# Simple-Robotics/proxsuite

Hardware: AMD Instinct MI355X
Metric: QPs/sec (batch, dense backend) at fixed (n, n_eq, n_in); max |KKT residual| vs ref (higher is better)
Workload: dtype f64; 1 GPU; c2: 2048 random dense fp64 QPs per GPU, n=100 n_eq=50 n_in=100, eps_abs=1e-09 eps_rel=0 NO_INITIAL_GUESS (reference generators and seeds, benchmark/timings-parallel.cpp:43-63; BASELINE.json configs); batch_per_gpu=2048, n=100, n_eq=50, n_in=100, threads_per_qp=64, lds_bytes_per_qp=18968, parallelism=batch sharded over 1 GPU(s), dense_backend=PrimalDualLDLT

## Files before the change

include/proxqp_hip.h:

```cpp
#ifndef PROXQP_HIP_H
#define PROXQP_HIP_H

#include "pqp_types.h"

#ifdef __cplusplus
extern "C" {
#endif

typedef struct pqp_batch pqp_batch;

enum pqp_error
{
  PQP_OK = 0,
  PQP_ERR_INVALID_ARGUMENT = -1,
  PQP_ERR_NO_DEVICE = -2,
  PQP_ERR_HIP = -3,
  PQP_ERR_UNSUPPORTED = -4
};

#define PQP_STATS_COUNT 33

const char* pqp_last_error(void);
int pqp_device_count(void);

int pqp_batch_create(int64_t batch_size, int64_t dim, int64_t n_eq, int64_t n_in,
                     int box_constraints, int hessian_type, int dense_backend, int device,
                     pqp_batch** out);
void pqp_batch_destroy(pqp_batch* h);

int64_t pqp_batch_size(const pqp_batch* h);
int pqp_batch_dense_backend(const pqp_batch* h);

pqp_settings* pqp_batch_settings(pqp_batch* h, int64_t idx);

int pqp_batch_init(pqp_batch* h, int64_t idx, const double* H, const double* g, const double* A,
                   const double* b, const double* C, const double* l, const double* u,
                   const double* l_box, const double* u_box, int compute_preconditioner,
                   double rho, double mu_eq, double mu_in, double manual_minimal_H_eigenvalue);

int pqp_batch_update(pqp_batch* h, int64_t idx, const double* H, const double* g, const double* A,
                     const double* b, const double* C, const double* l, const double* u,
                     const double* l_box, const double* u_box, int update_preconditioner,
                     double rho, double mu_eq, double mu_in, double manual_minimal_H_eigenvalue);

int pqp_batch_warm_start(pqp_batch* h, int64_t idx, const double* x, const double* y,
                         const double* z);

int pqp_batch_cleanup(pqp_batch* h, int64_t idx);

int pqp_batch_reset_qp(pqp_batch* h, int64_t idx);

int pqp_batch_flush(pqp_batch* h);

int pqp_batch_solve(pqp_batch* h);

int pqp_batch_solve_range(pqp_batch* h, int64_t first, int64_t count);

int pqp_batch_solve_subset(pqp_batch* h, const int64_t* idx, int64_t count);

int pqp_batch_solve_async(pqp_batch* h);
int pqp_batch_solve_range_async(pqp_batch* h, int64_t first, int64_t count);
int pqp_batch_solve_subset_async(pqp_batch* h, const int64_t* idx, int64_t count);
int pqp_batch_wait(pqp_batch* h);

int pqp_batch_enable_host_results(pqp_batch* h, int enable);
int pqp_batch_host_results(pqp_batch* h, const double** x, const double** y, const double** z, const double** se,
                           const double** si, const pqp_info** info);
int pqp_batch_host_results_fresh(pqp_batch* h, int64_t idx);
int pqp_batch_host_results_fresh_range(pqp_batch* h, int64_t first, int64_t count);

int pqp_batch_copy_qp(pqp_batch* dst, int64_t dst_idx, pqp_batch* src, int64_t src_idx);

int pqp_batch_set_stream(pqp_batch* h, void* stream);
int pqp_batch_own_stream(pqp_batch* h);

int pqp_batch_backward(pqp_batch* h, const double* loss_derivatives, double eps, double rho_backward,
                       double mu_backward);
int pqp_batch_backward_range(pqp_batch* h, int64_t first, int64_t count, const double* loss_derivatives,
                             double eps, double rho_backward, double mu_backward);
int pqp_batch_backward_subset(pqp_batch* h, const int64_t* idx, int64_t count, const double* loss_derivatives,
                              double eps, double rho_backward, double mu_backward);
int pqp_batch_get_backward(pqp_batch* h, int64_t idx, double* dL_dH, double* dL_dg, double* dL_dA,
                           double* dL_db, double* dL_dC, double* dL_du, double* dL_dl);

int pqp_batch_set_schedule(pqp_batch* h, int longest_first);

int pqp_batch_get_results(pqp_batch* h, int64_t idx, double* x, double* y, double* z, double* se,
                          double* si, pqp_info* info);

int pqp_batch_result_device_ptrs(pqp_batch* h, double** x, double** y, double** z);

int pqp_batch_pack_results(pqp_batch* h, int64_t first, int64_t count, double* out, void* stream);

int pqp_batch_get_scaled(pqp_batch* h, int64_t idx, double* H, double* g, double* A, double* b,
                         double* C, double* l, double* u, double* delta, double* c);

int pqp_batch_get_schur_factor(pqp_batch* h, int64_t idx, double* WS, double* dS, double* G, int32_t* slots,
                               int64_t* meta, double* mus);

int pqp_batch_get_primal_factor(pqp_batch* h, int64_t idx, double* F, double* dF, double* WL, double* WU,
                                double* Zr, double* Zc, int64_t* meta, double* rho, double* i_scaled);

int pqp_batch_get_stats(pqp_batch* h, int64_t* stats);

int pqp_batch_get_trace(pqp_batch* h, int64_t idx, double* records, int64_t capacity, int64_t* n_records);

double pqp_batch_last_solve_ms(const pqp_batch* h);
double pqp_batch_last_prologue_ms(const pqp_batch* h);
int pqp_batch_launch_config(const pqp_batch* h, int* threads, int64_t* lds_bytes);
const char* pqp_batch_last_kernel(const pqp_batch* h);

typedef struct pqp_multi pqp_multi;
int pqp_multi_create(int64_t batch_size, int64_t dim, int64_t n_eq, int64_t n_in, int box_constraints,
                     int hessian_type, int dense_backend, const int* devices, int n_devices, pqp_multi** out);
void pqp_multi_destroy(pqp_multi* m);
int64_t pqp_multi_size(const pqp_multi* m);
int pqp_multi_shard_count(const pqp_multi* m);
int pqp_multi_shard(pqp_multi* m, int g, pqp_batch** shard, int64_t* first, int64_t* count);
int pqp_multi_locate(const pqp_multi* m, int64_t idx, int* shard, int64_t* local);
pqp_settings* pqp_multi_settings(pqp_multi* m, int64_t idx);
int pqp_multi_init(pqp_multi* m, int64_t idx, const double* H, const double* g, const double* A, const double* b,
                   const double* C, const double* l, const double* u, const double* l_box, const double* u_box,
                   int compute_preconditioner, double rho, double mu_eq, double mu_in,
                   double manual_minimal_H_eigenvalue);
int pqp_multi_update(pqp_multi* m, int64_t idx, const double* H, const double* g, const double* A, const double* b,
                     const double* C, const double* l, const double* u, const double* l_box, const double* u_box,
                     int update_preconditioner, double rho, double mu_eq, double mu_in,
                     double manual_minimal_H_eigenvalue);
int pqp_multi_warm_start(pqp_multi* m, int64_t idx, const double* x, const double* y, const double* z);
int pqp_multi_cleanup(pqp_multi* m, int64_t idx);
int pqp_multi_flush(pqp_multi* m);
int pqp_multi_solve(pqp_multi* m);
int pqp_multi_solve_range(pqp_multi* m, int64_t first, int64_t count);
int pqp_multi_solve_async(pqp_multi* m);
int pqp_multi_solve_range_async(pqp_multi* m, int64_t first, int64_t count);
int pqp_multi_wait(pqp_multi* m);
int pqp_multi_get_results(pqp_multi* m, int64_t idx, double* x, double* y, double* z, double* se, double* si,
                          pqp_info* info);
int pqp_multi_gather_device(pqp_multi* m, int root_shard, double* out);
int pqp_multi_get_trace(pqp_multi* m, int64_t idx, double* records, int64_t capacity, int64_t* n_records);
double pqp_multi_last_solve_ms(const pqp_multi* m);

int pqp_box_calibrate(int device, double* out, int n_out);

#ifdef __cplusplus
}
#endif

#endif
```

proxsuite_amd/_build.py:

```python
from __future__ import annotations

import os
import shutil
import subprocess
from pathlib import Path

ROOT = Path(__file__).resolve().parent.parent
CSRC = ROOT / "proxsuite_amd" / "csrc"
INCLUDE = ROOT / "include"

HIP_LIB = CSRC / "libproxqp_hip.so"
HIP_STATS_LIB = CSRC / "libproxqp_hip_stats.so"
RANDQP_LIB = CSRC / "libpqp_randqp.so"

HOST_CXXFLAGS = ["-O3", "-march=x86-64-v3", "-mtune=generic", "-std=gnu++17", "-fPIC", "-fopenmp"]


def _newer(target: Path, sources) -> bool:
    if not target.exists():
        return False
    t = target.stat().st_mtime
    return all(Path(s).stat().st_mtime <= t for s in sources)


def _run(cmd, cwd=None):
    r = subprocess.run(cmd, cwd=cwd, capture_output=True, text=True)
    if r.returncode != 0:
        raise RuntimeError("build failed: %s\n%s\n%s" % (" ".join(map(str, cmd)), r.stdout, r.stderr))
    return r


def build_randqp(force: bool = False) -> Path:
    src = [CSRC / "random_qp.cpp"]
    if not force and _newer(RANDQP_LIB, src):
        return RANDQP_LIB
    _run(["g++", *HOST_CXXFLAGS, "-shared", "-o", str(RANDQP_LIB), *map(str, src)])
    return RANDQP_LIB


KERNEL_TUS = (1, 2, 3, 4, 5, 6, 7, 8, 9, 12, 13, 14, 15, 16, 17, 18)
OBJ_DIR = ROOT / "build" / "obj"


def hip_sources():
    return [CSRC / "pqp_capi.hip", CSRC / "pqp_multi.hip", CSRC / "pqp_kernels.hip", CSRC / "pqp_calib.hip"]


def hip_headers():
    return sorted(CSRC.glob("*.hpp")) + sorted(INCLUDE.glob("*.h"))


CODEGEN_FLAGS = ["-mllvm", "-sink-insts-to-avoid-spills", "-mllvm", "-disable-machine-licm"]
TU_FLAGS = {17: ["-mllvm", "-disable-lsr"],
            18: ["-mllvm", "-disable-lsr", "-DPQP_ZG_DEPTH=4"],
            1: ["-mllvm", "-disable-lsr"], 4: ["-mllvm", "-disable-lsr"], 7: ["-mllvm", "-disable-lsr"], 13: ["-mllvm", "-disable-lsr"], 15: ["-mllvm", "-disable-lsr"]}


def hip_flags(extra_flags=()):
    return ["--offload-arch=gfx950", "-O3", "-std=c++17", "-fPIC", "-ffp-contract=fast", *CODEGEN_FLAGS,
            "-Rpass-analysis=kernel-resource-usage",
            "-I", str(INCLUDE), "-I", str(CSRC), *extra_flags]


def parse_kernel_resources(stderr: str) -> dict:
    import re
    out, cur = {}, None
    for line in stderr.splitlines():
        m = re.search(r"remark:\s+(Function Name|[A-Za-z ]+(?:\[[^\]]*\])?):\s*(\S+)", line)
        if not m:
            continue
        key, val = m.group(1).strip(), m.group(2)
        if key == "Function Name":
            cur = out.setdefault(val, {})
        elif cur is not None:
            key = re.sub(r"\s*\[.*\]", "", key).strip().replace(" ", "_")
            try:
                cur[key] = int(val)
            except ValueError:
                cur[key] = val
    return out


def kernel_label(mangled: str) -> str:
    import re
    m = re.match(r"_Z\d+([A-Za-z_0-9]+?)I((?:Li\d+E)+)E", mangled)
    if not m:
        return mangled
    return "%s<%s>" % (m.group(1), ",".join(re.findall(r"Li(\d+)E", m.group(2))))


def flags_tag(extra_flags) -> str:
    import hashlib
    return "v" + hashlib.sha1(" ".join(extra_flags).encode()).hexdigest()[:8]


def hipcc() -> str:
    return shutil.which("hipcc") or "/opt/rocm/bin/hipcc"


HOST_OBJECTS = {"capi.o": "pqp_capi.hip", "multi.o": "pqp_multi.hip", "calib.o": "pqp_calib.hip"}


def hip_objects(odir: Path, tus=KERNEL_TUS):
    return [odir / o for o in HOST_OBJECTS] + [odir / ("kernels_%d.o" % k) for k in tus]


def compile_tu(k: int, obj: Path, extra_flags=()):
    return _run([hipcc(), *hip_flags(extra_flags), *TU_FLAGS.get(k, []), "-DPQP_TU=%d" % k, "-c",
                 str(CSRC / "pqp_kernels.hip"), "-o", str(obj)])


def link_hip(lib: Path, odir: Path = None, replaced=None, tus=KERNEL_TUS) -> Path:
    odir, replaced = odir or OBJ_DIR / "default", replaced or {}
    Path(lib).parent.mkdir(parents=True, exist_ok=True)
    _run([hipcc(), "--offload-arch=gfx950", "-shared", "-fPIC", "-o", str(lib),
          *[str(replaced.get(o.name, o)) for o in hip_objects(odir, tus)]])
    return Path(lib)


def build_hip(force: bool = False, extra_flags=(), out: Path = None, tus=KERNEL_TUS) -> Path:
    from concurrent.futures import ThreadPoolExecutor
    lib = Path(out) if out else HIP_LIB
    deps = list(hip_sources()) + hip_headers() + [Path(__file__)]
    if not force and _newer(lib, deps):
        return lib
    tag = "default" if not extra_flags else flags_tag(extra_flags)
    odir = OBJ_DIR / tag
    odir.mkdir(parents=True, exist_ok=True)
    common = hip_headers() + [Path(__file__)]
    only = {"pqp_dwave.hpp": ("kernels_17.o", "kernels_6.o")}
    def deps_of(o):
        return [h for h in common if h.name not in only or o.name in only[h.name]] + [CSRC / HOST_OBJECTS.get(o.name, "pqp_kernels.hip")]
    def compile_object(o):
        if o.name in HOST_OBJECTS:
            return _run([hipcc(), *hip_flags(extra_flags), "-c", str(CSRC / HOST_OBJECTS[o.name]), "-o", str(o)])
        return compile_tu(int(o.stem.split("_")[1]), o, extra_flags)
    todo = [o for o in hip_objects(odir, tus) if force or not _newer(o, deps_of(o))]
    with ThreadPoolExecutor(max_workers=max(1, min(len(todo), os.cpu_count() or 1))) as ex:
        results = list(ex.map(compile_object, todo))
    link_hip(lib, odir, tus=tus)
    import json
    rec_path = odir / "kernel_resources.json"
    rec = json.loads(rec_path.read_text()) if rec_path.exists() else {}
    for o, r in zip(todo, results):
        rec = {k: v for k, v in rec.items() if v.get("object") != o.name}
        for name, fields in parse_kernel_resources(r.stderr).items():
            rec[kernel_label(name)] = dict(fields, object=o.name)
    rec_path.write_text(json.dumps(rec, indent=1, sort_keys=True))
    return lib


def kernel_resources(tag: str = "default") -> dict:
    import json
    p = OBJ_DIR / tag / "kernel_resources.json"
    rec = json.loads(p.read_text()) if p.exists() else {}
    live = {"kernels_%d.o" % k for k in KERNEL_TUS}
    return {k: v for k, v in rec.items() if v.get("object") in live}


def build_hip_stats(force: bool = False) -> Path:
    lib = HIP_STATS_LIB
    deps = list(hip_sources()) + hip_headers() + [Path(__file__)]
    if not force and _newer(lib, deps):
        return lib
    return build_hip(extra_flags=("-DPQP_STATS",), out=lib)


VARIANT_DIR = CSRC / "variants"


def build_hip_variants(force: bool = False):
    out = []
    deps = list(hip_sources()) + hip_headers() + [Path(__file__)]
    build_hip()
    for w in (3, 4):
        lib = VARIANT_DIR / ("libproxqp_hip_wps512_%d.so" % w)
        if force or not _newer(lib, deps):
            o3 = OBJ_DIR / "default" / ("kernels_3_wps%d.o" % w)
            compile_tu(3, o3, ("-DPQP_WPS_512=%d" % w,))
            link_hip(lib, replaced={"kernels_3.o": o3})
        out.append(lib)
    return out


def build_tu_variant(tu, extra_flags, out: Path):
    build_hip()
    repl, res = {}, {}
    for t in ([tu] if isinstance(tu, int) else list(tu)):
        o = OBJ_DIR / "default" / ("kernels_%d_%s.o" % (t, flags_tag(extra_flags)))
        r = compile_tu(t, o, tuple(extra_flags))
        repl["kernels_%d.o" % t] = o
        res.update({kernel_label(k): v for k, v in parse_kernel_resources(r.stderr).items()})
    return link_hip(out, replaced=repl), res


def build_oracle(force: bool = False) -> Path:
    odir = ROOT / "oracle"
    lib = odir / "liboracle.so"
    srcs = [odir / "proxqp_oracle.cpp", odir / "oracle_capi.cpp", odir / "proxqp_oracle.hpp",
            odir / "ldlt_oracle.hpp", INCLUDE / "pqp_types.h", odir / "Makefile"]
    if not force and _newer(lib, srcs):
        return lib
    if force and lib.exists():
        os.remove(lib)
    _run(["make", "-C", str(odir), "-B" if force else "-s", "liboracle.so"])
    return lib


def kernel_sources_sha(diag: bool = False, dwave: bool = False) -> str:
    import hashlib
    files = ["pqp_solver.hpp", "pqp_block.hpp"] + (["pqp_diag.hpp"] if diag or dwave else []) + (["pqp_dwave.hpp"] if dwave else [])
    import re
    h = hashlib.sha256()
    for f in files:
        text = (CSRC / f).read_text()
        text = re.sub(r"/\*.*?\*/", "", text, flags=re.S)
        lines = [re.sub(r"//.*$", "", ln).rstrip() for ln in text.splitlines()]
        h.update("\n".join(ln for ln in lines if ln.strip()).encode())
    return h.hexdigest()[:16]


def freeze_kernel_resources():
    import json
    build_hip()
    rec = kernel_resources()
    keep = ("VGPRs", "AGPRs", "VGPRs_Spill", "SGPRs_Spill", "ScratchSize", "Occupancy")
    out = {k: {f: v[f] for f in keep if f in v} for k, v in sorted(rec.items()) if k.startswith("pqp_")}
    p = ROOT / "tests" / "golden" / "kernel_resources_expected.json"
    p.write_text(json.dumps(out, indent=1, sort_keys=True))
    return p


if __name__ == "__main__":
    import sys
    if "--freeze" in sys.argv:
        print(freeze_kernel_resources())
```

proxsuite_amd/_native.py:

```python
from __future__ import annotations

import ctypes as C
import os
from pathlib import Path

import numpy as np

from ._ctypes_defs import pqp_info, pqp_settings

PQP_STATS_COUNT = 33
STAT_NAMES = ("cyc_total", "cyc_scale", "cyc_factor_h", "cyc_zg", "cyc_schur", "cyc_kkt_solve",
              "cyc_residual", "cyc_linesearch", "cyc_global_res", "cyc_newton_misc", "n_newton",
              "n_schur_fact", "n_new_rows", "n_kkt_solves", "n_ls_breakpoints", "n_active_final",
              "cyc_f_load", "cyc_f_update", "cyc_f_panel", "cyc_f_writeback", "cyc_f_tinv", "cyc_s_gather",
              "cyc_solve_ldlt", "n_schur_blocked", "n_append", "n_delete", "bytes_engine", "n_refactorize", "cyc_ls_eval", "cyc_cert", "cyc_update", "wall_ticks", "flops_fact")

_DP = C.POINTER(C.c_double)
NAN = float("nan")


class NativeError(RuntimeError):
    pass


class _Tolerant:

    class _Sink:
        pass

    def __init__(self, lib):
        object.__setattr__(self, "_lib", lib)

    def __getattr__(self, name):
        try:
            return getattr(object.__getattribute__(self, "_lib"), name)
        except AttributeError:
            return _Tolerant._Sink()


class NativeLib:

    SYMBOLS = ("pqp_last_error", "pqp_device_count", "pqp_batch_create", "pqp_batch_destroy",
               "pqp_batch_size", "pqp_batch_dense_backend", "pqp_batch_settings", "pqp_batch_init",
               "pqp_batch_update", "pqp_batch_warm_start", "pqp_batch_cleanup", "pqp_batch_reset_qp", "pqp_batch_flush",
               "pqp_batch_solve", "pqp_batch_solve_range", "pqp_batch_solve_subset", "pqp_batch_copy_qp", "pqp_batch_set_stream", "pqp_batch_set_schedule", "pqp_batch_backward", "pqp_batch_backward_range",
               "pqp_batch_get_backward", "pqp_batch_get_results", "pqp_batch_result_device_ptrs", "pqp_batch_pack_results",
               "pqp_batch_get_scaled", "pqp_batch_get_schur_factor", "pqp_batch_get_primal_factor", "pqp_batch_get_stats", "pqp_batch_get_trace", "pqp_batch_last_solve_ms", "pqp_batch_last_prologue_ms",
               "pqp_batch_launch_config", "pqp_batch_last_kernel", "pqp_batch_solve_async", "pqp_batch_solve_range_async",
               "pqp_batch_solve_subset_async", "pqp_batch_wait", "pqp_batch_enable_host_results",
               "pqp_batch_host_results", "pqp_batch_host_results_fresh", "pqp_batch_own_stream", "pqp_batch_backward_subset",
               "pqp_multi_create", "pqp_multi_destroy", "pqp_multi_size", "pqp_multi_shard_count", "pqp_multi_shard",
               "pqp_multi_locate", "pqp_multi_settings", "pqp_multi_init", "pqp_multi_update", "pqp_multi_warm_start",
               "pqp_multi_cleanup", "pqp_multi_flush", "pqp_multi_solve", "pqp_multi_solve_range",
               "pqp_multi_solve_async", "pqp_multi_solve_range_async", "pqp_multi_wait", "pqp_multi_get_results",
               "pqp_multi_gather_device", "pqp_multi_get_trace", "pqp_multi_last_solve_ms", "pqp_box_calibrate",
               "pqp_batch_host_results_fresh_range")

    def __init__(self, path, legacy=False):
        self.path = str(path)
        real = C.CDLL(self.path)
        L = _Tolerant(real) if legacy else real
        vp = C.c_void_p
        L.pqp_last_error.restype = C.c_char_p
        L.pqp_device_count.restype = C.c_int
        L.pqp_batch_create.argtypes = [C.c_int64] * 4 + [C.c_int] * 4 + [C.POINTER(vp)]
        L.pqp_batch_destroy.argtypes = [vp]
        L.pqp_batch_destroy.restype = None
        L.pqp_batch_size.argtypes = [vp]
        L.pqp_batch_size.restype = C.c_int64
        L.pqp_batch_dense_backend.argtypes = [vp]
        L.pqp_batch_settings.argtypes = [vp, C.c_int64]
        L.pqp_batch_settings.restype = C.POINTER(pqp_settings)
        for name in ("pqp_batch_init", "pqp_batch_update"):
            getattr(L, name).argtypes = [vp, C.c_int64] + [_DP] * 9 + [C.c_int] + [C.c_double] * 4
        L.pqp_batch_warm_start.argtypes = [vp, C.c_int64] + [_DP] * 3
        L.pqp_batch_cleanup.argtypes = [vp, C.c_int64]
        L.pqp_batch_reset_qp.argtypes = [vp, C.c_int64]
        L.pqp_batch_flush.argtypes = [vp]
        L.pqp_batch_solve.argtypes = [vp]
        L.pqp_batch_solve_range.argtypes = [vp, C.c_int64, C.c_int64]
        L.pqp_batch_solve_subset.argtypes = [vp, C.POINTER(C.c_int64), C.c_int64]
        L.pqp_batch_copy_qp.argtypes = [vp, C.c_int64, vp, C.c_int64]
        L.pqp_batch_set_stream.argtypes = [vp, vp]
        L.pqp_batch_set_schedule.argtypes = [vp, C.c_int]
        L.pqp_batch_backward.argtypes = [vp, _DP] + [C.c_double] * 3
        L.pqp_batch_backward_range.argtypes = [vp, C.c_int64, C.c_int64, _DP] + [C.c_double] * 3
        L.pqp_batch_get_backward.argtypes = [vp, C.c_int64] + [_DP] * 7
        L.pqp_batch_get_results.argtypes = [vp, C.c_int64] + [_DP] * 5 + [C.POINTER(pqp_info)]
        L.pqp_batch_result_device_ptrs.argtypes = [vp] + [C.POINTER(_DP)] * 3
        L.pqp_batch_pack_results.argtypes = [vp, C.c_int64, C.c_int64, vp, vp]
        L.pqp_batch_get_scaled.argtypes = [vp, C.c_int64] + [_DP] * 9
        L.pqp_batch_get_stats.argtypes = [vp, C.POINTER(C.c_int64)]
        L.pqp_batch_get_trace.argtypes = [vp, C.c_int64, C.c_void_p, C.c_int64, C.POINTER(C.c_int64)]
        L.pqp_batch_get_schur_factor.argtypes = [vp, C.c_int64] + [_DP] * 3 + [C.POINTER(C.c_int32), C.POINTER(C.c_int64), _DP]
        L.pqp_batch_get_primal_factor.argtypes = [vp, C.c_int64] + [_DP] * 6 + [C.POINTER(C.c_int64), _DP, _DP]
        L.pqp_batch_last_solve_ms.argtypes = [vp]
        L.pqp_batch_last_solve_ms.restype = C.c_double
        L.pqp_batch_last_prologue_ms.argtypes = [vp]
        L.pqp_batch_last_prologue_ms.restype = C.c_double
        L.pqp_batch_launch_config.argtypes = [vp, C.POINTER(C.c_int), C.POINTER(C.c_int64)]
        L.pqp_batch_last_kernel.argtypes = [vp]
        L.pqp_batch_last_kernel.restype = C.c_char_p
        L.pqp_batch_solve_async.argtypes = [vp]
        L.pqp_batch_solve_range_async.argtypes = [vp, C.c_int64, C.c_int64]
        L.pqp_batch_solve_subset_async.argtypes = [vp, C.POINTER(C.c_int64), C.c_int64]
        L.pqp_batch_wait.argtypes = [vp]
        L.pqp_batch_enable_host_results.argtypes = [vp, C.c_int]
        L.pqp_batch_host_results.argtypes = [vp] + [C.POINTER(_DP)] * 5 + [C.POINTER(C.POINTER(pqp_info))]
        L.pqp_batch_host_results_fresh.argtypes = [vp, C.c_int64]
        L.pqp_batch_own_stream.argtypes = [vp]
        L.pqp_batch_backward_subset.argtypes = [vp, C.POINTER(C.c_int64), C.c_int64, _DP] + [C.c_double] * 3
        L.pqp_multi_create.argtypes = [C.c_int64] * 4 + [C.c_int] * 3 + [C.POINTER(C.c_int), C.c_int, C.POINTER(vp)]
        L.pqp_multi_destroy.argtypes = [vp]
        L.pqp_multi_destroy.restype = None
        L.pqp_multi_size.argtypes = [vp]
        L.pqp_multi_size.restype = C.c_int64
        L.pqp_multi_shard_count.argtypes = [vp]
        L.pqp_multi_shard.argtypes = [vp, C.c_int, C.POINTER(vp), C.POINTER(C.c_int64), C.POINTER(C.c_int64)]
        L.pqp_multi_locate.argtypes = [vp, C.c_int64, C.POINTER(C.c_int), C.POINTER(C.c_int64)]
        L.pqp_multi_settings.argtypes = [vp, C.c_int64]
        L.pqp_multi_settings.restype = C.POINTER(pqp_settings)
        for name in ("pqp_multi_init", "pqp_multi_update"):
            getattr(L, name).argtypes = [vp, C.c_int64] + [_DP] * 9 + [C.c_int] + [C.c_double] * 4
        L.pqp_multi_warm_start.argtypes = [vp, C.c_int64] + [_DP] * 3
        L.pqp_multi_cleanup.argtypes = [vp, C.c_int64]
        for name in ("pqp_multi_flush", "pqp_multi_solve", "pqp_multi_solve_async", "pqp_multi_wait"):
            getattr(L, name).argtypes = [vp]
        for name in ("pqp_multi_solve_range", "pqp_multi_solve_range_async"):
            getattr(L, name).argtypes = [vp, C.c_int64, C.c_int64]
        L.pqp_multi_get_results.argtypes = [vp, C.c_int64] + [_DP] * 5 + [C.POINTER(pqp_info)]
        L.pqp_multi_gather_device.argtypes = [vp, C.c_int, vp]
        L.pqp_multi_last_solve_ms.argtypes = [vp]
        L.pqp_multi_last_solve_ms.restype = C.c_double
        L.pqp_multi_get_trace.argtypes = [vp, C.c_int64, C.c_void_p, C.c_int64, C.POINTER(C.c_int64)]
        L.pqp_box_calibrate.argtypes = [C.c_int, _DP, C.c_int]
        L.pqp_batch_host_results_fresh_range.argtypes = [vp, C.c_int64, C.c_int64]
        self.L = real

    def check(self, rc):
        if rc != 0:
            msg = self.L.pqp_last_error().decode(errors="replace")
            if rc == -1:
                raise ValueError(msg)
            raise NativeError("libproxqp_hip error %d: %s" % (rc, msg))


_lib = None


def hip_library_path() -> Path:
    override = os.environ.get("PQP_HIP_LIBRARY")
    if override:
        return Path(override).resolve()
    return Path(__file__).resolve().parent / "csrc" / "libproxqp_hip.so"


def load() -> NativeLib:
    global _lib
    if _lib is None:
        p = hip_library_path()
        if not p.exists():
            raise NativeError("%s is missing: build it with `python -c 'import __graft_entry__ as g; "
                              "g.build()'` (hipcc --offload-arch=gfx950); there is no CPU fallback" % p)
        try:
            import torch
        except ImportError:
            pass
        lib = NativeLib(p)
        if lib.L.pqp_device_count() <= 0:
            raise NativeError("no HIP device visible: proxsuite_amd runs on MI355X only (no CPU fallback)")
        _lib = lib
    return _lib


def box_calibration(device: int = 0, lib: NativeLib = None) -> dict:
    lib = lib or load()
    out = (C.c_double * 8)()
    rc = lib.L.pqp_box_calibrate(int(device), out, 8)
    if rc != 0:
        raise NativeError("pqp_box_calibrate: %s" % (lib.L.pqp_last_error() or b"").decode())
    return {"hbm_read_gbs": out[0], "chain_ms": out[1], "valu_ms": out[2], "sclk_mhz_est": out[3], "n_cu": int(out[4])}


def _as_array(a, shape, name):
    if a is None:
        return None, None
    if hasattr(a, "data_ptr"):
        import torch
        if a.numel() == 0:
            return None, None
        t = a.detach()
        if t.dtype != torch.float64 or not t.is_contiguous():
            t = t.to(torch.float64).contiguous()
        if tuple(t.shape) != tuple(shape):
            raise ValueError("wrong argument size: %s has shape %s, expected %s" % (name, tuple(t.shape), shape))
        return t, C.cast(t.data_ptr(), _DP)
    arr = np.ascontiguousarray(np.asarray(a, dtype=np.float64))
    if arr.size == 0:
        return None, None
    if tuple(arr.shape) != tuple(shape):
        raise ValueError("wrong argument size: %s has shape %s, expected %s" % (name, arr.shape, tuple(shape)))
    return arr, arr.ctypes.data_as(_DP)


def _opt(v):
    return NAN if v is None else float(v)


class Batch:

    def __init__(self, batch_size, n, n_eq, n_in, box_constraints=False, hessian_type=1, dense_backend=0,
                 device=0, lib: NativeLib | None = None):
        self.lib = lib if lib is not None else load()
        self.B, self.n, self.n_eq, self.n_in = int(batch_size), int(n), int(n_eq), int(n_in)
        self.box = bool(box_constraints)
        self.n_c = self.n_in + (self.n if self.box else 0)
        h = C.c_void_p()
        self.lib.check(self.lib.L.pqp_batch_create(self.B, self.n, self.n_eq, self.n_in, int(self.box),
                                                   int(hessian_type), int(dense_backend), int(device),
                                                   C.byref(h)))
        self._h = h

    def close(self):
        if getattr(self, "_h", None):
            self.lib.L.pqp_batch_destroy(self._h)
            self._h = None

    def __del__(self):
        try:
            self.close()
        except Exception:
            pass

    @property
    def dense_backend(self):
        return self.lib.L.pqp_batch_dense_backend(self._h)

    def settings(self, idx) -> pqp_settings:
        p = self.lib.L.pqp_batch_settings(self._h, int(idx))
        if not p:
            raise IndexError(idx)
        return p.contents

    def settings_table(self):
        p = self.lib.L.pqp_batch_settings(self._h, 0)
        arr = (pqp_settings * self.B).from_address(C.addressof(p.contents))
        return np.frombuffer(arr, dtype=np.dtype(pqp_settings))

    def set_all_settings(self, **fields):
        tab = self.settings_table()
        for k, v in fields.items():
            tab[k][:] = v

    def _shapes(self, idx):
        pre = (self.B,) if idx < 0 else ()
        n, ne, ni = self.n, self.n_eq, self.n_in
        return dict(H=pre + (n, n), g=pre + (n,), A=pre + (ne, n), b=pre + (ne,), C=pre + (ni, n),
                    l=pre + (ni,), u=pre + (ni,), l_box=pre + (n,), u_box=pre + (n,))

    def _setup(self, fn, idx, H, g, A, b, Cm, l, u, l_box, u_box, flag, rho, mu_eq, mu_in, min_eig):
        sh = self._shapes(idx)
        keep, ptrs = [], []
        for name, arr in (("H", H), ("g", g), ("A", A), ("b", b), ("C", Cm), ("l", l), ("u", u),
                          ("l_box", l_box), ("u_box", u_box)):
            k, p = _as_array(arr, sh[name], name)
            keep.append(k)
            ptrs.append(p)
        self.lib.check(fn(self._h, int(idx), *ptrs, int(bool(flag)), _opt(rho), _opt(mu_eq), _opt(mu_in),
                          _opt(min_eig)))

    def init(self, idx=-1, H=None, g=None, A=None, b=None, C=None, l=None, u=None, l_box=None, u_box=None,
             compute_preconditioner=True, rho=None, mu_eq=None, mu_in=None, manual_minimal_H_eigenvalue=None):
        self._setup(self.lib.L.pqp_batch_init, idx, H, g, A, b, C, l, u, l_box, u_box,
                    compute_preconditioner, rho, mu_eq, mu_in, manual_minimal_H_eigenvalue)

    def update(self, idx=-1, H=None, g=None, A=None, b=None, C=None, l=None, u=None, l_box=None, u_box=None,
               update_preconditioner=False, rho=None, mu_eq=None, mu_in=None,
               manual_minimal_H_eigenvalue=None):
        self._setup(self.lib.L.pqp_batch_update, idx, H, g, A, b, C, l, u, l_box, u_box,
                    update_preconditioner, rho, mu_eq, mu_in, manual_minimal_H_eigenvalue)

    def warm_start(self, idx=-1, x=None, y=None, z=None):
        pre = (self.B,) if idx < 0 else ()
        kx, px = _as_array(x, pre + (self.n,), "x")
        ky, py = _as_array(y, pre + (self.n_eq,), "y")
        kz, pz = _as_array(z, pre + (self.n_c,), "z")
        self.lib.check(self.lib.L.pqp_batch_warm_start(self._h, int(idx), px, py, pz))

    def cleanup(self, idx=-1):
        self.lib.check(self.lib.L.pqp_batch_cleanup(self._h, int(idx)))

    def flush(self):
        self.lib.check(self.lib.L.pqp_batch_flush(self._h))

    def solve(self, first=None, count=None):
        if first is None:
            self.lib.check(self.lib.L.pqp_batch_solve(self._h))
        else:
            self.lib.check(self.lib.L.pqp_batch_solve_range(self._h, int(first), int(1 if count is None else count)))

    def solve_async(self, first=None, count=None):
        if first is None:
            self.lib.check(self.lib.L.pqp_batch_solve_async(self._h))
        else:
            self.lib.check(self.lib.L.pqp_batch_solve_range_async(self._h, int(first), int(1 if count is None else count)))

    def wait(self):
        self.lib.check(self.lib.L.pqp_batch_wait(self._h))

    def solve_subset(self, idx, asynchronous=False):
        ii = np.ascontiguousarray(idx, dtype=np.int64)
        fn = self.lib.L.pqp_batch_solve_subset_async if asynchronous else self.lib.L.pqp_batch_solve_subset
        self.lib.check(fn(self._h, ii.ctypes.data_as(C.POINTER(C.c_int64)), len(ii)))

    def enable_host_results(self, on=True):
        self.lib.check(self.lib.L.pqp_batch_enable_host_results(self._h, int(bool(on))))

    def host_results(self):
        px = [_DP() for _ in range(5)]
        pi = C.POINTER(pqp_info)()
        self.lib.check(self.lib.L.pqp_batch_host_results(self._h, *[C.byref(p) for p in px], C.byref(pi)))
        shapes = ((self.B, self.n), (self.B, self.n_eq), (self.B, self.n_c), (self.B, self.n_eq), (self.B, self.n_c))
        out = []
        for p, sh in zip(px, shapes):
            cnt = sh[0] * sh[1]
            out.append(np.ctypeslib.as_array(p, shape=(cnt,)).reshape(sh) if cnt else np.zeros(sh))
        if self.B:
            arr = (pqp_info * self.B).from_address(C.addressof(pi.contents))
            info = np.frombuffer(arr, dtype=np.dtype(pqp_info))
        else:
            info = np.zeros(0, dtype=np.dtype(pqp_info))
        return (*out, info)

    def host_results_fresh(self, idx=-1, count=None):
        if count is not None:
            return bool(self.lib.L.pqp_batch_host_results_fresh_range(self._h, int(idx), int(count)))
        return bool(self.lib.L.pqp_batch_host_results_fresh(self._h, int(idx)))

    def backward(self, loss_derivatives, eps=1e-4, rho_backward=1e-6, mu_backward=1e-6, first=None, count=None):
        ntot = self.n + self.n_eq + self.n_in
        rows = self.B if first is None else int(1 if count is None else count)
        k, p = _as_array(loss_derivatives, (rows, ntot), "loss_derivatives")
        if first is None:
            self.lib.check(self.lib.L.pqp_batch_backward(self._h, p, float(eps), float(rho_backward),
                                                         float(mu_backward)))
        else:
            self.lib.check(self.lib.L.pqp_batch_backward_range(self._h, int(first), rows, p, float(eps),
                                                               float(rho_backward), float(mu_backward)))

    def backward_results(self, idx=-1, into=None):
        pre = (self.B,) if idx < 0 else ()
        n, ne, ni = self.n, self.n_eq, self.n_in
        shapes = dict(dL_dH=pre + (n, n), dL_dg=pre + (n,), dL_dA=pre + (ne, n), dL_db=pre + (ne,),
                      dL_dC=pre + (ni, n), dL_du=pre + (ni,), dL_dl=pre + (ni,))
        out = into if into is not None else {k: np.zeros(v) for k, v in shapes.items()}
        ptrs = []
        for name in ("dL_dH", "dL_dg", "dL_dA", "dL_db", "dL_dC", "dL_du", "dL_dl"):
            buf = out.get(name)
            if buf is None or (hasattr(buf, "numel") and buf.numel() == 0) or (
                    not hasattr(buf, "numel") and buf.size == 0):
                ptrs.append(None)
            elif hasattr(buf, "data_ptr"):
                import torch
                if buf.dtype != torch.float64 or not buf.is_contiguous() or tuple(buf.shape) != shapes[name]:
                    raise ValueError("backward_results: %s must be contiguous float64 of shape %s" % (name, shapes[name]))
                ptrs.append(C.cast(buf.data_ptr(), _DP))
            else:
                ptrs.append(buf.ctypes.data_as(_DP))
        self.lib.check(self.lib.L.pqp_batch_get_backward(self._h, int(idx), *ptrs))
        return out

    def pack_results(self, out, first=0, count=None, stream=None):
        count = self.B - first if count is None else count
        ptr = out.data_ptr() if hasattr(out, "data_ptr") else (out.ctypes.data if hasattr(out, "ctypes") else int(out))
        self.lib.check(self.lib.L.pqp_batch_pack_results(self._h, int(first), int(count), C.c_void_p(ptr),
                                                         C.c_void_p(int(stream) if stream else None)))
        return out

    def set_schedule(self, longest_first=True):
        self.lib.check(self.lib.L.pqp_batch_set_schedule(self._h, int(bool(longest_first))))

    def own_stream(self):
        self.lib.check(self.lib.L.pqp_batch_own_stream(self._h))

    def backward_subset(self, idx, loss_derivatives, eps=1e-4, rho_backward=1e-6, mu_backward=1e-6):
        ntot = self.n + self.n_eq + self.n_in
        ii = np.ascontiguousarray(idx, dtype=np.int64)
        k, p = _as_array(loss_derivatives, (len(ii), ntot), "loss_derivatives")
        self.lib.check(self.lib.L.pqp_batch_backward_subset(self._h, ii.ctypes.data_as(C.POINTER(C.c_int64)), len(ii), p,
                                                            float(eps), float(rho_backward), float(mu_backward)))

    def set_stream(self, stream):
        self.lib.check(self.lib.L.pqp_batch_set_stream(self._h, C.c_void_p(int(stream) if stream else None)))

    @property
    def last_solve_ms(self):
        return self.lib.L.pqp_batch_last_solve_ms(self._h)

    @property
    def last_prologue_ms(self):
        return self.lib.L.pqp_batch_last_prologue_ms(self._h)

    def results(self, idx=-1):
        pre = (self.B,) if idx < 0 else ()
        x = np.zeros(pre + (self.n,))
        y = np.zeros(pre + (self.n_eq,))
        z = np.zeros(pre + (self.n_c,))
        se = np.zeros(pre + (self.n_eq,))
        si = np.zeros(pre + (self.n_c,))
        info = (pqp_info * self.B)() if idx < 0 else pqp_info()
        p = lambda a: a.ctypes.data_as(_DP)
        ip = C.cast(info, C.POINTER(pqp_info)) if idx < 0 else C.byref(info)
        self.lib.check(self.lib.L.pqp_batch_get_results(self._h, int(idx), p(x), p(y), p(z), p(se), p(si), ip))
        return x, y, z, se, si, info

    def results_into(self, x=None, y=None, z=None, se=None, si=None, idx=-1):
        pre = (self.B,) if idx < 0 else ()
        want = dict(x=pre + (self.n,), y=pre + (self.n_eq,), z=pre + (self.n_c,), se=pre + (self.n_eq,),
                    si=pre + (self.n_c,))
        ptrs = []
        for name, buf in (("x", x), ("y", y), ("z", z), ("se", se), ("si", si)):
            if buf is None or (hasattr(buf, "numel") and buf.numel() == 0) or (hasattr(buf, "size") and not callable(buf.size) and buf.size == 0):
                ptrs.append(None)
                continue
            if hasattr(buf, "data_ptr"):
                import torch
                if buf.dtype != torch.float64 or not buf.is_contiguous() or tuple(buf.shape) != want[name]:
                    raise ValueError("results_into: %s must be a contiguous float64 tensor of shape %s" % (name, want[name]))
                ptrs.append(C.cast(buf.data_ptr(), _DP))
            else:
                if buf.dtype != np.float64 or not buf.flags.c_contiguous or tuple(buf.shape) != want[name]:
                    raise ValueError("results_into: %s must be a C-contiguous float64 array of shape %s" % (name, want[name]))
                ptrs.append(buf.ctypes.data_as(_DP))
        self.lib.check(self.lib.L.pqp_batch_get_results(self._h, int(idx), *ptrs, None))

    def infos(self):
        info = (pqp_info * self.B)()
        self.lib.check(self.lib.L.pqp_batch_get_results(self._h, -1, None, None, None, None, None,
                                                        C.cast(info, C.POINTER(pqp_info))))
        return info

    def scaled(self, idx):
        n, ne, ni = self.n, self.n_eq, self.n_in
        out = dict(H=np.zeros((n, n)), g=np.zeros(n), A=np.zeros((ne, n)), b=np.zeros(ne), C=np.zeros((ni, n)),
                   l=np.zeros(ni), u=np.zeros(ni), delta=np.zeros(n + ne + self.n_c))
        c = C.c_double(0)
        p = lambda a: a.ctypes.data_as(_DP)
        self.lib.check(self.lib.L.pqp_batch_get_scaled(
            self._h, int(idx), p(out["H"]), p(out["g"]), p(out["A"]), p(out["b"]), p(out["C"]), p(out["l"]),
            p(out["u"]), p(out["delta"]), C.cast(C.byref(c), _DP)))
        out["c"] = c.value
        return out

    def schur_factor(self, idx):
        nd, nc = self.n_eq + self.n_c, self.n_c
        WS, dS, G = np.zeros((nd, nd)), np.zeros(nd), np.zeros((nd, nd))
        slots, meta, mus = np.zeros(max(nc, 1), dtype=np.int32), np.zeros(4, dtype=np.int64), np.zeros(2)
        self.lib.check(self.lib.L.pqp_batch_get_schur_factor(
            self._h, idx, WS.ctypes.data_as(_DP), dS.ctypes.data_as(_DP), G.ctypes.data_as(_DP),
            slots.ctypes.data_as(C.POINTER(C.c_int32)), meta.ctypes.data_as(C.POINTER(C.c_int64)), mus.ctypes.data_as(_DP)))
        return WS, dS, G, slots[:nc], dict(zip(("n_slots", "n_c", "ls_valid", "ls_edited"), meta.tolist())), mus

    def primal_factor(self, idx):
        n, nd = self.n, self.n_eq + self.n_c
        out = dict(F=np.zeros((n, n)), dF=np.zeros(n), WL=np.zeros((n, n)), WU=np.zeros((n, n)), Zr=np.zeros((nd, n)),
                   Zc=np.zeros((n, nd)), i_scaled=np.zeros(n))
        meta, rho = np.zeros(4, dtype=np.int64), C.c_double(0)
        p = lambda a: a.ctypes.data_as(_DP)
        self.lib.check(self.lib.L.pqp_batch_get_primal_factor(
            self._h, int(idx), p(out["F"]), p(out["dF"]), p(out["WL"]), p(out["WU"]), p(out["Zr"]), p(out["Zc"]),
            meta.ctypes.data_as(C.POINTER(C.c_int64)), C.cast(C.byref(rho), _DP), p(out["i_scaled"])))
        out["rho"] = rho.value
        out["meta"] = dict(zip(("factor_valid", "diag_mode", "backend", "hessian"), meta.tolist()))
        return out

    def stats(self):
        a = np.zeros((self.B, PQP_STATS_COUNT), dtype=np.int64)
        self.lib.check(self.lib.L.pqp_batch_get_stats(self._h, a.ctypes.data_as(C.POINTER(C.c_int64))))
        return a

    def trace(self, idx):
        n = C.c_int64(0)
        self.lib.check(self.lib.L.pqp_batch_get_trace(self._h, int(idx), None, 0, C.byref(n)))
        out = np.zeros((n.value, 8))
        if n.value:
            self.lib.check(self.lib.L.pqp_batch_get_trace(self._h, int(idx), out.ctypes.data, n.value, C.byref(n)))
        return out

    @property
    def last_kernel(self):
        return self.lib.L.pqp_batch_last_kernel(self._h).decode()

    def launch_config(self):
        t = C.c_int(0)
        b = C.c_int64(0)
        self.lib.check(self.lib.L.pqp_batch_launch_config(self._h, C.byref(t), C.byref(b)))
        return t.value, b.value

    def result_device_ptrs(self):
        x, y, z = _DP(), _DP(), _DP()
        self.lib.check(self.lib.L.pqp_batch_result_device_ptrs(self._h, C.byref(x), C.byref(y), C.byref(z)))
        return tuple(C.cast(p, C.c_void_p).value for p in (x, y, z))



class MultiBatch:

    def __init__(self, batch_size, n, n_eq, n_in, devices, box_constraints=False, hessian_type=1, dense_backend=0,
                 lib: NativeLib | None = None):
        self.lib = lib if lib is not None else load()
        self.B, self.n, self.n_eq, self.n_in = int(batch_size), int(n), int(n_eq), int(n_in)
        self.box = bool(box_constraints)
        self.n_c = self.n_in + (self.n if self.box else 0)
        devs = (C.c_int * len(devices))(*[int(d) for d in devices])
        h = C.c_void_p()
        self.lib.check(self.lib.L.pqp_multi_create(self.B, self.n, self.n_eq, self.n_in, int(self.box), int(hessian_type),
                                                   int(dense_backend), devs, len(devices), C.byref(h)))
        self._h = h
        self.devices = [int(d) for d in devices]

    def close(self):
        if getattr(self, "_h", None):
            self.lib.L.pqp_multi_destroy(self._h)
            self._h = None

    def __del__(self):
        try:
            self.close()
        except Exception:
            pass

    @property
    def shard_count(self):
        return self.lib.L.pqp_multi_shard_count(self._h)

    def shard(self, g):
        f, c = C.c_int64(0), C.c_int64(0)
        self.lib.check(self.lib.L.pqp_multi_shard(self._h, int(g), None, C.byref(f), C.byref(c)))
        return f.value, c.value

    def settings(self, idx) -> pqp_settings:
        p = self.lib.L.pqp_multi_settings(self._h, int(idx))
        if not p:
            raise IndexError(idx)
        return p.contents

    _shapes = Batch._shapes

    def _setup(self, fn, idx, H, g, A, b, Cm, l, u, l_box, u_box, flag, rho, mu_eq, mu_in, min_eig):
        Batch._setup(self, fn, idx, H, g, A, b, Cm, l, u, l_box, u_box, flag, rho, mu_eq, mu_in, min_eig)

    def init(self, idx=-1, H=None, g=None, A=None, b=None, C=None, l=None, u=None, l_box=None, u_box=None,
             compute_preconditioner=True, rho=None, mu_eq=None, mu_in=None, manual_minimal_H_eigenvalue=None):
        self._setup(self.lib.L.pqp_multi_init, idx, H, g, A, b, C, l, u, l_box, u_box, compute_preconditioner, rho, mu_eq,
                    mu_in, manual_minimal_H_eigenvalue)
# ... 61 lines not shown
```

proxsuite_amd/csrc/pqp_capi.hip:

```cpp
#include <hip/hip_runtime.h>

#include <algorithm>
#include <cmath>
#include <cstdio>
#include <cstdlib>
#include <cstring>
#include <limits>
#include <string>
#include <vector>

#include "pqp_host.hpp"
#include "pqp_diag.hpp"

namespace {

thread_local std::string g_err;

bool
absent(double v)
{
  return std::isnan(v);
}

int
// ... 237 lines not shown
    h->dev.wall_us_per_tick =
      (hipDeviceGetAttribute(&khz, hipDeviceAttributeWallClockRate, device) == hipSuccess && khz > 0) ? 1.0e3 / double(khz)
                                                                                                      : 1.0e-2;
  }
  h->backend = dense_backend_choice(dense_backend, dim, n_eq, n_in, box_constraints != 0);
  pqp::Dims& d = h->dev.d;
  d.n = int(dim);
  d.n_eq = int(n_eq);
  d.n_in = int(n_in);
  d.box = box_constraints ? 1 : 0;
  d.nc = int(n_in + (box_constraints ? dim : 0));
  d.nd = d.n_eq + d.nc;
  d.ntot = d.n + d.nd;
  d.hessian = hessian_type;
  d.backend = h->backend;
  d._pad = 0;
  h->dev.B = batch_size;
  const int need = d.nd > d.n ? d.nd : d.n;
  h->nt = need <= 256 ? 256 : (need <= 512 ? 512 : 1024);
  if (need > PQP_MAX_ROWS || pqp::setup_lds_bytes(d, 1024) > 160 * 1024) {
    delete h;
    return fail(PQP_ERR_UNSUPPORTED, "max(n, n_eq + n_in (+ n)) > " + std::to_string(PQP_MAX_ROWS) +
                                       " (or n + n_eq + n_in (+ n) > ~10000) is not supported by this build");
  }
#if PQP_CHUNK_ALL
  if (const char* e = std::getenv("PQP_TEST_NT_MAX")) {
    const int f = std::atoi(e);
    if ((f == 256 || f == 512) && h->nt > f)
      h->nt = f;
  }
#endif
  if (const char* e = std::getenv("PQP_SCHEDULE"))
    h->lpt = std::string(e) == "lpt";
  h->dev.rep_phase = 0;
  h->dev.rep_count = 1;
  h->dev.trace = nullptr;
  h->dev.trace_slot = nullptr;
  h->dev.trace_cap = 0;
  if (const char* e = std::getenv("PQP_REPEAT_PHASE"))
    h->dev.rep_phase = std::atoi(e);
  if (const char* e = std::getenv("PQP_REPEAT_COUNT"))
    h->dev.rep_count = std::atoi(e);
  h->lds_solve = pqp::lds_bytes(d, h->nt);
  h->lds_setup = pqp::setup_lds_bytes(d, h->nt);
  const char* force_hbm = std::getenv("PQP_FORCE_HBM_VECTORS");
  const bool vectors_in_hbm = h->lds_solve > 160 * 1024 || (force_hbm && force_hbm[0] == '1');
  if (vectors_in_hbm)
    h->nt = 1024;
  const size_t B = size_t(batch_size), n = size_t(dim), ne = size_t(n_eq), ni = size_t(n_in),
               nc = size_t(d.nc), nd = size_t(d.nd);
  pqp::Batch& D = h->dev;
  int rc = 0;
#define ALLOC(ptr, cnt)                                                                             \
  if ((rc = dalloc(h, &(ptr), (cnt)))) {                                                            \
    pqp_batch_destroy(h);                                                                           \
    return rc;                                                                                      \
  }                                                                                                 \
  if (B > 0 && size_t(cnt) % B == 0 && (void*)(ptr) != (void*)h->d_order && (void*)(ptr) != (void*)h->d_cmd)           \
    h->per_qp.push_back({ reinterpret_cast<char*>(ptr), (size_t(cnt) / B) * sizeof(*(ptr)) });
  ALLOC(D.H, B * n * n)
  ALLOC(D.g, B * n)
  ALLOC(D.A, B * ne * n)
  ALLOC(D.b, B * ne)
  ALLOC(D.C, B * ni * n)
  ALLOC(D.u, B * ni)
  ALLOC(D.l, B * ni)
  ALLOC(D.u_box, B * n)
  ALLOC(D.l_box, B * n)
  ALLOC(D.Hs, B * n * n)
  ALLOC(D.gs, B * n)
  ALLOC(D.As, B * ne * n)
  ALLOC(D.ATs, B * ne * n)
  ALLOC(D.bs, B * ne)
  ALLOC(D.Cs, B * ni * n)
  ALLOC(D.CTs, B * ni * n)
  ALLOC(D.us, B * ni)
  ALLOC(D.ls, B * ni)
  ALLOC(D.ubs, B * n)
  ALLOC(D.lbs, B * n)
  ALLOC(D.is, B * n)
  ALLOC(D.delta, B * size_t(d.ntot))
  ALLOC(D.x, B * n)
  ALLOC(D.y, B * ne)
  ALLOC(D.z, B * nc)
  ALLOC(D.se, B * ne)
  ALLOC(D.si, B * nc)
  ALLOC(D.info, B)
  ALLOC(D.state, B)
  ALLOC(D.F, B * n * n)
  ALLOC(D.WL, B * n * n)
  ALLOC(D.WU, B * n * n)
  ALLOC(D.dF, B * n)
  ALLOC(D.Zr, B * nd * n)
  ALLOC(D.Zc, B * nd * n)
  ALLOC(D.G, B * nd * nd)
  ALLOC(D.WS, B * nd * nd)
  ALLOC(D.LS, B * nd * nd)
  ALLOC(D.dS, B * nd)
  ALLOC(D.act, B * nc)
  ALLOC(D.stats, B * size_t(pqp::ST_COUNT))
  if (vectors_in_hbm) {
    h->lds_solve = pqp::lds_bytes(d, h->nt);
    h->lds_setup = pqp::setup_lds_bytes(d, h->nt);
    if ((rc = dalloc(h, &h->vec_scratch, B * ((h->lds_solve + 7) / 8)))) {
      pqp_batch_destroy(h);
      return rc;
    }
  }
  ALLOC(h->d_order, B)
  ALLOC(h->d_settings, B)
  ALLOC(h->d_cmd, B)
#undef ALLOC
  D.settings = h->d_settings;
  D.cmd = h->d_cmd;

  h->settings.resize(B);
  for (auto& s : h->settings)
    pqp_settings_default(&s, h->backend);
  h->cmd.assign(B, pqp::Cmd{});
  h->is_initialized.assign(B, 0);
  h->c_diag.assign(B, 0);
  {
    std::vector<pqp_info> info(B);
    for (auto& i : info)
      pqp_info_default(&i, h->backend);
    if (B)
      HIP_TRY(hipMemcpy(D.info, info.data(), B * sizeof(pqp_info), hipMemcpyHostToDevice));
    std::vector<pqp::State> st(B);
    for (auto& s : st) {
      std::memset(&s, 0, sizeof(s));
      s.ruiz_c = 1.0;
    }
    if (B)
      HIP_TRY(hipMemcpy(D.state, st.data(), B * sizeof(pqp::State), hipMemcpyHostToDevice));
    const double ib = std::sqrt(std::numeric_limits<double>::max());
    std::vector<double> tmp;
    auto fill = [&](double* dst, size_t cnt, double v) -> int {
      if (!cnt)
        return PQP_OK;
      tmp.assign(cnt, v);
      HIP_TRY(hipMemcpy(dst, tmp.data(), cnt * sizeof(double), hipMemcpyHostToDevice));
      return PQP_OK;
    };
    if ((rc = fill(D.u, B * ni, +ib)) || (rc = fill(D.l, B * ni, -ib)) ||
        (rc = fill(D.u_box, B * n, +ib)) || (rc = fill(D.l_box, B * n, -ib)) ||
        (rc = fill(D.delta, B * size_t(d.ntot), 1.0)) || (rc = fill(D.is, B * n, 1.0))) {
      pqp_batch_destroy(h);
      return rc;
    }
  }
  HIP_TRY(hipEventCreate(&h->ev0));
  HIP_TRY(hipEventCreate(&h->ev1));
  HIP_TRY(hipEventCreate(&h->ev_mid));
  *out = h;
  return PQP_OK;
}

void
pqp_batch_destroy(pqp_batch* h)
{
  if (!h)
    return;
  (void)settle(h);
  DeviceGuard guard_(h->device);
  for (void* p : h->host_allocs)
    (void)hipHostFree(p);
  if (h->owned_stream)
    (void)hipStreamDestroy(h->owned_stream);
  for (void* p : h->allocs)
    (void)hipFree(p);
  if (h->trace_dev)
    (void)hipFree(h->trace_dev);
  if (h->trace_slot_dev)
    (void)hipFree(h->trace_slot_dev);
  if (h->ev0)
    (void)hipEventDestroy(h->ev0);
  if (h->ev1)
    (void)hipEventDestroy(h->ev1);
  if (h->ev_mid)
    (void)hipEventDestroy(h->ev_mid);
  delete h;
}

int64_t
pqp_batch_size(const pqp_batch* h)
{
  return h ? h->dev.B : 0;
}

int
pqp_batch_dense_backend(const pqp_batch* h)
{
  return h ? h->backend : PQP_BACKEND_AUTOMATIC;
}

pqp_settings*
pqp_batch_settings(pqp_batch* h, int64_t idx)
{
  if (!h || idx < 0 || idx >= h->dev.B)
    return nullptr;
  return &h->settings[size_t(idx)];
}

int
pqp_batch_init(pqp_batch* h, int64_t idx, const double* H, const double* g, const double* A,
               const double* b, const double* C, const double* l, const double* u,
               const double* l_box, const double* u_box, int compute_preconditioner, double rho,
               double mu_eq, double mu_in, double manual_minimal_H_eigenvalue)
{
  if (h && h->dev.d.box == 0 && (l_box || u_box))
    return fail(PQP_ERR_INVALID_ARGUMENT,
                "wrong model setup: the QP object is designed without box constraints, but is "
                "initialized with lower or upper box inequalities.");
  return enqueue_setup(h, idx, false, H, g, A, b, C, l, u, l_box, u_box, compute_preconditioner ? 1 : 0,
                       rho, mu_eq, mu_in, manual_minimal_H_eigenvalue);
}

int
pqp_batch_update(pqp_batch* h, int64_t idx, const double* H, const double* g, const double* A,
                 const double* b, const double* C, const double* l, const double* u,
                 const double* l_box, const double* u_box, int update_preconditioner, double rho,
                 double mu_eq, double mu_in, double manual_minimal_H_eigenvalue)
{
  return enqueue_setup(h, idx, true, H, g, A, b, C, l, u, l_box, u_box, update_preconditioner ? 1 : 0,
                       rho, mu_eq, mu_in, manual_minimal_H_eigenvalue);
}

int
pqp_batch_warm_start(pqp_batch* h, int64_t idx, const double* x, const double* y, const double* z)
{
  if (int rc = check_idx(h, idx))
    return rc;
  if (!x && !y && !z)
    return PQP_OK;
  if (int rc = settle(h))
    return rc;
  mirror_stale(h, idx);
  PQP_ON_DEVICE(h->device);
  if (h->cmd_pending)
    if (int rc = pqp_batch_flush(h))
      return rc;
  const pqp::Dims& d = h->dev.d;
  int rc = 0;
  if ((rc = copy_in(h->dev.x, x, idx, h->dev.B, size_t(d.n))) ||
      (rc = copy_in(h->dev.y, y, idx, h->dev.B, size_t(d.n_eq))) ||
      (rc = copy_in(h->dev.z, z, idx, h->dev.B, size_t(d.nc))))
    return rc;
  const int64_t lo = idx < 0 ? 0 : idx, hi = idx < 0 ? h->dev.B : idx + 1;
  for (int64_t q = lo; q < hi; ++q)
    h->settings[size_t(q)].initial_guess = PQP_WARM_START;
  return PQP_OK;
}

int
pqp_batch_cleanup(pqp_batch* h, int64_t idx)
{
  if (int rc = check_idx(h, idx))
    return rc;
  if (int rc = settle(h))
    return rc;
  mirror_stale(h, idx);
  if (h->cmd_pending)
    if (int rc = pqp_batch_flush(h))
      return rc;
  const int64_t lo = idx < 0 ? 0 : idx, hi = idx < 0 ? h->dev.B : idx + 1;
  for (int64_t q = lo; q < hi; ++q) {
    pqp::Cmd c{};
    c.op = pqp::CMD_CLEANUP;
    h->cmd[size_t(q)] = c;
    h->is_initialized[size_t(q)] = 0;
  }
  h->cmd_pending = true;
  return pqp_batch_flush(h);
}

int
pqp_batch_reset_qp(pqp_batch* h, int64_t idx)
{
  if (!h || idx < 0 || idx >= h->dev.B)
    return fail(PQP_ERR_INVALID_ARGUMENT, "QP index out of range");
  if (int rc = settle(h))
    return rc;
  mirror_stale(h, idx);
  PQP_ON_DEVICE(h->device);
  if (h->cmd_pending)
    if (int rc = pqp_batch_flush(h))
      return rc;
  const size_t q = size_t(idx);
  for (const auto& a : h->per_qp)
    HIP_TRY(hipMemset(a.base + q * a.bytes_per_qp, 0, a.bytes_per_qp));
  pqp::Batch& D = h->dev;
  const pqp::Dims& d = D.d;
  const size_t n = size_t(d.n), ni = size_t(d.n_in);
  pqp_info info;
  pqp_info_default(&info, h->backend);
  HIP_TRY(hipMemcpy(D.info + q, &info, sizeof(info), hipMemcpyHostToDevice));
  pqp::State st;
  std::memset(&st, 0, sizeof(st));
  st.ruiz_c = 1.0;
  HIP_TRY(hipMemcpy(D.state + q, &st, sizeof(st), hipMemcpyHostToDevice));
  const double ib = std::sqrt(std::numeric_limits<double>::max());
  std::vector<double> tmp;
  auto fill = [&](double* dst, size_t cnt, double v) -> int {
    if (!cnt)
      return PQP_OK;
    tmp.assign(cnt, v);
    HIP_TRY(hipMemcpy(dst, tmp.data(), cnt * sizeof(double), hipMemcpyHostToDevice));
    return PQP_OK;
  };
  int rc = 0;
  if ((rc = fill(D.u + q * ni, ni, +ib)) || (rc = fill(D.l + q * ni, ni, -ib)) ||
      (rc = fill(D.u_box + q * n, n, +ib)) || (rc = fill(D.l_box + q * n, n, -ib)) ||
      (rc = fill(D.delta + q * size_t(d.ntot), size_t(d.ntot), 1.0)) || (rc = fill(D.is + q * n, n, 1.0)))
    return rc;
  pqp_settings_default(&h->settings[q], h->backend);
  h->settings_dirty = true;
  h->settings_uploaded.clear();
  h->cmd[q] = pqp::Cmd{};
  h->is_initialized[q] = 0;
  h->c_diag[q] = 0;
  h->order_valid = false;
  return PQP_OK;
}

int
pqp_batch_flush(pqp_batch* h)
{
  if (!h)
    return fail(PQP_ERR_INVALID_ARGUMENT, "null batch handle");
  if (!h->cmd_pending || h->dev.B == 0)
    return PQP_OK;
  if (int rc = settle(h))
    return rc;
// ... 154 lines not shown
static int
verbose_report(pqp_batch* h, const int64_t* idx, int64_t first, int64_t count)
{
  bool any = false;
  for (int64_t i = 0; i < count && !any; ++i)
    any = h->settings[size_t(idx ? idx[i] : first + i)].verbose != 0;
  if (!any)
    return PQP_OK;
  if (h->dev.trace) {
    int nv = 0;
    for (int s : h->trace_slot)
      nv = std::max(nv, s + 1);
    h->trace_host.resize(size_t(nv) * PQP_TRACE_RECORDS * 8);
    HIP_TRY(hipMemcpy(h->trace_host.data(), h->trace_dev, h->trace_host.size() * sizeof(double), hipMemcpyDeviceToHost));
  }
  const pqp::Dims& d = h->dev.d;
  static const char* const status_name[] = { "Solved", "Maximum number of iterations reached", "Primal infeasible",
                                             "Solved closest primal feasible", "Dual infeasible", "Solver not run" };
  for (int64_t i = 0; i < count; ++i) {
    const int64_t q = idx ? idx[i] : first + i;
    const pqp_settings& st = h->settings[size_t(q)];
    if (!st.verbose)
      continue;
    pqp_info info;
    HIP_TRY(hipMemcpy(&info, h->dev.info + q, sizeof(info), hipMemcpyDeviceToHost));
    std::printf("-------------------------------------------------------------------------------------------------\n"
                "ProxQP dense backend, batched on MI355X (QP %lld of the batch)\n"
                "problem:  \n          variables n = %d, equality constraints n_eq = %d,\n"
                "          inequality constraints n_in = %d\n"
                "settings: \n          backend = dense,\n          eps_abs = %g eps_rel = %g\n"
                "          eps_prim_inf = %g, eps_dual_inf = %g,\n          rho = %g, mu_eq = %g, mu_in = %g,\n"
                "          max_iter = %lld, max_iter_in = %lld,\n          box constraints: %s, \n"
                "          dense backend: %s, \n          problem type: %s, \n          scaling: %s, \n"
                "          timings: %s, \n",
                (long long)q, d.n, d.n_eq, d.n_in, st.eps_abs, st.eps_rel, st.eps_primal_inf, st.eps_dual_inf, info.rho,
                info.mu_eq, info.mu_in, (long long)st.max_iter, (long long)st.max_iter_in, d.box ? "on" : "off",
                h->backend == PQP_BACKEND_PRIMAL_LDLT ? "PrimalLDLT" : "PrimalDualLDLT",
                d.hessian == PQP_HESSIAN_DENSE
                  ? "Quadratic Program"
                  : (d.hessian == PQP_HESSIAN_ZERO ? "Linear Program" : "Quadratic Program with diagonal Hessian"),
                st.compute_preconditioner ? "on" : "off", st.compute_timings ? "on" : "off");
    if (!h->trace_host.empty() && h->trace_slot[size_t(q)] >= 0)
      print_trace(h->trace_host.data() + size_t(h->trace_slot[size_t(q)]) * PQP_TRACE_RECORDS * 8);
    std::printf("-------------------SOLVER STATISTICS-------------------\n"
                "outer iter:     %lld\ntotal iter:     %lld\nmu updates:     %lld\nrho updates:    %lld\n"
                "objective:      %g\nstatus:         %s\n",
                (long long)info.iter_ext, (long long)info.iter, (long long)info.mu_updates,
                (long long)info.rho_updates, info.objValue,
                (info.status >= 0 && info.status <= 5) ? status_name[info.status] : "?");
    if (st.compute_timings)
      std::printf("run time [\xce\xbcs]:  %g\n", info.solve_time);
    std::printf("--------------------------------------------------------\n");
  }
  std::fflush(stdout);
  return PQP_OK;
}

static int
finish_solve(pqp_batch* h)
{
  const int64_t* idx = h->flight_idx.empty() ? nullptr : h->flight_idx.data();
  const int64_t first = h->flight_first, count = h->flight_count;
  for (int64_t i = 0; i < count; ++i) {
    const size_t q = size_t(idx ? idx[i] : first + i);
    h->is_initialized[q] = 1;
    if (h->host_results)
      h->mirror_fresh[q] = 1;
  }
  return verbose_report(h, idx, first, count);
}

static int
solve_impl(pqp_batch* h, int64_t first, int64_t count, const int64_t* idx, bool async)
{
  if (!h)
    return fail(PQP_ERR_INVALID_ARGUMENT, "null batch handle");
  if (int rc = settle(h))
    return rc;
  std::vector<int> order;
  if (idx) {
    if (count < 0 || count > h->dev.B)
      return fail(PQP_ERR_INVALID_ARGUMENT, "subset larger than the batch");
    if (count == 0)
      return PQP_OK;
    order.resize(static_cast<size_t>(count));
    std::vector<char> seen(static_cast<size_t>(h->dev.B), 0);
    for (int64_t i = 0; i < count; ++i) {
      if (idx[i] < 0 || idx[i] >= h->dev.B)
        return fail(PQP_ERR_INVALID_ARGUMENT, "QP index out of range");
      if (seen[size_t(idx[i])])
        return fail(PQP_ERR_INVALID_ARGUMENT, "pqp_batch_solve_subset: a QP index is listed twice");
      seen[size_t(idx[i])] = 1;
      order[size_t(i)] = int(idx[i]);
    }
  } else {
    if (first < 0 || count < 0 || first + count > h->dev.B)
      return fail(PQP_ERR_INVALID_ARGUMENT, "solve range [" + std::to_string(first) + ", " +
                                              std::to_string(first + count) + ") outside the batch of " +
                                              std::to_string(h->dev.B) + " QPs");
    if (count == 0)
      return PQP_OK;
  }
  PQP_ON_DEVICE(h->device);
  if (int rc = pqp_batch_flush(h))
    return rc;
  if (int rc = upload_settings(h))
    return rc;
  if (int rc = prepare_trace(h, idx, first, count))
    return rc;
  int rc = 0;
  if (idx) {
    HIP_TRY(hipMemcpy(h->d_order, order.data(), order.size() * sizeof(int), hipMemcpyHostToDevice));
    h->order_valid = false;
    h->range_first = 0;
    h->range_count = long(count);
    h->subset_order = h->d_order;
    h->subset_host = &order;
    rc = pqp_launch_solve(h);
    h->subset_order = nullptr;
    h->subset_host = nullptr;
    h->flight_idx.assign(idx, idx + count);
  } else {
    h->range_first = first;
    h->range_count = count;
    rc = pqp_launch_solve(h);
    h->flight_idx.clear();
    if (!rc && h->lpt && first == 0 && count == h->dev.B && count > 1) {
      rc = pqp_launch_order(h, long(count));
      h->order_valid = rc == 0;
    }
  }
  if (rc)
    return rc;
  h->flight_first = long(first);
  h->flight_count = long(count);
  h->solve_in_flight = true;
  return async ? PQP_OK : pqp_batch_wait(h);
}

int
pqp_batch_wait(pqp_batch* h)
{
  if (!h)
    return fail(PQP_ERR_INVALID_ARGUMENT, "null batch handle");
  if (!h->solve_in_flight)
    return PQP_OK;
  PQP_ON_DEVICE(h->device);
  h->solve_in_flight = false;
  HIP_TRY(hipEventSynchronize(h->ev1));
  HIP_TRY(hipEventElapsedTime(&h->last_ms, h->ev0, h->ev1));
  h->last_prologue_ms = 0.f;
  if (h->prologue_timed)
    HIP_TRY(hipEventElapsedTime(&h->last_prologue_ms, h->ev0, h->ev_mid));
  return finish_solve(h);
}

int
pqp_batch_solve_range(pqp_batch* h, int64_t first, int64_t count)
{
  return solve_impl(h, first, count, nullptr, false);
}

int
pqp_batch_solve_subset(pqp_batch* h, const int64_t* idx, int64_t count)
{
  if (!h || (count > 0 && !idx))
    return fail(PQP_ERR_INVALID_ARGUMENT, "null argument");
  if (count == 0)
    return PQP_OK;
  return solve_impl(h, 0, count, idx, false);
}

int
pqp_batch_solve_async(pqp_batch* h)
{
  if (!h)
    return fail(PQP_ERR_INVALID_ARGUMENT, "null batch handle");
  return solve_impl(h, 0, h->dev.B, nullptr, true);
}

int
pqp_batch_solve_range_async(pqp_batch* h, int64_t first, int64_t count)
{
  return solve_impl(h, first, count, nullptr, true);
}

int
pqp_batch_solve_subset_async(pqp_batch* h, const int64_t* idx, int64_t count)
{
  if (!h || (count > 0 && !idx))
    return fail(PQP_ERR_INVALID_ARGUMENT, "null argument");
  if (count == 0)
    return PQP_OK;
  return solve_impl(h, 0, count, idx, true);
}

int
pqp_batch_enable_host_results(pqp_batch* h, int enable)
{
  if (!h)
    return fail(PQP_ERR_INVALID_ARGUMENT, "null batch handle");
  if (int rc = settle(h))
    return rc;
  if ((enable != 0) == h->host_results)
    return PQP_OK;
  PQP_ON_DEVICE(h->device);
  pqp::Batch& D = h->dev;
  if (!enable) {
    for (void* p : h->host_allocs)
      (void)hipHostFree(p);
    h->host_allocs.clear();
    D.hx = D.hy = D.hz = D.hse = D.hsi = nullptr;
    D.hinfo = nullptr;
    h->m_x = h->m_y = h->m_z = h->m_se = h->m_si = nullptr;
    h->m_info = nullptr;
    h->host_results = false;
    return PQP_OK;
  }
  const pqp::Dims& d = D.d;
  const size_t B = size_t(D.B);
  auto halloc = [&](size_t bytes, void** host, void** dev) -> int {
    void* p = nullptr;
    HIP_TRY(hipHostMalloc(&p, bytes ? bytes : 8, hipHostMallocMapped));
    h->host_allocs.push_back(p);
    std::memset(p, 0, bytes ? bytes : 8);
    void* dp = nullptr;
    HIP_TRY(hipHostGetDevicePointer(&dp, p, 0));
    *host = p;
    *dev = dp;
    return PQP_OK;
  };
  int rc = 0;
  if ((rc = halloc(B * size_t(d.n) * 8, (void**)&h->m_x, (void**)&D.hx)) ||
      (rc = halloc(B * size_t(d.n_eq) * 8, (void**)&h->m_y, (void**)&D.hy)) ||
      (rc = halloc(B * size_t(d.nc) * 8, (void**)&h->m_z, (void**)&D.hz)) ||
      (rc = halloc(B * size_t(d.n_eq) * 8, (void**)&h->m_se, (void**)&D.hse)) ||
      (rc = halloc(B * size_t(d.nc) * 8, (void**)&h->m_si, (void**)&D.hsi)) ||
      (rc = halloc(B * sizeof(pqp_info), (void**)&h->m_info, (void**)&D.hinfo))) {
    for (void* p : h->host_allocs)
      (void)hipHostFree(p);
    h->host_allocs.clear();
    D.hx = D.hy = D.hz = D.hse = D.hsi = nullptr;
    D.hinfo = nullptr;
    return rc;
  }
  h->mirror_fresh.assign(B, 0);
  h->host_results = true;
  return PQP_OK;
}

int
pqp_batch_host_results(pqp_batch* h, const double** x, const double** y, const double** z, const double** se,
                       const double** si, const pqp_info** info)
{
  if (!h)
    return fail(PQP_ERR_INVALID_ARGUMENT, "null batch handle");
  if (!h->host_results)
    return fail(PQP_ERR_INVALID_ARGUMENT, "pqp_batch_enable_host_results has not been called on this batch");
  if (int rc = settle(h))
    return rc;
  if (x)
    *x = h->m_x;
  if (y)
    *y = h->m_y;
  if (z)
    *z = h->m_z;
  if (se)
    *se = h->m_se;
  if (si)
    *si = h->m_si;
  if (info)
    *info = h->m_info;
  return PQP_OK;
}

int
pqp_batch_host_results_fresh(pqp_batch* h, int64_t idx)
{
  if (!h || !h->host_results || idx < -1 || idx >= h->dev.B)
    return 0;
  if (settle(h))
    return 0;
  if (idx >= 0)
    return h->mirror_fresh[size_t(idx)] ? 1 : 0;
  for (char c : h->mirror_fresh)
    if (!c)
      return 0;
  return 1;
}

int
pqp_batch_host_results_fresh_range(pqp_batch* h, int64_t first, int64_t count)
{
  if (!h || !h->host_results || first < 0 || count < 0 || first + count > h->dev.B)
    return 0;
  if (settle(h))
    return 0;
  for (int64_t q = first; q < first + count; ++q)
    if (!h->mirror_fresh[size_t(q)])
      return 0;
  return 1;
}

int
pqp_batch_copy_qp(pqp_batch* dst, int64_t dst_idx, pqp_batch* src, int64_t src_idx)
{
// ... 241 lines not shown
int
pqp_batch_get_scaled(pqp_batch* h, int64_t idx, double* H, double* g, double* A, double* b, double* C,
                     double* l, double* u, double* delta, double* c)
{
  if (int rc = check_idx(h, idx))
    return rc;
  if (idx < 0)
    return fail(PQP_ERR_INVALID_ARGUMENT, "pqp_batch_get_scaled addresses one QP");
  if (int rc = settle(h))
    return rc;
  PQP_ON_DEVICE(h->device);
  if (h->cmd_pending)
    if (int rc = pqp_batch_flush(h))
      return rc;
  const pqp::Dims& d = h->dev.d;
  const pqp::Batch& D = h->dev;
  const size_t n = size_t(d.n), ne = size_t(d.n_eq), ni = size_t(d.n_in);
  int rc = 0;
  if ((rc = copy_out(H, D.Hs, idx, D.B, n * n)) || (rc = copy_out(g, D.gs, idx, D.B, n)) ||
      (rc = copy_out(A, D.As, idx, D.B, ne * n)) || (rc = copy_out(b, D.bs, idx, D.B, ne)) ||
      (rc = copy_out(C, D.Cs, idx, D.B, ni * n)) || (rc = copy_out(l, D.ls, idx, D.B, ni)) ||
      (rc = copy_out(u, D.us, idx, D.B, ni)) || (rc = copy_out(delta, D.delta, idx, D.B, size_t(d.ntot))))
    return rc;
  if (c) {
    pqp::State s;
    HIP_TRY(hipMemcpy(&s, D.state + idx, sizeof(s), hipMemcpyDefault));
    *c = s.ruiz_c;
  }
  return PQP_OK;
}

int
pqp_batch_get_schur_factor(pqp_batch* h, int64_t idx, double* WS, double* dS, double* G, int32_t* slots,
                           int64_t* meta, double* mus)
{
  if (int rc = check_idx(h, idx))
    return rc;
  if (idx < 0)
    return fail(PQP_ERR_INVALID_ARGUMENT, "pqp_batch_get_schur_factor addresses one QP");
  if (int rc = settle(h))
    return rc;
  PQP_ON_DEVICE(h->device);
  const pqp::Dims& d = h->dev.d;
  const pqp::Batch& D = h->dev;
  const size_t nd = size_t(d.nd), nc = size_t(d.nc);
  int rc = 0;
  if ((rc = copy_out(WS, D.WS, idx, D.B, nd * nd)) || (rc = copy_out(dS, D.dS, idx, D.B, nd)) ||
      (rc = copy_out(G, D.G, idx, D.B, nd * nd)))
    return rc;
  if (slots && nc) {
    std::vector<int> raw(nc);
    HIP_TRY(hipMemcpy(raw.data(), D.act + size_t(idx) * nc, nc * sizeof(int), hipMemcpyDefault));
    for (size_t j = 0; j < nc; ++j)
      slots[j] = pqp::act_cid(raw[j]);
  }
  pqp::State s;
  HIP_TRY(hipMemcpy(&s, D.state + idx, sizeof(s), hipMemcpyDefault));
  if (meta) {
    meta[0] = s.n_slots;
    meta[1] = s.n_c;
    meta[2] = s.ls_valid;
    meta[3] = s.ls_edited;
  }
  if (mus) {
    mus[0] = s.mu_eq_fact;
    mus[1] = s.mu_in_fact;
  }
  return PQP_OK;
}

int
pqp_batch_get_primal_factor(pqp_batch* h, int64_t idx, double* F, double* dF, double* WL, double* WU, double* Zr,
                            double* Zc, int64_t* meta, double* rho, double* i_scaled)
{
  if (int rc = check_idx(h, idx))
    return rc;
  if (idx < 0)
    return fail(PQP_ERR_INVALID_ARGUMENT, "pqp_batch_get_primal_factor addresses one QP");
  if (int rc = settle(h))
    return rc;
  PQP_ON_DEVICE(h->device);
  const pqp::Dims& d = h->dev.d;
  const pqp::Batch& D = h->dev;
  const size_t n = size_t(d.n), nd = size_t(d.nd);
  int rc = 0;
  if ((rc = copy_out(F, D.F, idx, D.B, n * n)) || (rc = copy_out(dF, D.dF, idx, D.B, n)) ||
      (rc = copy_out(WL, D.WL, idx, D.B, n * n)) || (rc = copy_out(WU, D.WU, idx, D.B, n * n)) ||
      (rc = copy_out(Zr, D.Zr, idx, D.B, nd * n)) || (rc = copy_out(Zc, D.Zc, idx, D.B, n * nd)) ||
      (rc = copy_out(i_scaled, D.is, idx, D.B, n)))
    return rc;
  pqp::State s;
  HIP_TRY(hipMemcpy(&s, D.state + idx, sizeof(s), hipMemcpyDefault));
  if (meta) {
    meta[0] = s.factor_valid;
    meta[1] = (pqp::diag_structure_signature(d.hessian, d.n_eq, d.n_in, d.box) && s.c_diag != 0) ? 1 : 0;
    meta[2] = d.backend;
    meta[3] = d.hessian;
  }
  if (rho)
    *rho = s.rho_fact;
  return PQP_OK;
}

int
pqp_batch_get_stats(pqp_batch* h, int64_t* stats)
{
  if (!h || !stats)
    return fail(PQP_ERR_INVALID_ARGUMENT, "null argument");
  static_assert(PQP_STATS_COUNT == pqp::ST_COUNT, "stats record size");
  static_assert(sizeof(long long) == sizeof(int64_t), "stats element size");
  if (int rc = settle(h))
    return rc;
  PQP_ON_DEVICE(h->device);
  HIP_TRY(hipMemcpy(stats, h->dev.stats, size_t(h->dev.B) * pqp::ST_COUNT * sizeof(int64_t), hipMemcpyDefault));
  return PQP_OK;
}

int
pqp_batch_get_trace(pqp_batch* h, int64_t idx, double* records, int64_t capacity, int64_t* n_records)
{
  if (!h || !n_records)
    return fail(PQP_ERR_INVALID_ARGUMENT, "null argument");
  if (idx < 0 || idx >= h->dev.B)
    return fail(PQP_ERR_INVALID_ARGUMENT, "QP index out of range");
  if (int rc = settle(h))
    return rc;
  *n_records = 0;
  if (h->trace_host.empty() || h->trace_slot.empty() || h->trace_slot[size_t(idx)] < 0)
    return PQP_OK;
  const double* slot = h->trace_host.data() + size_t(h->trace_slot[size_t(idx)]) * PQP_TRACE_RECORDS * 8;
  const int64_t n = int64_t(slot[0]);
  *n_records = n;
  if (records && capacity > 0)
    std::memcpy(records, slot + 8, size_t(std::min(n, capacity)) * 8 * sizeof(double));
  return PQP_OK;
}

double
pqp_batch_last_solve_ms(const pqp_batch* h)
{
  if (h && h->solve_in_flight)
    (void)pqp_batch_wait(const_cast<pqp_batch*>(h));
  return h ? double(h->last_ms) : 0.0;
}

double
pqp_batch_last_prologue_ms(const pqp_batch* h)
{
  if (h && h->solve_in_flight)
    (void)pqp_batch_wait(const_cast<pqp_batch*>(h));
  return h ? double(h->last_prologue_ms) : 0.0;
}

int
pqp_batch_launch_config(const pqp_batch* h, int* threads, int64_t* lds_bytes)
{
  if (!h)
    return fail(PQP_ERR_INVALID_ARGUMENT, "null batch handle");
  const LaunchPlan p = pqp_plan_solve(h, 0, long(h->dev.B), nullptr);
  if (threads)
    *threads = p.threads;
  if (lds_bytes)
    *lds_bytes = int64_t(p.lds);
  return PQP_OK;
}

const char*
pqp_batch_last_kernel(const pqp_batch* h)
{
  return h ? h->last_kernel : "";
}

}
```

proxsuite_amd/csrc/pqp_dwave.hpp:

```cpp
#ifndef PQP_DWAVE_HPP
#define PQP_DWAVE_HPP

#include "pqp_diag.hpp"
#include <utility>

namespace pqp {

#ifndef PQP_DW_HB
#define PQP_DW_HB 2
#endif
#ifndef PQP_DW_SCHUR_LAZY
#define PQP_DW_SCHUR_LAZY 1
#endif
#ifndef PQP_DW_SCHUR_REG_BLOCKS
#define PQP_DW_SCHUR_REG_BLOCKS 8
#endif
constexpr int DW_SCHUR_REG_BLOCKS = PQP_DW_SCHUR_REG_BLOCKS;
constexpr int DW_MAXDIM = 128;

enum
{
  DLV_XP = 0,
  DLV_YP,
  DLV_ZP,
  DLV_GS,
  DLV_BS,
  DLV_US,
  DLV_LS,
  DLV_COUNT
};
constexpr int DW_SCR = 1024;
constexpr int DW_INTS = 128 + 128 + 256 + 256 + 2 * INCR_MAX;

__host__ __device__ inline size_t
dwave_lds_bytes()
{
  return (size_t)DW_INTS * sizeof(int) + (size_t)(DLV_COUNT * 128 + DW_SCR) * sizeof(double) + (ST_COUNT + 2) * sizeof(long long);
}

__host__ __device__ inline bool
dwave_signature(const Dims& d)
{
  return d.box == 0 && d.hessian == PQP_HESSIAN_DENSE && d.backend != PQP_BACKEND_PRIMAL_LDLT && d.n <= DW_MAXDIM &&
         d.n_eq <= DW_MAXDIM && d.n_in <= DW_MAXDIM && d.n >= 2;
}

struct DPair
{
  double x, y;
};
__device__ __forceinline__ DPair
dw_load_pair(cgptr p)
{
#ifndef PQP_EMULATED_MFMA
  typedef double pqp_d2u __attribute__((ext_vector_type(2), aligned(8)));
  const pqp_d2u t = *reinterpret_cast<const PQP_GLOBAL pqp_d2u*>(p);
  return DPair{ t.x, t.y };
#else
  return DPair{ p[0], p[1] };
#endif
}

template<bool LOW>
__device__ __forceinline__ DPair
dw_load_row(cgptr base, int off8, int nrec8, int col, int clo)
{
#ifndef PQP_EMULATED_MFMA
  typedef unsigned pqp_u4 __attribute__((ext_vector_type(4)));
  typedef double pqp_d2v __attribute__((ext_vector_type(2)));
  const __amdgpu_buffer_rsrc_t rs = __builtin_amdgcn_make_buffer_rsrc((void*)base, (short)0, nrec8, 0x00020000);
  int off = col * 8;
  if (LOW)
    off = (col + 1 >= clo) ? off : 0x7ffffff0;
  const pqp_u4 raw = __builtin_amdgcn_raw_buffer_load_b128(rs, off, off8, 0);
  const pqp_d2v t = __builtin_bit_cast(pqp_d2v, raw);
  return DPair{ t.x, t.y };
#else
  DPair r{ 0.0, 0.0 };
  auto in_range = [&](int c) {
    const long o = (long)off8 + 8L * c;
    return o >= 0 && o + 8 <= (long)nrec8;
  };
  if (!LOW || col + 1 >= clo) {
    if (in_range(col))
      r.x = base[((long)off8 + 8L * col) / 8];
    if (in_range(col + 1))
      r.y = base[((long)off8 + 8L * (col + 1)) / 8];
  }
  return r;
#endif
}

__device__ __forceinline__ void
dw_sched_fence()
{
#ifndef PQP_EMULATED_MFMA
  __builtin_amdgcn_sched_barrier(0);
#endif
}

__device__ __forceinline__ int
wave_bcast_i(int v, int src)
{
#ifndef PQP_EMULATED_MFMA
  return __builtin_amdgcn_readlane(v, src);
#else
  return __shfl(v, src);
#endif
}

#define DW_S(s) _Pragma("unroll") for (int s = 0; s < 2; ++s)
#define DW_B(b) _Pragma("unroll") for (int b = 0; b < 2; ++b)

struct DWave
{
  const Batch& batch;
  const long q;
  const Dims d;
  const QpRef P;
  const pqp_settings& st;
  UInfo info;
  const int lane;
  const int n, ne, ni, nd;
  PQP_LDS int* slot_of;
  PQP_LDS int* actl;
  PQP_LDS int* rowid;
  PQP_LDS int* sid;
  PQP_LDS int* chg;
  lptr lds_v;
  lptr scr;
  PQP_LDS long long* lds_stat;
  UD ruiz_c, dual_feasibility_rhs_2;
  int n_c, n_slots, r;
  bool schur_dirty, schur_incremental, aty_fresh, iterate_zero, nonfinite;
  double x[2], dx[2], dres[2], Hdx[2], ATdy[2], CTdz[2], CTzin[2], rx[2], ex[2], dF[2];
  double y[2], dy[2], se[2], Adx[2];
  double z[2], dz[2], Cdx[2], si[2], rup[2];
  int fl[2];
  double sd[2][2], rd[2][2], ed[2][2], dS[2][2];

  __device__ __forceinline__ DWave(const Batch& b, long q_, lptr lds)
    : batch(b)
    , q(uni(q_))
    , d(b.d)
    , P(b, uni(q_))
    , st(b.settings[uni(q_)])
    , lane((int)(threadIdx.x & (WAVE - 1)))
    , n(uni(b.d.n))
    , ne(uni(b.d.n_eq))
    , ni(uni(b.d.n_in))
    , nd(uni(b.d.nd))
  {
    PQP_LDS int* li = (PQP_LDS int*)lds;
    slot_of = li;
    actl = li + 128;
    rowid = li + 256;
    sid = li + 512;
    chg = li + 768;
    lds_v = (lptr)(li + DW_INTS);
    scr = lds_v + DLV_COUNT * 128;
    lds_stat = (PQP_LDS long long*)(scr + DW_SCR);
    n_c = 0;
    n_slots = 0;
    r = ne;
    schur_dirty = true;
    schur_incremental = false;
    aty_fresh = false;
    iterate_zero = false;
    nonfinite = false;
  }
  __device__ __forceinline__ int idx(int s) const { return 2 * lane + s; }
  __device__ __forceinline__ int didx(int b, int s) const { return 128 * b + 2 * lane + s; }
  __device__ __forceinline__ bool active(int s) const { return (fl[s] & 8) != 0; }
  __device__ __forceinline__ double lv(int V, int s) const { return lds_v[V * 128 + idx(s)]; }
  __device__ __forceinline__ void lv_set(int V, int s, double v) { lds_v[V * 128 + idx(s)] = v; }

  __device__ __forceinline__ void tic()
  {
#ifdef PQP_STATS
    if (lane == 0)
      lds_stat[ST_COUNT] = clock64();
#endif
  }
  __device__ __forceinline__ void toc(int which)
  {
#ifdef PQP_STATS
    if (lane == 0) {
      long long t = clock64();
      lds_stat[which] += t - lds_stat[ST_COUNT];
      lds_stat[ST_COUNT] = t;
    }
#else
    (void)which;
#endif
  }
  __device__ __forceinline__ void sub_tic(int which)
  {
#ifdef PQP_STATS
    if (lane == 0)
      lds_stat[which] -= clock64();
#else
    (void)which;
#endif
  }
  __device__ __forceinline__ void sub_toc(int which)
  {
#ifdef PQP_STATS
    if (lane == 0)
      lds_stat[which] += clock64();
#else
    (void)which;
#endif
  }
  __device__ __forceinline__ void count(int which, long long v = 1)
  {
#ifdef PQP_STATS
    if (lane == 0)
      lds_stat[which] += v;
#else
    (void)which;
    (void)v;
#endif
  }
  __device__ __forceinline__ void bytes(long long b) { count(ST_BYTES_ENGINE, b); }
  __device__ __forceinline__ void trace_line(double kind, double i, double a, double b, double c, double d4, double e)
  {
    if (batch.trace == nullptr || lane != 0)
      return;
    const int slot = batch.trace_slot[q];
    if (slot < 0)
      return;
    gptr t = (gptr)(batch.trace + (long)slot * batch.trace_cap * 8);
    const int k = (int)t[0];
    if (k + 1 >= batch.trace_cap) {
      t[1] += 1.0;
      return;
    }
    gptr rr = t + (long)(k + 1) * 8;
    rr[0] = kind;
    rr[1] = i;
    rr[2] = a;
    rr[3] = b;
    rr[4] = c;
    rr[5] = d4;
    rr[6] = e;
    t[0] = double(k + 1);
  }

  __device__ __forceinline__ void vload(double (&v)[2], cgptr src, int len, double fill = 0.0)
  {
    DW_S(s) v[s] = (idx(s) < len) ? src[idx(s)] : fill;
  }
  __device__ __forceinline__ void vstore(gptr dst, const double (&v)[2], int len)
  {
    DW_S(s) if (idx(s) < len) dst[idx(s)] = v[s];
  }
  __device__ __forceinline__ void vzero(double (&v)[2]) { DW_S(s) v[s] = 0.0; }
  __device__ __forceinline__ void vcopy(double (&a)[2], const double (&b)[2]) { DW_S(s) a[s] = b[s]; }
  __device__ __forceinline__ void dzero(double (&v)[2][2])
  {
    DW_B(b) DW_S(s) v[b][s] = 0.0;
  }
  __device__ __forceinline__ void lv_load(int V, cgptr src, int len, double fill = 0.0)
  {
    DW_S(s) lv_set(V, s, (idx(s) < len) ? src[idx(s)] : fill);
  }
  __device__ __forceinline__ void to_lds(lptr dst, const double (&v)[2]) const
  {
    DW_S(s) dst[idx(s)] = v[s];
  }
  __device__ __forceinline__ void to_lds2(lptr dst, const double (&v)[2][2]) const
  {
    DW_B(b) DW_S(s) dst[didx(b, s)] = v[b][s];
  }

  template<bool COLS, bool ROWS, int NCB, bool LOW>
  __device__ __forceinline__ void mat_pass_block(cgptr base, int kb, int t1, const int (&offv)[2], const int (&nrecv)[2],
                                                 const double (&cvec)[2], const double (&xop)[NCB][2], double (&cacc)[NCB][2],
                                                 lptr rout)
  {
    const int lo_t = 128 * kb;
    const int hi_t = (t1 < 128 * kb + 128) ? t1 : 128 * kb + 128;
    if (lo_t >= hi_t)
      return;
    const int lr = lane & 15, lk = lane >> 4;
    double acc2[NCB][2];
#pragma unroll
    for (int cb = 0; cb < NCB; ++cb) {
      acc2[cb][0] = 0.0;
      acc2[cb][1] = 0.0;
    }
    auto issue = [&](DPair(&v)[8][NCB], int tb) {
#pragma unroll
      for (int u = 0; u < 8; ++u) {
        const int t = tb + u;
        const int so = wave_bcast_i(offv[u & 1], (t & 127) >> 1);
        const int nr = wave_bcast_i(nrecv[u & 1], (t & 127) >> 1);
#pragma unroll
        for (int cb = 0; cb < NCB; ++cb)
          v[u][cb] = dw_load_row<LOW>(base, so, nr, 128 * cb + 2 * lane, t);
      }
    };
    auto consume = [&](const DPair(&v)[8][NCB], int tb, double* p8) {
#pragma unroll
      for (int u = 0; u < 8; ++u) {
        if (COLS) {
          const int t = tb + u;
          const double c = wave_bcast(cvec[u & 1], (t & 127) >> 1);
#pragma unroll
          for (int cb = 0; cb < NCB; ++cb) {
            if (u & 1) {
              acc2[cb][0] = fma(c, v[u][cb].x, acc2[cb][0]);
              acc2[cb][1] = fma(c, v[u][cb].y, acc2[cb][1]);
            } else {
              cacc[cb][0] = fma(c, v[u][cb].x, cacc[cb][0]);
              cacc[cb][1] = fma(c, v[u][cb].y, cacc[cb][1]);
            }
          }
        }
        if (ROWS) {
          double pv = 0.0;
#pragma unroll
          for (int cb = 0; cb < NCB; ++cb)
            pv = fma(v[u][cb].x, xop[cb][0], fma(v[u][cb].y, xop[cb][1], pv));
          p8[u] = pv;
        }
      }
    };
    auto reduce16 = [&](const double* p, int g) {
      pqp_d4 T;
#pragma unroll
      for (int k = 0; k < 4; ++k)
        T[k] = 0.0;
#pragma unroll
      for (int j = 0; j < 16; ++j)
        T = mfma_f64_16x16x4(p[j], (lr == j) ? 1.0 : 0.0, T);
      const double qv = (T[0] + T[1]) + (T[2] + T[3]);
      pqp_d4 T2;
#pragma unroll
      for (int k = 0; k < 4; ++k)
        T2[k] = 0.0;
      T2 = mfma_f64_16x16x4(qv, 1.0, T2);
      if (lr == 0) {
#pragma unroll
        for (int k = 0; k < 4; ++k) {
          const int t = g + lk + 4 * k;
          if (t < hi_t)
            rout[t] = T2[k];
        }
      }
    };
    constexpr int HB = (NCB == 1) ? PQP_DW_HB : 1;
    constexpr int GR = (HB >= 2) ? 8 * HB : 16;
    for (int g = lo_t; g < hi_t; g += GR) {
      double p[GR];
#pragma unroll
      for (int h0 = 0; h0 < GR; h0 += 8 * HB) {
        DPair v[HB][8][NCB];
#pragma unroll
        for (int hb = 0; hb < HB; ++hb)
          issue(v[hb], g + h0 + 8 * hb);
        dw_sched_fence();
#pragma unroll
        for (int hb = 0; hb < HB; ++hb)
          consume(v[hb], g + h0 + 8 * hb, p + h0 + 8 * hb);
      }
      if (ROWS) {
#pragma unroll
        for (int k = 0; k < GR; k += 16)
          if (g + k < hi_t)
            reduce16(p + k, g + k);
      }
    }
    if (COLS) {
#pragma unroll
      for (int cb = 0; cb < NCB; ++cb) {
        cacc[cb][0] += acc2[cb][0];
        cacc[cb][1] += acc2[cb][1];
      }
    }
  }
  struct Rows1
  {
    int off[2], nrec[2];
  };
  struct Rows2
  {
    int off[2][2], nrec[2][2];
  };
  __device__ __forceinline__ Rows1 rows_full(int stride, int len, int R) const
  {
    Rows1 w;
    DW_S(s)
    {
      w.off[s] = idx(s) * stride * 8;
      w.nrec[s] = (idx(s) < R) ? w.off[s] + len * 8 : 0;
    }
    return w;
  }
  __device__ __forceinline__ Rows1 rows_tril(int stride, int R) const
  {
    Rows1 w;
    DW_S(s)
    {
      w.off[s] = idx(s) * stride * 8;
      w.nrec[s] = (idx(s) < R) ? w.off[s] + (idx(s) + 1) * 8 : 0;
    }
    return w;
  }
  __device__ __forceinline__ Rows2 rows2_tril(int stride, int R) const
  {
    Rows2 w;
    DW_B(b) DW_S(s)
    {
      w.off[b][s] = didx(b, s) * stride * 8;
      w.nrec[b][s] = (didx(b, s) < R) ? w.off[b][s] + (didx(b, s) + 1) * 8 : 0;
    }
    return w;
  }
  __device__ __forceinline__ Rows1 rows_list(const int (&sel)[2], int stride, int len, int R) const
  {
    Rows1 w;
    DW_S(s)
    {
      w.off[s] = sel[s] * stride * 8;
      w.nrec[s] = (idx(s) < R) ? w.off[s] + len * 8 : 0;
    }
    return w;
  }
  __device__ __forceinline__ Rows2 rows2_list(const int (&sel)[2][2], int stride, int len, int R) const
  {
    Rows2 w;
    DW_B(b) DW_S(s)
    {
      w.off[b][s] = sel[b][s] * stride * 8;
      w.nrec[b][s] = (didx(b, s) < R) ? w.off[b][s] + len * 8 : 0;
    }
    return w;
  }
  template<bool COLS, bool ROWS, int NCB>
  __device__ __forceinline__ void mat_pass2(cgptr base, int t1, const Rows2& w, const double (&cvec)[2][2],
                                            const double (&xop)[NCB][2], double (&cacc)[NCB][2], lptr rout)
  {
    mat_pass_block<COLS, ROWS, NCB, false>(base, 0, t1, w.off[0], w.nrec[0], cvec[0], xop, cacc, rout);
    if (t1 > 128)
      mat_pass_block<COLS, ROWS, NCB, false>(base, 1, t1, w.off[1], w.nrec[1], cvec[1], xop, cacc, rout);
  }
  template<bool COLS, bool ROWS, int NCB, bool LOW = false>
  __device__ __forceinline__ void mat_pass1(cgptr base, int t1, const Rows1& w, const double (&cvec)[2],
                                            const double (&xop)[NCB][2], double (&cacc)[NCB][2], lptr rout)
  {
    mat_pass_block<COLS, ROWS, NCB, LOW>(base, 0, t1, w.off, w.nrec, cvec, xop, cacc, rout);
  }

  __device__ __forceinline__ void hess_mv(const double (&v)[2], double (&out)[2])
  {
    cgptr Hs = P.Hs();
    const int nn = n;
    double dg[2];
    DW_S(s) dg[s] = (idx(s) < nn) ? Hs[(unsigned)(idx(s) * (nn + 1))] : 0.0;
    double acc[1][2] = { { 0.0, 0.0 } };
    const double xop[1][2] = { { v[0], v[1] } };
    mat_pass1<true, true, 1>(Hs, nn, rows_tril(nn, nn), v, xop, acc, scr);
    __syncthreads();
    DW_S(s) out[s] = (idx(s) < nn) ? (acc[0][s] + scr[idx(s)]) - dg[s] * v[s] : 0.0;
    __syncthreads();
  }
  template<bool COLS, bool ROWS>
  __device__ __forceinline__ void dual_pass(cgptr M, int R, const double (&c)[2], const double (&xv)[2], double (&colout)[2],
                                            double (&rowout)[2])
  {
    const int nn = n;
    double acc[1][2] = { { 0.0, 0.0 } };
    const double xop[1][2] = { { xv[0], xv[1] } };
    mat_pass1<COLS, ROWS, 1>(M, R, rows_full(nn, nn, R), c, xop, acc, scr);
    if (COLS) {
      DW_S(s) colout[s] = (idx(s) < nn) ? acc[0][s] : 0.0;
    }
    if (ROWS) {
      __syncthreads();
      DW_S(s) rowout[s] = (idx(s) < R) ? scr[idx(s)] : 0.0;
      __syncthreads();
    }
  }

  __device__ __forceinline__ bool slot_live(int a) const
  {
    const int k = a - ne;
    if (k < 0)
      return true;
    return slot_of[actl[k]] == k;
  }
  __device__ __forceinline__ void zero_dead(double (&v)[2][2]) const
  {
    DW_B(b) DW_S(s)
    {
      const int a = didx(b, s);
      const bool live = (a < r) && slot_live(a < r ? a : 0);
      if (!live)
        v[b][s] = 0.0;
    }
  }
  __device__ __forceinline__ void build_rowid()
  {
    DW_B(b) DW_S(s)
    {
      const int a = didx(b, s);
      if (a < r)
        rowid[a] = (a < ne) ? a : ne + actl[a - ne];
    }
    __syncthreads();
  }

  __device__ __forceinline__ TilePair diag_tile_factor(int k0, int rr, lptr dSl, lptr tile, lptr dinv)
  {
    const int lr = lane & 15, lk = lane >> 4;
    TilePair Pm;
    const int nb = (rr - k0 < 16) ? (rr - k0) : 16;
    const int rw = lane & 15;
    double a[16];
#pragma unroll
    for (int c = 0; c < 16; ++c) {
      const double v = tile[rw * 16 + c];
      a[c] = (rw < nb && c < nb) ? v : ((rw == c) ? 1.0 : 0.0);
// ... 1372 lines not shown
        ATdy[k] /= sc;
        CTdz[k] /= sc;
        lb2 = vmax_abs(lb2, ATdy[k] + CTdz[k]);
        Hdx[k] /= sc;
        nhdx = vmax_abs(nhdx, Hdx[k]);
        gdx += dx[k] * lv(DLV_GS, k);
        dx[k] *= sx[k];
        ndx = vmax_abs(ndx, dx[k]);
      }
      DW_S(k) if (idx(k) < ne)
      {
        lb1 += dy[k] * lv(DLV_BS, k);
        dy[k] = dy[k] * sq[k] / c;
        nrm_dy = vmax_abs(nrm_dy, dy[k]);
        Adx[k] /= sq[k];
        nadx = vmax_abs(nadx, Adx[k]);
      }
      DW_S(k) if (idx(k) < ni)
      {
        const double v = dz[k];
        const double ubk = lv(DLV_US, k), lbk = lv(DLV_LS, k);
        lb1 += (v > 0 ? v : 0.0) * ubk;
        lb1 -= (v < 0 ? v : 0.0) * lbk;
        dz[k] = v * sc_[k] / c;
        nrm_dz = vmax_abs(nrm_dz, dz[k]);
        const double w = Cdx[k] / sc_[k];
        Cdx[k] = w;
        const double val = (ubk <= 1.E20 && lbk >= -1.E20) ? fabs(w) : ((ubk > 1.E20) ? -w : w);
        mviol = vmax(mviol, val);
      }
    }
    lb1 = lane_sum(lb1);
    gdx = lane_sum(gdx);
    nrm_dy = lane_max0(nrm_dy);
    nrm_dz = lane_max0(nrm_dz);
    lb2 = lane_max0(lb2);
    ndx = lane_max0(ndx);
    nadx = lane_max0(nadx);
    nhdx = lane_max0(nhdx);
    mviol = wave_max(mviol);
    e1 = lane_max0(e1);
    e2 = lane_max0(e2);
    e3 = lane_max0(e3);
    err_in = fmax(e1, fmax(e2, e3));
    primal_infeasible = false;
    dual_infeasible = false;
    if (!do_cert)
      return;
    {
      const double upper_bound = st.eps_primal_inf * fmax(nrm_dy, nrm_dz);
      primal_infeasible = (nrm_dy != 0 || nrm_dz != 0) && lb2 <= upper_bound && lb1 <= -upper_bound;
    }
    {
      double bound = ndx * st.eps_dual_inf;
      const bool first_cond = (nadx <= bound) && !(mviol > bound);
      bound *= c;
      const bool second_cond_alt1 = nhdx <= bound && gdx <= -bound;
      dual_infeasible = first_cond && second_cond_alt1 && ndx != 0;
    }
  }

  __device__ __forceinline__ void newton_semi_smooth(double eps_int, int mode)
  {
    bool refactorized = false;
    for (long iter = 0; iter <= st.max_iter_in; ++iter) {
      if (mode == 0 && iter == st.max_iter_in) {
        info.iter += st.max_iter_in + 1;
        break;
      }
      if (mode == 0)
        count(ST_N_NEWTON);
      const bool missed = linear_step(mode, eps_int);
      if (mode != 0)
        break;
      if (PQP_UNLIKELY(missed) && !refactorized) {
        schur_dirty = true;
        refactorized = true;
        count(ST_N_REFACTORIZE);
        --iter;
        continue;
      }
      refactorized = false;
      tic();
      if (st.merit_function_type == PQP_MERIT_GPDAL) {
        DW_S(c) Cdx[c] += (st.alpha_gpdal - 1.) * info.mu_in * dz[c];
      }
      UD alpha = 1.0;
      double dw_max = 0;
      if (ni > 0) {
        alpha = primal_dual_ls(dw_max);
      } else {
        DW_S(c)
        {
          dw_max = vmax_abs(dw_max, dx[c]);
          dw_max = vmax_abs(dw_max, dy[c]);
        }
        dw_max = lane_max0(dw_max);
      }
      toc(ST_CYC_LINESEARCH);
      sub_tic(ST_CYC_UPDATE);
      if (fabs(alpha) * dw_max < 1.E-11 && iter > 0) {
        info.iter += iter + 1;
        sub_toc(ST_CYC_UPDATE);
        break;
      }
      DW_S(c)
      {
        x[c] += alpha * dx[c];
        dres[c] += alpha * (info.rho * dx[c] + Hdx[c] + ATdy[c] + CTdz[c]);
        rup[c] += alpha * Cdx[c];
        si[c] += alpha * Cdx[c];
        z[c] += alpha * dz[c];
        se[c] += alpha * (Adx[c] - info.mu_eq * dy[c]);
        y[c] += alpha * dy[c];
      }
      sub_toc(ST_CYC_UPDATE);
      bool stop = false;
      UD err_in = 0.0;
      {
        sub_tic(ST_CYC_CERT);
        const bool do_cert = iter % st.frequence_infeasibility_check == 0 || st.primal_infeasibility_solving;
        bool is_primal_infeasible, is_dual_infeasible;
        double e;
        saddle_point_and_certificates(do_cert, e, is_primal_infeasible, is_dual_infeasible);
        err_in = e;
        if (PQP_UNLIKELY(st.verbose != 0))
          trace_line(2.0, double(iter + 1), e, alpha, 0.0, 0.0, 0.0);
        sub_toc(ST_CYC_CERT);
        if (PQP_UNLIKELY(is_primal_infeasible)) {
          info.status = PQP_PRIMAL_INFEASIBLE;
          if (!st.primal_infeasibility_solving) {
            info.iter += iter + 1;
            stop = true;
          }
        } else if (PQP_UNLIKELY(is_dual_infeasible)) {
          info.status = PQP_DUAL_INFEASIBLE;
          info.iter += iter + 1;
          stop = true;
        }
      }
      toc(ST_CYC_NEWTON_MISC);
      if (stop)
        break;
      if (err_in <= eps_int) {
        info.iter += iter + 1;
        break;
      }
      if (PQP_UNLIKELY(!(err_in == err_in))) {
        info.iter += iter + 1;
        nonfinite = true;
        break;
      }
    }
  }

  __device__ __forceinline__ void unscaled_cols(cgptr M, int R, const double (&c)[2], double (&out)[2])
  {
    const int nn = n;
    double acc[1][2] = { { 0.0, 0.0 } };
    const double xn[1][2] = { { 0.0, 0.0 } };
    mat_pass1<true, false, 1>(M, R, rows_full(nn, nn, R), c, xn, acc, scr);
    DW_S(s) out[s] = (idx(s) < nn) ? acc[0][s] : 0.0;
  }

  __device__ __forceinline__ void global_primal_residual(UD& lhs, UD& eq_rhs_0, UD& in_rhs_0, UD& eq_lhs, UD& in_lhs)
  {
    double m_eq0 = 0, m_in0 = 0, m_eql = 0, m_inl = 0;
    if (iterate_zero) {
      vzero(se);
      vzero(rup);
      vzero(ATdy);
      vzero(CTdz);
    } else {
      if (ne > 0)
        dual_pass<true, true>(P.As(), ne, y, x, ATdy, se);
      else {
        vzero(ATdy);
        vzero(se);
      }
      if (ni > 0)
        dual_pass<true, true>(P.Cs(), ni, z, x, CTdz, rup);
      else {
        vzero(CTdz);
        vzero(rup);
      }
      bytes(((long)ne * n + (long)ni * n) * 8);
    }
    aty_fresh = true;
    {
      cgptr de = P.dlt_eq(), bb = P.bvec(), di = P.dlt_in(), uu = P.u(), ll = P.l();
      double dev[2], bv[2], div_[2], uv[2], lwv[2];
      vload(dev, de, ne, 1.0);
      vload(bv, bb, ne);
      vload(div_, di, ni, 1.0);
      vload(uv, uu, ni);
      vload(lwv, ll, ni);
      DW_S(k) if (idx(k) < ne)
      {
        double v = se[k] / dev[k];
        m_eq0 = vmax_abs(m_eq0, v);
        v -= bv[k];
        m_eql = vmax_abs(m_eql, v);
        se[k] = v;
      }
      DW_S(k) if (idx(k) < ni)
      {
        const double v = rup[k] / div_[k];
        rup[k] = v;
        m_in0 = vmax_abs(m_in0, v);
        const double pu = v - uv[k], pl = v - lwv[k];
        const double sv = (pu > 0 ? pu : 0.0) + (pl < 0 ? pl : 0.0);
        si[k] = sv;
        m_inl = vmax_abs(m_inl, sv);
      }
      eq_rhs_0 = lane_max0(m_eq0);
      in_rhs_0 = lane_max0(m_in0);
      eq_lhs = lane_max0(m_eql);
      in_lhs = lane_max0(m_inl);
      lhs = fmax(eq_lhs, in_lhs);
      if (PQP_UNLIKELY(st.primal_infeasibility_solving && info.status == PQP_PRIMAL_INFEASIBLE)) {
        double t1[2], t2[2];
        vzero(t1);
        vzero(t2);
        if (ne > 0)
          unscaled_cols(P.A(), ne, se, t1);
        if (ni > 0)
          unscaled_cols(P.C(), ni, si, t2);
        double m = 0;
        DW_S(k) if (idx(k) < n) m = vmax_abs(m, t1[k] + t2[k]);
        lhs = lane_max0(m);
      }
      DW_S(k) if (idx(k) < ne) se[k] *= dev[k];
    }
  }

  __device__ __forceinline__ void global_dual_residual(UD& lhs, UD& rhs_0, UD& rhs_1, UD& rhs_3, UD& rhs_duality_gap,
                                                       UD& duality_gap)
  {
    const double c = ruiz_c;
    double m0 = 0, m1 = 0, m3 = 0, ml = 0, xHx = 0, gx = 0, by = 0, zu = 0, zl = 0;
    const double ib = 1.3407807929942596e+154;
    double hx[2];
    if (iterate_zero)
      vzero(hx);
    else
      hess_mv(x, hx);
    const bool have_products = aty_fresh;
    bytes(((iterate_zero ? 0L : (long)n * (n + 1) / 2) + (have_products ? 0L : (long)ne * n + (long)ni * n)) * 8);
    double aty[2], ctz[2];
    if (have_products) {
      vcopy(aty, ATdy);
      vcopy(ctz, CTdz);
    } else {
      double dummy[2];
      if (ne > 0)
        dual_pass<true, false>(P.As(), ne, y, x, aty, dummy);
      else
        vzero(aty);
      if (ni > 0)
        dual_pass<true, false>(P.Cs(), ni, z, x, ctz, dummy);
      else
        vzero(ctz);
    }
    {
      double sx[2], gv[2];
      vload(sx, P.dlt_x(), n, 1.0);
      vload(gv, P.g(), n);
      DW_S(k) if (idx(k) < n)
      {
        const double sc = sx[k] * c;
        const double v = hx[k] / sc;
        m0 = vmax_abs(m0, v);
        const double xu = x[k] * sx[k];
        xHx += v * xu;
        gx += gv[k] * xu;
        m1 = vmax_abs(m1, aty[k] / sc);
        m3 = vmax_abs(m3, ctz[k] / sc);
        const double dr = lv(DLV_GS, k) + hx[k] + aty[k] + ctz[k];
        dres[k] = dr;
        ml = vmax_abs(ml, dr / sc);
      }
    }
    {
      double dev[2], bv[2], div_[2], uv[2], lwv[2];
      vload(dev, P.dlt_eq(), ne, 1.0);
      vload(bv, P.bvec(), ne);
      vload(div_, P.dlt_in(), ni, 1.0);
      vload(uv, P.u(), ni);
      vload(lwv, P.l(), ni);
      DW_S(k) if (idx(k) < ne) by += bv[k] * (y[k] * dev[k] / c);
      DW_S(k) if (idx(k) < ni)
      {
        const double zi = z[k] * div_[k] / c;
        const double uk = uv[k] < ib ? uv[k] : ib;
        const double lk = lwv[k] > -ib ? lwv[k] : -ib;
        if (fl[k] & 1)
          zu += zi * uk;
        if (fl[k] & 2)
          zl += zi * lk;
      }
    }
    gx = lane_sum(gx);
    xHx = lane_sum(xHx);
    by = lane_sum(by);
    zu = lane_sum(zu);
    zl = lane_sum(zl);
    m0 = lane_max0(m0);
    m1 = lane_max0(m1);
    m3 = lane_max0(m3);
    ml = lane_max0(ml);
    rhs_0 = m0;
    rhs_1 = m1;
    rhs_3 = m3;
    lhs = ml;
    duality_gap = gx;
    rhs_duality_gap = fabs(gx);
    duality_gap += xHx;
    rhs_duality_gap = fmax(rhs_duality_gap, fabs(xHx));
    rhs_duality_gap = fmax(rhs_duality_gap, fabs(by));
    duality_gap += by;
    rhs_duality_gap = fmax(rhs_duality_gap, fabs(zu));
    duality_gap += zu;
    rhs_duality_gap = fmax(rhs_duality_gap, fabs(zl));
    duality_gap += zl;
  }

  __device__ __forceinline__ void solve()
  {
    State W = *P.state();
    info.load(*P.info());
    ruiz_c = W.ruiz_c;
    dual_feasibility_rhs_2 = W.dual_feasibility_rhs_2;
#ifdef PQP_STATS
    {
      const PQP_GLOBAL long long* gs0 = P.stats();
      for (int k = lane; k < ST_COUNT + 2; k += WAVE)
        lds_stat[k] = (k < ST_COUNT) ? gs0[k] : 0;
      __syncthreads();
    }
#endif
    const long long cyc0 = clock64();
    const long long wall0 = wall_clock64();
    DW_S(c)
    {
      dx[c] = dres[c] = Hdx[c] = ATdy[c] = CTdz[c] = CTzin[c] = rx[c] = ex[c] = 0.0;
      dy[c] = se[c] = Adx[c] = 0.0;
      dz[c] = Cdx[c] = si[c] = rup[c] = 0.0;
      lv_set(DLV_XP, c, 0.0);
      lv_set(DLV_YP, c, 0.0);
      lv_set(DLV_ZP, c, 0.0);
    }
    dzero(sd);
    dzero(rd);
    dzero(ed);
    DW_B(b) DW_S(s) dS[b][s] = 1.0;
    vload(x, P.x(), n);
    vload(y, P.y(), ne);
    vload(z, P.z(), ni);
    {
      const PQP_GLOBAL int* ga = P.act();
      DW_S(c)
      {
        fl[c] = (idx(c) < ni) ? act_flags(ga[idx(c) < ni ? idx(c) : 0]) : 0;
        slot_of[idx(c)] = -1;
        actl[idx(c)] = 0;
      }
    }
    __syncthreads();
    tic();
    const int ig = st.initial_guess;
    const bool wswpr = (ig == PQP_WARM_START_WITH_PREVIOUS_RESULT);
    const bool dirty = W.dirty != 0;
    bool do_factor, do_scale_ws, do_aset_from_z, do_eq_guess = false, do_restore = false;
    if (dirty) {
      if (ig == PQP_EQUALITY_CONSTRAINED_INITIAL_GUESS || ig == PQP_NO_INITIAL_GUESS) {
        vzero(x);
        vzero(y);
        vzero(z);
        cold_start(info, st);
      } else if (wswpr) {
        cleanup_statistics(info);
      } else {
        cold_start(info, st);
      }
    }
    if (ig == PQP_EQUALITY_CONSTRAINED_INITIAL_GUESS) {
      do_factor = true;
      do_scale_ws = false;
      do_aset_from_z = false;
      do_eq_guess = true;
    } else if (ig == PQP_NO_INITIAL_GUESS) {
      do_factor = true;
      do_scale_ws = false;
      do_aset_from_z = false;
    } else if (ig == PQP_COLD_START_WITH_PREVIOUS_RESULT || ig == PQP_WARM_START) {
      do_factor = true;
      do_scale_ws = true;
      do_aset_from_z = true;
    } else {
      do_scale_ws = true;
      if (!dirty && W.refactorize) {
        do_factor = true;
        do_aset_from_z = true;
      } else if (!W.factor_valid) {
        do_factor = true;
        do_aset_from_z = true;
      } else {
        do_factor = false;
        do_aset_from_z = false;
        do_restore = true;
      }
    }
    lv_load(DLV_GS, P.gs(), n);
    lv_load(DLV_BS, P.bs(), ne);
    lv_load(DLV_US, P.us(), ni);
    lv_load(DLV_LS, P.ls(), ni);
    if (do_scale_ws) {
      double sx[2], sq[2], sc_[2];
      vload(sx, P.dlt_x(), n, 1.0);
      vload(sq, P.dlt_eq(), ne, 1.0);
      vload(sc_, P.dlt_in(), ni, 1.0);
      DW_S(k)
      {
        x[k] /= sx[k];
        y[k] = y[k] / sq[k] * ruiz_c;
        z[k] = z[k] / sc_[k] * ruiz_c;
      }
    }
    vload(dF, P.dF(), n, 1.0);
    {
      const bool primal_kept = W.primal_valid != 0 && W.rho_fact == info.rho && !(dirty && !wswpr && W.scaled_valid == 0);
      W.primal_valid = (do_factor || primal_kept) ? 1 : 0;
    }
    if (do_factor) {
      n_c = 0;
      n_slots = 0;
      r = ne;
      schur_dirty = true;
    }
    if (do_restore) {
      n_c = W.n_c;
      n_slots = W.n_slots;
      r = ne + n_slots;
      {
        cgptr dSg = P.dS();
        DW_B(b) DW_S(s)
        {
          const int a = didx(b, s);
          dS[b][s] = (a < r) ? dSg[a] : 1.0;
        }
        const PQP_GLOBAL int* ga = P.act();
        DW_S(c)
        {
          const int j = idx(c);
          if (j < n_slots) {
            const int i = act_cid(ga[j]);
            actl[j] = (i >= 0) ? i : 0;
            if (i >= 0)
              slot_of[i] = j;
          }
        }
        __syncthreads();
        DW_S(c) if (idx(c) < ni && slot_of[idx(c)] >= 0) fl[c] |= 8;
      }
      build_rowid();
      schur_dirty = !(W.ls_valid && W.mu_eq_fact == info.mu_eq && W.mu_in_fact == info.mu_in);
      schur_incremental = W.ls_edited != 0;
    }
    bool pend = false;
    int pend_mode = 0;
    double pend_eps = 1.0;
    if (do_aset_from_z || do_eq_guess) {
      if (do_aset_from_z) {
        DW_S(c) fl[c] = (fl[c] & 11) | ((idx(c) < ni && z[c] != 0) ? 4 : 0);
      } else {
        DW_S(c) fl[c] = (fl[c] & 11);
      }
      pend = true;
      pend_mode = do_eq_guess ? 1 : 2;
    }

    const UD bcl_eta_ext_init = pow(0.1, st.alpha_bcl);
    UD bcl_eta_ext = bcl_eta_ext_init;
    UD bcl_eta_in = 1;
    const UD eps_in_min = fmin(st.eps_abs, 1.E-9);
    UD primal_feasibility_eq_rhs_0 = 0, primal_feasibility_in_rhs_0 = 0;
    UD dual_feasibility_rhs_0 = 0, dual_feasibility_rhs_1 = 0, dual_feasibility_rhs_3 = 0;
    UD primal_feasibility_lhs = 0, primal_feasibility_eq_lhs = 0, primal_feasibility_in_lhs = 0;
    UD dual_feasibility_lhs = 0;
    UD duality_gap = 0, rhs_duality_gap = 0;
    UD scaled_eps = st.eps_abs;
    UD primal_feasibility_lhs_new = 0, dual_feasibility_lhs_new = 0;
    UD new_bcl_mu_in = 0, new_bcl_mu_eq = 0, new_bcl_mu_in_inv = 0, new_bcl_mu_eq_inv = 0;
    bool is_primal_feasible = false, is_dual_feasible = false;
    long iter = 0;
    int stage = 0;
    bool done = (st.max_iter <= 0);
    bool gpr_fresh = false, gdr_fresh = false;
    aty_fresh = false;
    {
      double mz = 0;
      DW_S(k)
      {
        mz = vmax_abs(mz, x[k]);
        mz = vmax_abs(mz, y[k]);
        mz = vmax_abs(mz, z[k]);
      }
      iterate_zero = lane_max0(mz) == 0.0;
    }
    UD pl_cache = 0, dl_cache = 0;
    toc(ST_CYC_F_PANEL);
    for (;;) {
      if (pend) {
        newton_semi_smooth(pend_eps, pend_mode);
        pend = false;
        tic();
        if (pend_mode != 0) {
          double mz = 0;
          DW_S(k)
          {
            mz = vmax_abs(mz, x[k]);
            mz = vmax_abs(mz, y[k]);
            mz = vmax_abs(mz, z[k]);
          }
          iterate_zero = lane_max0(mz) == 0.0;
        } else {
          iterate_zero = false;
          gpr_fresh = false;
          gdr_fresh = false;
          aty_fresh = false;
          if (PQP_UNLIKELY(nonfinite)) {
            info.status = PQP_MAX_ITER_REACHED;
            break;
          }
          if ((info.status == PQP_PRIMAL_INFEASIBLE && !st.primal_infeasibility_solving) || info.status == PQP_DUAL_INFEASIBLE) {
            vcopy(x, dx);
            vcopy(y, dy);
            vcopy(z, dz);
            break;
          }
          if (PQP_UNLIKELY(scaled_eps == st.eps_abs && st.primal_infeasibility_solving && info.status == PQP_PRIMAL_INFEASIBLE)) {
            double one_e[2], one_i[2], t1[2], t2[2];
            DW_S(k)
            {
              one_e[k] = (idx(k) < ne) ? 1.0 : 0.0;
              one_i[k] = (idx(k) < ni) ? 1.0 : 0.0;
            }
            vzero(t1);
            vzero(t2);
            if (ne > 0)
              unscaled_cols(P.A(), ne, one_e, t1);
            if (ni > 0)
              unscaled_cols(P.C(), ni, one_i, t2);
            double m = 0;
            DW_S(k) if (idx(k) < n) m = vmax_abs(m, t1[k] + t2[k]);
            scaled_eps = lane_max0(m) * st.eps_abs;
          }
          stage = 1;
        }
      }
      if (done)
        break;
      tic();
      if (st.primal_infeasibility_solving)
        gpr_fresh = false;
      UD pl = pl_cache, dl = dl_cache;
      const bool want_primal = (stage != 2);
      const bool want_dual_pre = (stage != 1);
      if (want_primal && !gpr_fresh) {
        global_primal_residual(pl, primal_feasibility_eq_rhs_0, primal_feasibility_in_rhs_0, primal_feasibility_eq_lhs,
                               primal_feasibility_in_lhs);
        pl_cache = pl;
        gpr_fresh = true;
      }
      bool want_dual = want_dual_pre;
      if (stage == 1) {
        primal_feasibility_lhs_new = pl;
        is_primal_feasible = primal_feasibility_lhs_new <=
                             (scaled_eps + st.eps_rel * fmax(primal_feasibility_eq_rhs_0, primal_feasibility_in_rhs_0));
        info.pri_res = primal_feasibility_lhs_new;
        want_dual = is_primal_feasible;
      }
      if (want_dual && !gdr_fresh) {
        global_dual_residual(dl, dual_feasibility_rhs_0, dual_feasibility_rhs_1, dual_feasibility_rhs_3, rhs_duality_gap,
                             duality_gap);
        dl_cache = dl;
        gdr_fresh = true;
      }
      toc(ST_CYC_GLOBAL_RES);
      const UD rhs_dua_rel = st.eps_rel * fmax(fmax(dual_feasibility_rhs_3, dual_feasibility_rhs_0),
                                               fmax(dual_feasibility_rhs_1, dual_feasibility_rhs_2));
      if (stage == 0) {
        primal_feasibility_lhs = pl;
        dual_feasibility_lhs = dl;
        info.pri_res = primal_feasibility_lhs;
        info.dua_res = dual_feasibility_lhs;
        info.duality_gap = duality_gap;
        new_bcl_mu_in = info.mu_in;
        new_bcl_mu_eq = info.mu_eq;
        new_bcl_mu_in_inv = info.mu_in_inv;
        new_bcl_mu_eq_inv = info.mu_eq_inv;
        UD rhs_pri = scaled_eps;
        if (st.eps_rel != 0)
          rhs_pri += st.eps_rel * fmax(primal_feasibility_eq_rhs_0, primal_feasibility_in_rhs_0);
        is_primal_feasible = primal_feasibility_lhs <= rhs_pri;
        UD rhs_dua = st.eps_abs;
        if (st.eps_rel != 0)
          rhs_dua += rhs_dua_rel;
        is_dual_feasible = dual_feasibility_lhs <= rhs_dua;
        if (PQP_UNLIKELY(st.verbose != 0)) {
          trace_line(1.0, double(info.iter_ext + 1), info.pri_res, info.dua_res, info.duality_gap, info.mu_in, info.rho);
          double sx[2], sq[2], sc_[2];
          vload(sx, P.dlt_x(), n, 1.0);
          vload(sq, P.dlt_eq(), ne, 1.0);
          vload(sc_, P.dlt_in(), ni, 1.0);
          DW_S(k)
          {
            x[k] = (x[k] * sx[k]) / sx[k];
            y[k] = (y[k] * sq[k] / ruiz_c) / sq[k] * ruiz_c;
            z[k] = (z[k] * sc_[k] / ruiz_c) / sc_[k] * ruiz_c;
          }
        }
        if (is_primal_feasible && is_dual_feasible) {
          if (st.check_duality_gap) {
            if (fabs(info.duality_gap) <= st.eps_duality_gap_abs + st.eps_duality_gap_rel * rhs_duality_gap) {
              info.status = (st.primal_infeasibility_solving && info.status == PQP_PRIMAL_INFEASIBLE)
                              ? PQP_SOLVED_CLOSEST_PRIMAL_FEASIBLE
                              : PQP_SOLVED;
              break;
            }
          } else {
            info.status = PQP_SOLVED;
            break;
          }
        }
        info.iter_ext += 1;
        DW_S(c)
        {
          lv_set(DLV_XP, c, x[c]);
          lv_set(DLV_YP, c, y[c]);
          lv_set(DLV_ZP, c, z[c]);
        }
        {
          double sc_[2];
          vload(sc_, P.dlt_in(), ni, 1.0);
          DW_S(i) if (idx(i) < ni)
          {
            double v = rup[i] * sc_[i] + z[i] * info.mu_in;
            if (st.merit_function_type == PQP_MERIT_GPDAL)
              v += (st.alpha_gpdal - 1.) * info.mu_in * z[i];
            rup[i] = v - lv(DLV_US, i);
            si[i] = v - lv(DLV_LS, i);
          }
        }
        toc(ST_CYC_F_PANEL);
        pend = true;
        pend_mode = 0;
        pend_eps = bcl_eta_in;
        continue;
      }
      if (stage == 1) {
        if (is_primal_feasible) {
          dual_feasibility_lhs_new = dl;
          info.dua_res = dual_feasibility_lhs_new;
          info.duality_gap = duality_gap;
          is_dual_feasible = dual_feasibility_lhs_new <= (st.eps_abs + rhs_dua_rel);
          if (is_dual_feasible) {
            bool gap_ok = true;
            if (st.check_duality_gap)
              gap_ok = fabs(info.duality_gap) <= st.eps_duality_gap_abs + st.eps_duality_gap_rel * rhs_duality_gap;
            if (gap_ok)
              info.status = (st.primal_infeasibility_solving && info.status == PQP_PRIMAL_INFEASIBLE)
                              ? PQP_SOLVED_CLOSEST_PRIMAL_FEASIBLE
                              : PQP_SOLVED;
          }
        }
        if (st.bcl_update) {
          if (primal_feasibility_lhs_new <= bcl_eta_ext || info.iter > st.safe_guard) {
            bcl_eta_ext *= pow(info.mu_in, st.beta_bcl);
            bcl_eta_in = fmax(bcl_eta_in * info.mu_in, eps_in_min);
          } else {
            DW_S(c)
            {
              y[c] = lv(DLV_YP, c);
              z[c] = lv(DLV_ZP, c);
            }
            gdr_fresh = false;
            aty_fresh = false;
            new_bcl_mu_in = fmax(info.mu_in * st.mu_update_factor, st.mu_min_in);
            new_bcl_mu_eq = fmax(info.mu_eq * st.mu_update_factor, st.mu_min_eq);
            new_bcl_mu_in_inv = fmin(info.mu_in_inv * st.mu_update_inv_factor, st.mu_max_in_inv);
            new_bcl_mu_eq_inv = fmin(info.mu_eq_inv * st.mu_update_inv_factor, st.mu_max_eq_inv);
            bcl_eta_ext = bcl_eta_ext_init * pow(new_bcl_mu_in, st.alpha_bcl);
            bcl_eta_in = fmax(new_bcl_mu_in, eps_in_min);
          }
        } else {
          bcl_eta_in = fmax(bcl_eta_in * 0.1, eps_in_min);
          if (!(primal_feasibility_lhs_new <= 0.95 * primal_feasibility_lhs)) {
            new_bcl_mu_in = fmax(info.mu_in * st.mu_update_factor, st.mu_min_in);
            new_bcl_mu_eq = fmax(info.mu_eq * st.mu_update_factor, st.mu_min_eq);
            new_bcl_mu_in_inv = fmin(info.mu_in_inv * st.mu_update_inv_factor, st.mu_max_in_inv);
            new_bcl_mu_eq_inv = fmin(info.mu_eq_inv * st.mu_update_inv_factor, st.mu_max_eq_inv);
          }
        }
        stage = 2;
        continue;
      }
      dual_feasibility_lhs_new = dl;
      info.dua_res = dual_feasibility_lhs_new;
      info.duality_gap = duality_gap;
      if (primal_feasibility_lhs_new >= primal_feasibility_lhs && dual_feasibility_lhs_new >= dual_feasibility_lhs &&
          info.mu_in <= 1e-5) {
        new_bcl_mu_in = st.cold_reset_mu_in;
        new_bcl_mu_eq = st.cold_reset_mu_eq;
        new_bcl_mu_in_inv = st.cold_reset_mu_in_inv;
        new_bcl_mu_eq_inv = st.cold_reset_mu_eq_inv;
      }
      if (info.mu_in != new_bcl_mu_in || info.mu_eq != new_bcl_mu_eq) {
        ++info.mu_updates;
        if (ne + n_c > 0)
          schur_dirty = true;
      }
      info.mu_eq = new_bcl_mu_eq;
      info.mu_in = new_bcl_mu_in;
      info.mu_eq_inv = new_bcl_mu_eq_inv;
      info.mu_in_inv = new_bcl_mu_in_inv;
      stage = 0;
      ++iter;
      if (iter >= st.max_iter)
        done = true;
    }

    tic();
    {
      double sx[2], sq[2], sc_[2];
      vload(sx, P.dlt_x(), n, 1.0);
      vload(sq, P.dlt_eq(), ne, 1.0);
      vload(sc_, P.dlt_in(), ni, 1.0);
      DW_S(k)
      {
        x[k] *= sx[k];
        y[k] = y[k] * sq[k] / ruiz_c;
        z[k] = z[k] * sc_[k] / ruiz_c;
      }
      if (st.primal_infeasibility_solving && info.status == PQP_PRIMAL_INFEASIBLE) {
        DW_S(k)
        {
          se[k] /= sq[k];
          si[k] /= sc_[k];
        }
      }
    }
    {
      double hx[2], gv[2];
      unscaled_cols(P.H(), n, x, hx);
      bytes((long)n * n * 8);
      vload(gv, P.g(), n);
      double obj = 0;
      DW_S(k) if (idx(k) < n) obj += 0.5 * hx[k] * x[k] + gv[k] * x[k];
      info.objValue = lane_sum(obj);
    }
    vstore(P.x(), x, n);
    vstore(P.y(), y, ne);
    vstore(P.z(), z, ni);
    vstore(P.se(), se, ne);
    vstore(P.si(), si, ni);
    {
      gptr dSg = P.dS();
      DW_B(b) DW_S(s)
      {
        const int a = didx(b, s);
        if (a < nd)
          dSg[a] = dS[b][s];
      }
    }
    if (batch.hx) {
      vstore((gptr)(batch.hx + P.lq() * n), x, n);
      vstore((gptr)(batch.hy + P.lq() * ne), y, ne);
      vstore((gptr)(batch.hz + P.lq() * ni), z, ni);
      vstore((gptr)(batch.hse + P.lq() * ne), se, ne);
      vstore((gptr)(batch.hsi + P.lq() * ni), si, ni);
    }
    {
      PQP_GLOBAL int* ga = P.act();
      DW_S(c)
      {
        const int i = idx(c);
        if (i < ni)
          ga[i] = act_pack((i < n_slots && slot_live(ne + i)) ? actl[i] : -1, fl[c] & 3);
      }
    }
    toc(ST_CYC_F_TINV);
    if (lane == 0) {
      if (st.compute_timings) {
        info.solve_time = (double)(wall_clock64() - wall0) * batch.wall_us_per_tick;
        info.run_time = info.solve_time + info.setup_time;
      }
      info.store(*P.info());
      if (batch.hinfo)
        info.store(batch.hinfo[q]);
      W.dirty = 1;
      W.is_initialized = 1;
      W.n_c = n_c;
      W.n_slots = n_slots;
      W.factor_valid = 1;
      W.ls_valid = schur_dirty ? 0 : 1;
      W.ls_edited = schur_incremental ? 1 : 0;
      W.mu_eq_fact = info.mu_eq;
      W.mu_in_fact = info.mu_in;
      W.rho_fact = info.rho;
      *P.state() = W;
      PQP_GLOBAL long long* gs_ = P.stats();
#ifdef PQP_STATS
      for (int k = 0; k < ST_COUNT; ++k)
        gs_[k] = lds_stat[k];
#else
      for (int k = 0; k < ST_COUNT; ++k)
        gs_[k] = 0;
#endif
      gs_[ST_N_ACTIVE_FINAL] = n_c;
      gs_[ST_CYC_TOTAL] = clock64() - cyc0;
      gs_[ST_WALL_TICKS] = wall_clock64() - wall0;
    }
  }
};

#undef DW_S
#undef DW_B

__device__ __forceinline__ void
dwave_solve_body(const Batch& batch, long q, lptr lds)
{
  DWave S(batch, q, lds);
  S.solve();
}

}

#endif
```

proxsuite_amd/csrc/pqp_host.hpp:

```cpp
#ifndef PQP_HOST_HPP
#define PQP_HOST_HPP

#include <hip/hip_runtime.h>

#include <algorithm>
#include <cmath>
#include <cstdio>
#include <cstdlib>
#include <cstring>
#include <limits>
#include <string>
#include <vector>

#include "proxqp_hip.h"
#include "pqp_solver.hpp"

constexpr int PQP_MAX_ROWS = 8192;
static_assert(PQP_MAX_ROWS + 1 < (1 << 16), "act[] packs constraint ids into 16 bits");

int pqp_fail(int code, const std::string& msg);
#define fail pqp_fail

#define HIP_TRY(expr)                                                                               \
  do {                                                                                              \
    hipError_t e_ = (expr);                                                                         \
    if (e_ != hipSuccess)                                                                           \
      return pqp_fail(PQP_ERR_HIP, std::string(#expr) + ": " + hipGetErrorString(e_));              \
  } while (0)

struct pqp_batch
{
  pqp::Batch dev{};
  int device = 0;
  int n_cu = 256;
  int nt = 256;
  int backend = PQP_BACKEND_PRIMAL_DUAL_LDLT;
  size_t lds_solve = 0, lds_setup = 0;
  std::vector<pqp_settings> settings;
  std::vector<pqp_settings> settings_uploaded;
  std::vector<pqp_settings> cmd_settings;
  std::vector<pqp::Cmd> cmd;
  std::vector<char> is_initialized;
  std::vector<char> c_diag;
  bool settings_dirty = true;
  bool cmd_pending = false;
  pqp_settings* d_settings = nullptr;
  pqp::Cmd* d_cmd = nullptr;
  std::vector<void*> allocs;
  hipEvent_t ev0 = nullptr, ev1 = nullptr;
  hipEvent_t ev_mid = nullptr;
  bool prologue_timed = false;
  float last_prologue_ms = 0.f;
  float last_ms = 0.f;
  bool solve_in_flight = false;
  long flight_first = 0, flight_count = 0;
  std::vector<int64_t> flight_idx;
  bool host_results = false;
  std::vector<char> mirror_fresh;
  std::vector<void*> host_allocs;
  double *m_x = nullptr, *m_y = nullptr, *m_z = nullptr, *m_se = nullptr, *m_si = nullptr;
  pqp_info* m_info = nullptr;
  double* trace_dev = nullptr;
  int64_t trace_slots = 0;
  int* trace_slot_dev = nullptr;
  std::vector<int> trace_slot;
  std::vector<double> trace_host;
  hipStream_t stream = nullptr;
  hipStream_t owned_stream = nullptr;
  double* vec_scratch = nullptr;
  long range_first = 0, range_count = 0;
  const char* last_kernel = "";
  long setup_first = 0, setup_count = 0;
  const int* subset_order = nullptr;
  const std::vector<int>* subset_host = nullptr;
  struct Arr
  {
    char* base;
    size_t bytes_per_qp;
  };
  std::vector<Arr> per_qp;
  double *bw_dH = nullptr, *bw_dg = nullptr, *bw_dA = nullptr, *bw_db = nullptr, *bw_dC = nullptr,
         *bw_du = nullptr, *bw_dl = nullptr, *bw_ld = nullptr;
  bool lpt = false;
  bool order_valid = false;
  int* d_order = nullptr;
};

struct DeviceGuard
{
  int prev = -1;
  bool switched = false;
  bool failed = false;
  explicit DeviceGuard(int device)
  {
    if (hipGetDevice(&prev) != hipSuccess)
      failed = true;
    else if (prev != device) {
      switched = hipSetDevice(device) == hipSuccess;
      failed = !switched;
    }
  }
  bool ok() const { return !failed; }
  ~DeviceGuard()
  {
    if (switched)
      (void)hipSetDevice(prev);
  }
  DeviceGuard(const DeviceGuard&) = delete;
  DeviceGuard& operator=(const DeviceGuard&) = delete;
};
#define PQP_ON_DEVICE(dev)                                                                          \
  DeviceGuard guard_(dev);                                                                          \
  if (!guard_.ok())                                                                                 \
    return pqp_fail(PQP_ERR_HIP, "hipSetDevice(" + std::to_string(dev) + ") failed: the call did not run")

enum pqp_kernel : int
{
  PQP_K_256_4_1, PQP_K_256_3_1, PQP_K_256_2_1, PQP_K_256_1_1, PQP_K_256_3_0, PQP_K_256_1_0, PQP_K_256_2_2,
  PQP_K_DIAG_1, PQP_K_DIAG_2, PQP_K_DIAG_4, PQP_K_DWAVE,
  PQP_K_512_2_1, PQP_K_512_2_0, PQP_K_512_4_1, PQP_K_512_4_0, PQP_K_1024_1, PQP_K_1024_0, PQP_K_HBM_1, PQP_K_HBM_0,
  PQP_K_COUNT
};

struct LaunchPlan
{
  pqp_kernel kernel;
  int threads;
  size_t lds;
  bool prologue;
};

int pqp_launch_setup(pqp_batch* h);
LaunchPlan pqp_plan_solve(const pqp_batch* h, long first, long count, const std::vector<int>* subset);
int pqp_launch_solve(pqp_batch* h);
int pqp_launch_backward(pqp_batch* h, const pqp::BackwardArgs& bw, long count);
int pqp_launch_order(pqp_batch* h, long count);
int pqp_launch_pack(pqp_batch* h, long first, long count, double* out, hipStream_t stream);

#endif
```

proxsuite_amd/csrc/pqp_kernels.hip:

```cpp
#ifndef PQP_TU
#define PQP_TU 0
#endif
#if PQP_TU == 9
#define PQP_VECTORS_IN_HBM 1
#define PQP_LDS __attribute__((address_space(1)))
#define PQP_GLOBAL __attribute__((address_space(1)))
#endif
#if PQP_TU == 1 && !defined(PQP_GEMV_DEEP_256)
#define PQP_GEMV_DEEP_256 0
#endif
#if (PQP_TU == 1 || PQP_TU == 4 || PQP_TU == 8 || PQP_TU == 9) && !defined(PQP_ZG_DEPTH)
#define PQP_ZG_DEPTH 4
#endif
#if PQP_TU == 16 || PQP_TU == 17
#define PQP_OPAQUE_SCALAR(v)
#define PQP_OPAQUE_VECTOR(v)
#endif
#include "pqp_host.hpp"
#include "pqp_dwave.hpp"

#define PQP_TU_HAS(k) (PQP_TU == 0 || PQP_TU == (k))

#ifndef PQP_WPS_256_DENSE
#define PQP_WPS_256_DENSE 4
#endif
#ifndef PQP_WPS_256
#define PQP_WPS_256 3
#endif
#ifndef PQP_WPS_512
#define PQP_WPS_512 2
#endif
#ifndef PQP_WPS_512_DENSE
#define PQP_WPS_512_DENSE 4
#endif
#ifndef PQP_WPS_1024
#define PQP_WPS_1024 4
#endif

template<int NT, int WPS, int SPEC>
__global__ __launch_bounds__(NT, WPS) void
pqp_solve_kernel(pqp::Batch batch, long first, const int* __restrict__ order)
{
  HIP_DYNAMIC_SHARED(double, smem)
  const long slot = order ? (long)order[blockIdx.x] : (long)blockIdx.x;
  pqp::solve_body<NT, SPEC>(batch, first + slot, (pqp::lptr)smem);
}

template<int... A>
static std::string
kernel_label(const char* name)
{
  std::string s = std::string(name) + "<";
  ((s += std::to_string(A) + ","), ...);
  s.back() = '>';
  return s;
}

template<class K, class... Extra>
static int
enqueue(K* kernel, const std::string& label, pqp_batch* h, int threads, size_t lds, const int* order, bool prepare,
        Extra... extra)
{
  if (prepare) {
    if (lds > 64 * 1024)
      HIP_TRY(hipFuncSetAttribute(reinterpret_cast<const void*>(kernel), hipFuncAttributeMaxDynamicSharedMemorySize, (int)lds));
    return PQP_OK;
  }
  hipLaunchKernelGGL((kernel), dim3((unsigned)h->range_count), dim3(threads), lds, h->stream, h->dev, h->range_first,
                     order, extra...);
  HIP_TRY(hipGetLastError());
  h->last_kernel = label.c_str();
  return PQP_OK;
}

template<int NT, int WPS, int SPEC>
static int
enqueue_solve(pqp_batch* h, const LaunchPlan& p, const int* order, bool prepare)
{
  static const std::string label = kernel_label<NT, WPS, SPEC>("pqp_solve_kernel");
  return enqueue(&pqp_solve_kernel<NT, WPS, SPEC>, label, h, NT, p.lds, order, prepare);
}

using pqp_enqueue = int(pqp_batch* h, const LaunchPlan& p, const int* order, bool prepare);
pqp_enqueue pqp_enqueue_256_4_1, pqp_enqueue_256_3_1, pqp_enqueue_256_2_1, pqp_enqueue_256_1_1, pqp_enqueue_256_3_0,
  pqp_enqueue_256_1_0, pqp_enqueue_256_2_2, pqp_enqueue_diag_wave, pqp_enqueue_dense_wave, pqp_enqueue_prologue,
  pqp_enqueue_512_2, pqp_enqueue_512_4, pqp_enqueue_1024, pqp_enqueue_hbm;
#define PQP_SOLVE_ENTRY(name, NT, WPS, SPEC)                                                        \
  int name(pqp_batch* h, const LaunchPlan& p, const int* order, bool prepare) { return enqueue_solve<NT, WPS, SPEC>(h, p, order, prepare); }
#define PQP_SOLVE_ENTRY_1_0(name, NT, WPS, K_SPEC_1)  \
  int name(pqp_batch* h, const LaunchPlan& p, const int* order, bool prepare)                       \
  {                                                                                                 \
    return p.kernel == K_SPEC_1 ? enqueue_solve<NT, WPS, 1>(h, p, order, prepare) : enqueue_solve<NT, WPS, 0>(h, p, order, prepare); \
  }

#if PQP_TU_HAS(1)
PQP_SOLVE_ENTRY(pqp_enqueue_256_4_1, 256, PQP_WPS_256_DENSE, 1)
#endif
#if PQP_TU_HAS(7)
PQP_SOLVE_ENTRY(pqp_enqueue_256_3_1, 256, PQP_WPS_256, 1)
#endif
#if PQP_TU_HAS(13)
PQP_SOLVE_ENTRY(pqp_enqueue_256_1_1, 256, 1, 1)
#endif
#if PQP_TU_HAS(15)
PQP_SOLVE_ENTRY(pqp_enqueue_256_2_1, 256, 2, 1)
#endif
#if PQP_TU_HAS(14)
PQP_SOLVE_ENTRY(pqp_enqueue_256_1_0, 256, 1, 0)
#endif
#if PQP_TU_HAS(2)
PQP_SOLVE_ENTRY(pqp_enqueue_256_3_0, 256, PQP_WPS_256, 0)
#endif
#ifndef PQP_WPS_256_DIAG
#define PQP_WPS_256_DIAG 2
#endif
#if PQP_TU_HAS(12)
PQP_SOLVE_ENTRY(pqp_enqueue_256_2_2, 256, PQP_WPS_256_DIAG, 2)
#endif
#if PQP_TU_HAS(16)
#ifndef PQP_WPS_DIAG_WAVE
#define PQP_WPS_DIAG_WAVE 2
#endif
template<int E, int WPS>
__global__ __launch_bounds__(64, WPS) void
pqp_diag_kernel(pqp::Batch batch, long first, const int* __restrict__ order)
{
  HIP_DYNAMIC_SHARED(double, smem)
  const long slot = order ? (long)order[blockIdx.x] : (long)blockIdx.x;
  pqp::diag_solve_body<E>(batch, first + slot, (pqp::lptr)smem);
}

template<int E>
static int
enqueue_diag(pqp_batch* h, const LaunchPlan& p, const int* order, bool prepare)
{
  static const std::string label = kernel_label<E, PQP_WPS_DIAG_WAVE>("pqp_diag_kernel");
  return enqueue(&pqp_diag_kernel<E, PQP_WPS_DIAG_WAVE>, label, h, 64, p.lds, order, prepare);
}

int
pqp_enqueue_diag_wave(pqp_batch* h, const LaunchPlan& p, const int* order, bool prepare)
{
  switch (p.kernel) {
    case PQP_K_DIAG_1:
      return enqueue_diag<1>(h, p, order, prepare);
    case PQP_K_DIAG_2:
      return enqueue_diag<2>(h, p, order, prepare);
    default:
      return enqueue_diag<4>(h, p, order, prepare);
  }
}
#endif
#if PQP_TU_HAS(18)
template<int NT>
__global__ __launch_bounds__(NT, 4) void
pqp_prologue_kernel(pqp::Batch batch, long first, const int* __restrict__ order)
{
  HIP_DYNAMIC_SHARED(double, smem)
  const long slot = order ? (long)order[blockIdx.x] : (long)blockIdx.x;
  pqp::Solver<NT, 1> S(batch, first + slot, (pqp::lptr)smem);
  S.prologue();
}

int
pqp_enqueue_prologue(pqp_batch* h, const LaunchPlan&, const int* order, bool prepare)
{
  static const std::string label = kernel_label<256>("pqp_prologue_kernel");
  return enqueue(&pqp_prologue_kernel<256>, label, h, 256, h->lds_solve, order, prepare);
}
#endif
#if PQP_TU_HAS(17)
#ifndef PQP_WPS_DENSE_WAVE
#define PQP_WPS_DENSE_WAVE 2
#endif
template<int WPS>
__global__ __launch_bounds__(64, WPS) void
pqp_dwave_kernel(pqp::Batch batch, long first, const int* __restrict__ order)
{
  HIP_DYNAMIC_SHARED(double, smem)
  const long slot = order ? (long)order[blockIdx.x] : (long)blockIdx.x;
  pqp::dwave_solve_body(batch, first + slot, (pqp::lptr)smem);
}

int
pqp_enqueue_dense_wave(pqp_batch* h, const LaunchPlan& p, const int* order, bool prepare)
{
  static const std::string label = kernel_label<PQP_WPS_DENSE_WAVE>("pqp_dwave_kernel");
  return enqueue(&pqp_dwave_kernel<PQP_WPS_DENSE_WAVE>, label, h, 64, p.lds, order, prepare);
}
#endif
#if PQP_TU_HAS(3)
PQP_SOLVE_ENTRY_1_0(pqp_enqueue_512_2, 512, PQP_WPS_512, PQP_K_512_2_1)
#endif
#if PQP_TU_HAS(8)
PQP_SOLVE_ENTRY_1_0(pqp_enqueue_512_4, 512, PQP_WPS_512_DENSE, PQP_K_512_4_1)
#endif
#if PQP_TU_HAS(4)
PQP_SOLVE_ENTRY_1_0(pqp_enqueue_1024, 1024, PQP_WPS_1024, PQP_K_1024_1)
#endif

#if PQP_TU == 9 || (PQP_TU == 0 && defined(PQP_EMULATED_MFMA))
template<int NT, int WPS, int SPEC>
__global__ __launch_bounds__(NT, WPS) void
pqp_solve_hbm_kernel(pqp::Batch batch, long first, const int* __restrict__ order, double* scratch, long stride)
{
  const long slot = order ? (long)order[blockIdx.x] : (long)blockIdx.x;
  pqp::solve_body<NT, SPEC>(batch, first + slot, (pqp::lptr)(scratch + (long)blockIdx.x * stride));
}

template<int SPEC>
static int
enqueue_hbm(pqp_batch* h, const LaunchPlan& p, const int* order, bool prepare)
{
  static const std::string label = kernel_label<1024, PQP_WPS_1024, SPEC>("pqp_solve_hbm_kernel");
  return enqueue(&pqp_solve_hbm_kernel<1024, PQP_WPS_1024, SPEC>, label, h, 1024, 0, order, prepare, h->vec_scratch,
                 (long)((p.lds + 7) / 8));
}

int
pqp_enqueue_hbm(pqp_batch* h, const LaunchPlan& p, const int* order, bool prepare)
{
  return p.kernel == PQP_K_HBM_1 ? enqueue_hbm<1>(h, p, order, prepare) : enqueue_hbm<0>(h, p, order, prepare);
}
#endif

#if PQP_TU_HAS(5)
template<int NT>
__global__ __launch_bounds__(NT, 2) void
pqp_backward_kernel(pqp::Batch batch, pqp::BackwardArgs bw)
{
  HIP_DYNAMIC_SHARED(double, smem)
  pqp::backward_body<NT>(batch, bw, (long)blockIdx.x, (pqp::lptr)smem);
}

template<int NT>
static int
launch_backward(pqp_batch* h, const pqp::BackwardArgs& bw, long count)
{
  if (h->lds_solve > 64 * 1024)
    HIP_TRY(hipFuncSetAttribute(reinterpret_cast<const void*>(&pqp_backward_kernel<NT>),
                                hipFuncAttributeMaxDynamicSharedMemorySize, (int)h->lds_solve));
  hipLaunchKernelGGL((pqp_backward_kernel<NT>), dim3((unsigned)count), dim3(NT), h->lds_solve, h->stream,
                     h->dev, bw);
  HIP_TRY(hipGetLastError());
  return PQP_OK;
}

int
pqp_launch_backward(pqp_batch* h, const pqp::BackwardArgs& bw, long count)
{
  switch (h->nt) {
    case 256:
      return launch_backward<256>(h, bw, count);
    case 512:
      return launch_backward<512>(h, bw, count);
    default:
      return launch_backward<1024>(h, bw, count);
  }
}
#endif

#if PQP_TU_HAS(6)
template<int NT>
__global__ __launch_bounds__(NT) void
pqp_setup_kernel(pqp::Batch batch, long first)
{
  HIP_DYNAMIC_SHARED(double, smem)
  pqp::setup_body<NT>(batch, first + (long)blockIdx.x, (pqp::lptr)smem);
}

__global__ __launch_bounds__(64) void
pqp_order_kernel(const long long* __restrict__ stats, int stride, int B, int* __restrict__ order)
{
  constexpr int TILE = 4096;
  __shared__ unsigned tile[TILE];
  const int i = blockIdx.x * blockDim.x + threadIdx.x;
  const long long raw = (i < B) ? stats[(long)i * stride] : 0;
  const unsigned ci = raw > 0xffffffffll ? 0xffffffffu : (raw < 0 ? 0u : (unsigned)raw);
  int rank = 0;
  for (int j0 = 0; j0 < B; j0 += TILE) {
    const int cnt = (B - j0 < TILE) ? (B - j0) : TILE;
    __syncthreads();
    for (int t = threadIdx.x; t < cnt; t += blockDim.x) {
      const long long r = stats[(long)(j0 + t) * stride];
      tile[t] = r > 0xffffffffll ? 0xffffffffu : (r < 0 ? 0u : (unsigned)r);
    }
    __syncthreads();
    const int split = (i - j0 < 0) ? 0 : ((i - j0 < cnt) ? (i - j0) : cnt);
    for (int t = 0; t < split; ++t)
      rank += (tile[t] >= ci) ? 1 : 0;
    for (int t = split; t < cnt; ++t)
      rank += (tile[t] > ci) ? 1 : 0;
  }
  if (i < B)
    order[rank] = i;
}

template<int NT>
static int
launch_setup(pqp_batch* h)
{
  if (h->lds_setup > 64 * 1024)
    HIP_TRY(hipFuncSetAttribute(reinterpret_cast<const void*>(&pqp_setup_kernel<NT>),
                                hipFuncAttributeMaxDynamicSharedMemorySize, (int)h->lds_setup));
  hipLaunchKernelGGL((pqp_setup_kernel<NT>), dim3((unsigned)h->setup_count), dim3(NT), h->lds_setup, h->stream,
                     h->dev, h->setup_first);
  HIP_TRY(hipGetLastError());
  return PQP_OK;
}

int
pqp_launch_setup(pqp_batch* h)
{
  switch (h->nt) {
    case 256:
      return launch_setup<256>(h);
    case 512:
      return launch_setup<512>(h);
    default:
      return launch_setup<1024>(h);
  }
}

int
pqp_launch_order(pqp_batch* h, long count)
{
  hipLaunchKernelGGL((pqp_order_kernel), dim3((unsigned)((count + 63) / 64)), dim3(64), 0, h->stream,
                     reinterpret_cast<const long long*>(h->dev.stats), (int)pqp::ST_COUNT, (int)count, h->d_order);
  HIP_TRY(hipGetLastError());
  return PQP_OK;
}

__global__ __launch_bounds__(256) void
pqp_pack_kernel(pqp::Batch batch, long first, long count, double* __restrict__ out)
{
  const int n = batch.d.n, ne = batch.d.n_eq, nc = batch.d.nc;
  const long width = (long)n + ne + nc + 2;
  const long total = count * width;
  for (long o = (long)blockIdx.x * blockDim.x + threadIdx.x; o < total; o += (long)gridDim.x * blockDim.x) {
    const long i = o / width;
    const int k = (int)(o - i * width);
    const long q = first + i;
    double v;
    if (k < n)
      v = batch.x[q * n + k];
    else if (k < n + ne)
      v = batch.y[q * ne + (k - n)];
    else if (k < n + ne + nc)
      v = batch.z[q * nc + (k - n - ne)];
    else if (k == n + ne + nc)
      v = (double)batch.info[q].status;
    else
      v = (double)batch.info[q].iter;
    out[o] = v;
  }
}

int
pqp_launch_pack(pqp_batch* h, long first, long count, double* out, hipStream_t stream)
{
  const long width = (long)h->dev.d.n + h->dev.d.n_eq + h->dev.d.nc + 2;
  long blocks = (count * width + 255) / 256;
  if (blocks > 4096)
    blocks = 4096;
  if (blocks < 1)
    blocks = 1;
  hipLaunchKernelGGL((pqp_pack_kernel), dim3((unsigned)blocks), dim3(256), 0, stream, h->dev, first, count, out);
  HIP_TRY(hipGetLastError());
  return PQP_OK;
}

static bool
diag_structure(const pqp_batch* h, long first, long count, const std::vector<int>* subset)
{
  const pqp::Dims& dd = h->dev.d;
  if (!pqp::diag_structure_signature(dd.hessian, dd.n_eq, dd.n_in, dd.box) || h->c_diag.empty())
    return false;
  if (subset)
    return std::all_of(subset->begin(), subset->end(), [&](int q) { return h->c_diag[size_t(q)] != 0; });
  const size_t hi = std::min(h->c_diag.size(), size_t(first + count));
  return std::all_of(h->c_diag.begin() + std::min(size_t(first), hi), h->c_diag.begin() + hi, [](char c) { return c != 0; });
}

static bool
dense_wave(const pqp_batch* h, long count)
{
  if (!pqp::dwave_signature(h->dev.d))
    return false;
  const char* e = std::getenv("PQP_DENSE_KERNEL");
  if (e && e[0] == 'w' && e[1] == 'o')
    return false;
  if (e && e[0] == 'w' && e[1] == 'a')
    return true;
  const long round = 8L * h->n_cu, rem = count % round;
  if (count < 64)
    return false;
  if (count < round)
    return 5 * count >= 3 * round;
  return rem == 0 || 5 * rem >= 2 * round;
}

LaunchPlan
pqp_plan_solve(const pqp_batch* h, long first, long count, const std::vector<int>* subset)
{
  const pqp::Dims& dd = h->dev.d;
  const bool common = dd.box == 0 && dd.hessian == PQP_HESSIAN_DENSE && dd.backend != PQP_BACKEND_PRIMAL_LDLT;
  const long n_cu = h->n_cu;
  const auto workgroup = [h](pqp_kernel k) { return LaunchPlan{ k, h->nt, h->lds_solve, false }; };
  if (h->vec_scratch)
    return workgroup(common ? PQP_K_HBM_1 : PQP_K_HBM_0);
  switch (h->nt) {
    case 256:
      if (!common) {
        if (diag_structure(h, first, count, subset)) {
          const char* e = std::getenv("PQP_DIAG_KERNEL");
          if ((e && e[0] == 'w') || dd.n > 256)
            return workgroup(PQP_K_256_2_2);
          const int slots = dd.n <= 64 ? 1 : (dd.n <= 128 ? 2 : 4);
          return LaunchPlan{ slots == 1 ? PQP_K_DIAG_1 : (slots == 2 ? PQP_K_DIAG_2 : PQP_K_DIAG_4), 64,
                             pqp::diag_lds_bytes(slots), false };
        }
        return workgroup(count <= n_cu ? PQP_K_256_1_0 : PQP_K_256_3_0);
      }
      if (dense_wave(h, count))
        return LaunchPlan{ PQP_K_DWAVE, 64, pqp::dwave_lds_bytes(), true };
      if (count > 3 * n_cu && 4 * h->lds_solve <= 160 * 1024)
        return workgroup(PQP_K_256_4_1);
      if (count <= n_cu)
        return workgroup(PQP_K_256_1_1);
      return workgroup(count <= 2 * n_cu ? PQP_K_256_2_1 : PQP_K_256_3_1);
    case 512:
      if (count > n_cu && 2 * h->lds_solve <= 160 * 1024)
        return workgroup(common ? PQP_K_512_4_1 : PQP_K_512_4_0);
      return workgroup(common ? PQP_K_512_2_1 : PQP_K_512_2_0);
    default:
      return workgroup(common ? PQP_K_1024_1 : PQP_K_1024_0);
  }
}

static pqp_enqueue* const ENTRY_OF[PQP_K_COUNT] = {
  pqp_enqueue_256_4_1, pqp_enqueue_256_3_1, pqp_enqueue_256_2_1, pqp_enqueue_256_1_1, pqp_enqueue_256_3_0, pqp_enqueue_256_1_0,
  pqp_enqueue_256_2_2, pqp_enqueue_diag_wave, pqp_enqueue_diag_wave, pqp_enqueue_diag_wave, pqp_enqueue_dense_wave,
  pqp_enqueue_512_2, pqp_enqueue_512_2, pqp_enqueue_512_4, pqp_enqueue_512_4, pqp_enqueue_1024, pqp_enqueue_1024,
  pqp_enqueue_hbm, pqp_enqueue_hbm
};

int
pqp_launch_solve(pqp_batch* h)
{
  const LaunchPlan p = pqp_plan_solve(h, h->range_first, h->range_count, h->subset_host);
  const char* reuse = std::getenv("PQP_PRIMAL_REUSE");
  h->dev.primal_reuse = (reuse && reuse[0] == '0') ? 0 : 1;
  const bool whole = h->range_first == 0 && h->range_count == h->dev.B;
  const int* order = h->subset_order ? h->subset_order : ((h->lpt && h->order_valid && whole) ? h->d_order : nullptr);
  h->prologue_timed = false;
  if (p.prologue)
    if (int rc = pqp_enqueue_prologue(h, p, order, true))
      return rc;
  if (int rc = ENTRY_OF[p.kernel](h, p, order, true))
    return rc;
  HIP_TRY(hipEventRecord(h->ev0, h->stream));
  if (p.prologue) {
    if (int rc = pqp_enqueue_prologue(h, p, order, false))
      return rc;
    HIP_TRY(hipEventRecord(h->ev_mid, h->stream));
    h->prologue_timed = true;
  }
  if (int rc = ENTRY_OF[p.kernel](h, p, order, false))
    return rc;
  HIP_TRY(hipEventRecord(h->ev1, h->stream));
  return PQP_OK;
}
#endif
```

proxsuite_amd/csrc/pqp_solver.hpp:

```cpp
#ifndef PQP_SOLVER_HPP
#define PQP_SOLVER_HPP

#include "pqp_block.hpp"
#include "pqp_types.h"

namespace pqp {

#define PQP_UNLIKELY(x) __builtin_expect(!!(x), 0)
#define PQP_LIKELY(x) __builtin_expect(!!(x), 1)

constexpr double MACHINE_EPS = 2.220446049250313e-16;
#ifndef PQP_ZG_DEPTH
#define PQP_ZG_DEPTH 8
#endif
constexpr int ZG_DEPTH = PQP_ZG_DEPTH;
#ifndef PQP_LS_UNROLL
#define PQP_LS_UNROLL 4
#endif
#ifndef PQP_LS_BRACKET
#define PQP_LS_BRACKET 1
#endif
#ifndef PQP_ZG_BLOCK2
#define PQP_ZG_BLOCK2 1
#endif
// ... 13 lines not shown
incr_max(int r)
{
#ifndef PQP_INCR_DIV
#define PQP_INCR_DIV 10
#endif
  const int v = r / PQP_INCR_DIV;
  return v < PQP_INCR_BASE ? (PQP_INCR_BASE < INCR_MAX ? PQP_INCR_BASE : INCR_MAX) : (v > INCR_MAX ? INCR_MAX : v);
}

#ifndef PQP_CHUNK_ALL
#define PQP_CHUNK_ALL 0
#endif
constexpr int MAX_ROWS = 4096;
static_assert(MAX_ROWS + 1 < (1 << 16), "act[] packs constraint ids into 16 bits");
__host__ __device__ inline int
act_pack(int cid, int flags)
{
  return (cid + 1) | ((flags & 3) << 16);
}
__host__ __device__ inline int
act_cid(int packed)
{
  return (packed & 0xffff) - 1;
}
__host__ __device__ inline int
act_flags(int packed)
{
  return (packed >> 16) & 3;
}

__host__ __device__ inline bool
diag_structure_signature(int hessian, int n_eq, int n_in, int box)
{
  return hessian != PQP_HESSIAN_DENSE && n_eq == 0 && !(n_in > 0 && box != 0);
}

struct Dims
{
  int n, n_eq, n_in;
  int nc;
  int nd;
  int ntot;
  int box;
  int hessian;
  int backend;
  int _pad;
};

enum
{
  CMD_NONE = 0,
  CMD_INIT = 1,
  CMD_UPDATE = 2,
  CMD_CLEANUP = 3
};
struct Cmd
{
  int op;
  int preconditioner;
  int matrices_given;
  int _pad;
  double rho, mu_eq, mu_in, min_eig;
};

struct State
{
  int dirty;
  int refactorize;
  int proximal_parameter_update;
  int is_initialized;
  int n_c;
  int factor_valid;
  int ls_valid;
  int n_slots;
  int c_diag;
  int ls_edited;
  int scaled_valid;
  int primal_valid;
  double ruiz_c;
  double dual_feasibility_rhs_2;
  double correction_guess_rhs_g;
  double mu_eq_fact, mu_in_fact, rho_fact;
};

enum
{
  ST_CYC_TOTAL = 0,
  ST_CYC_SCALE,
  ST_CYC_FACTOR_H,
  ST_CYC_ZG,
  ST_CYC_SCHUR,
  ST_CYC_KKT_SOLVE,
  ST_CYC_RESIDUAL,
  ST_CYC_LINESEARCH,
  ST_CYC_GLOBAL_RES,
  ST_CYC_NEWTON_MISC,
  ST_N_NEWTON,
  ST_N_SCHUR_FACT,
  ST_N_NEW_ROWS,
  ST_N_KKT_SOLVES,
  ST_N_LS_BREAKPOINTS,
  ST_N_ACTIVE_FINAL,
  ST_CYC_F_LOAD,
  ST_CYC_F_UPDATE,
  ST_CYC_F_PANEL,
  ST_CYC_F_WRITEBACK,
  ST_CYC_F_TINV,
  ST_CYC_S_GATHER,
  ST_CYC_SOLVE_LDLT,
  ST_N_SCHUR_BLOCKED,
  ST_N_APPEND,
  ST_N_DELETE,
  ST_BYTES_ENGINE,
  ST_N_REFACTORIZE,
  ST_CYC_LS_EVAL,
  ST_CYC_CERT,
  ST_CYC_UPDATE,
  ST_WALL_TICKS,
  ST_FLOPS_FACT,
  ST_COUNT
};

struct Batch
{
  Dims d;
  long B;
  double *H, *g, *A, *b, *C, *u, *l, *u_box, *l_box;
  double *Hs, *gs, *As, *ATs, *bs, *Cs, *CTs, *us, *ls, *ubs, *lbs, *is;
  double* delta;
  double *x, *y, *z, *se, *si;
  pqp_info* info;
  const pqp_settings* settings;
  State* state;
  const Cmd* cmd;
  double *F;
  double *WL, *WU;
  double *dF;
  double *Zr;
  double *Zc;
  double *G;
  double *WS;
  double *LS;
  double *dS;
  int* act;
  long long* stats;
  double wall_us_per_tick;
  int rep_phase, rep_count;
  double *hx, *hy, *hz, *hse, *hsi;
  pqp_info* hinfo;
  double* trace;
  const int* trace_slot;
  int trace_cap;
  int primal_reuse;
};

struct BackwardArgs
{
  const double* ld;
  double eps, rho_new, mu_new;
  double *dL_dH, *dL_dg, *dL_dA, *dL_db, *dL_dC, *dL_du, *dL_dl;
  long first;
  const int* order;
};

#ifndef PQP_VECTORS_IN_HBM
#define PQP_VECTORS_IN_HBM 0
#endif
#define ZG_LDS_TILED(nt) ((nt) >= 512 && !PQP_VECTORS_IN_HBM)
template<int NT>
struct Lds
{
  static constexpr int SH = ZG_LDS_TILED(NT) ? 2 : 0;
  static constexpr int DF = ZG_LDS_TILED(NT) ? 0 : 14;
  lptr base;
  int n, ne, nc, ni, nd, tmax, nt, plen;
  int o_ne, o_nc, o_ni, o_nd, o_t2;
  __device__ __forceinline__ lptr at(int off) const
  {
    PQP_OPAQUE_VECTOR(off);
    return base + off;
  }
#define PQP_LVEC(name, cls_off, len, slot) \
  __device__ __forceinline__ lptr name() const { return at((cls_off) + (slot) * (len)); }
  PQP_LVEC(dF, 0, n, DF)
  PQP_LVEC(t1, 0, n, DF + 1)
  PQP_LVEC(x, 0, n, SH + 0)
  PQP_LVEC(xp, 0, n, SH + 1)
  PQP_LVEC(gs, 0, n, SH + 2)
  PQP_LVEC(ubs, 0, n, SH + 3)
  PQP_LVEC(lbs, 0, n, SH + 4)
  PQP_LVEC(isc, 0, n, SH + 5)
  PQP_LVEC(dx, 0, n, SH + 6)
  PQP_LVEC(rx, 0, n, SH + 7)
  PQP_LVEC(ex, 0, n, SH + 8)
  PQP_LVEC(Hdx, 0, n, SH + 9)
  PQP_LVEC(ATdy, 0, n, SH + 10)
  PQP_LVEC(CTdz, 0, n, SH + 11)
  PQP_LVEC(CTzin, 0, n, SH + 12)
  PQP_LVEC(dres, 0, n, SH + 13)
  PQP_LVEC(y, o_ne, ne, 0)
  PQP_LVEC(yp, o_ne, ne, 1)
  PQP_LVEC(bs, o_ne, ne, 2)
  PQP_LVEC(dy, o_ne, ne, 3)
  PQP_LVEC(Adx, o_ne, ne, 4)
  PQP_LVEC(se, o_ne, ne, 5)
  PQP_LVEC(z, o_nc, nc, 0)
  PQP_LVEC(zp, o_nc, nc, 1)
  PQP_LVEC(dz, o_nc, nc, 2)
  PQP_LVEC(Cdx, o_nc, nc, 3)
  PQP_LVEC(si, o_nc, nc, 4)
  PQP_LVEC(rup, o_nc, nc, 5)
  PQP_LVEC(zfull, o_nc, nc, 6)
  PQP_LVEC(us, o_ni, ni, 0)
  PQP_LVEC(ls, o_ni, ni, 1)
  PQP_LVEC(rd, o_nd, nd, 0)
  PQP_LVEC(ed, o_nd, nd, 1)
  PQP_LVEC(sd, o_nd, nd, 2)
  PQP_LVEC(dS, o_nd, nd, 3)
#undef PQP_LVEC
  __device__ __forceinline__ lptr stage() const { return at(2 * n); }
  __device__ __forceinline__ int part_len() const { return plen; }
  __device__ __forceinline__ int red_len() const { return 2 * RED_VALS * (nt / WAVE) + 8; }
  __device__ __forceinline__ lptr t2() const { return at(o_t2); }
  __device__ __forceinline__ lptr part() const { return at(o_t2 + tmax); }
  __device__ __forceinline__ lptr red() const { return at(o_t2 + tmax + part_len()); }
  __device__ __forceinline__ lptr top() const { return at(o_t2 + tmax + part_len() + red_len()); }
  __device__ __forceinline__ PQP_LDS long long* stat() const
  {
    return (PQP_LDS long long*)at(o_t2 + tmax + part_len() + red_len() + TOP_DOUBLES + PARK_DOUBLES);
  }
  __device__ __forceinline__ lptr park() const { return at(o_t2 + tmax + part_len() + red_len() + TOP_DOUBLES); }
  __device__ __forceinline__ liptr ints(int off) const
  {
    liptr q = (liptr)(base + (o_t2 + tmax + part_len() + red_len() + TOP_DOUBLES + PARK_DOUBLES + ST_COUNT + 1));
    PQP_OPAQUE_VECTOR(off);
    return q + off;
  }
  __device__ __forceinline__ liptr slot_of() const { return ints(0); }
  __device__ __forceinline__ liptr act() const { return ints(nc); }
  __device__ __forceinline__ liptr iscr() const { return ints(2 * nc); }
  __device__ __forceinline__ liptr aflags() const { return ints(2 * nc + nd); }
  __device__ __forceinline__ liptr icnt() const { return ints(3 * nc + nd); }
  __device__ __forceinline__ liptr chg() const { return ints(3 * nc + nd + nt / WAVE + 16); }
};

__host__ __device__ inline int
part_doubles(int nt, int tmax, int n)
{
  const int a = gemv_part_len(nt, tmax);
  const int b = gemv_dual_part_len(nt, n);
  return a > b ? a : b;
}

__host__ __device__ inline int
lds_part_len(int n, int ne, int nc, int ni, int nd, int nt)
{
  const int tmax = nd > n ? nd : n;
  const int need = part_doubles(nt, tmax, n);
  const int behind_t1 = 14 * n + 6 * ne + 7 * nc + 2 * ni + 4 * nd + tmax;
  const int pad = ZG_LDS_TILED(nt) ? zg_stage_doubles(nt) - behind_t1 : 0;
  return need > pad ? need : pad;
}

__host__ __device__ inline size_t
lds_doubles(const Dims& d, int nt)
{
  size_t n = d.n, ne = d.n_eq, nc = d.nc, nd = d.nd;
  size_t tmax = nd > n ? nd : n;
  size_t s = 0;
  s += 2 * (n + ne + nc);
  s += n + ne + 2 * d.n_in + 3 * n;
  s += n + ne + nc;
  s += 2 * (n + nd);
  s += nd;
  s += n + ne + nc + 3 * n;
  s += n + ne + 2 * nc;
  s += n + nd;
  s += n + tmax + nc;
  s += lds_part_len(d.n, d.n_eq, d.nc, d.n_in, d.nd, nt);
  s += 2 * RED_VALS * (nt / WAVE) + 8;
  s += TOP_DOUBLES;
  s += PARK_DOUBLES;
  s += ST_COUNT + 1;
  return s;
}
__host__ __device__ inline size_t
lds_bytes(const Dims& d, int nt)
{
  size_t ints = (size_t)d.nc * 3 + d.nd + nt / WAVE + 16 + 2 * INCR_MAX;
  return lds_doubles(d, nt) * sizeof(double) + ints * sizeof(int) + 64;
}

template<int NT>
__device__ __forceinline__ void
lds_carve(Lds<NT>& L, lptr base, const Dims& d, int nt)
{
  L.base = base;
  L.n = uni(d.n);
  L.ne = uni(d.n_eq);
  L.nc = uni(d.nc);
  L.ni = uni(d.n_in);
  L.nd = uni(d.nd);
  L.tmax = uni(d.nd > d.n ? d.nd : d.n);
  L.nt = nt;
  L.plen = uni(lds_part_len(d.n, d.n_eq, d.nc, d.n_in, d.nd, nt));
  L.o_ne = uni(16 * L.n);
// ... 4043 lines not shown
```

Baseline: 325,400 QPs/s.

## Checkpoint straggler dense-wave QPs and resume them in a tail kernel

Adds a tail mechanism to the dense-wave solver. When the number of unfinished QPs drops below a threshold (about 2 per CU by default), each still-running wave saves its register vectors, scalar state and LDS block to a global checkpoint slot and exits. A second kernel with occupancy 1 and a different unroll factor then resumes those stragglers. The aim is to reduce tail latency from long-running QPs that occupy the GPU at low occupancy. It also adds an optional deferred-reduction variant of the matvec loop, tail timing events and API getters, at the cost of an extra launch, atomics on a control counter, and checkpoint memory traffic.

```diff
diff --git a/include/proxqp_hip.h b/include/proxqp_hip.h
--- a/include/proxqp_hip.h
+++ b/include/proxqp_hip.h
@@ -107,6 +107,8 @@
 
 double pqp_batch_last_solve_ms(const pqp_batch* h);
 double pqp_batch_last_prologue_ms(const pqp_batch* h);
+int64_t pqp_batch_last_tail_count(const pqp_batch* h);
+double pqp_batch_last_tail_ms(const pqp_batch* h);
 int pqp_batch_launch_config(const pqp_batch* h, int* threads, int64_t* lds_bytes);
 const char* pqp_batch_last_kernel(const pqp_batch* h);
 
diff --git a/proxsuite_amd/_build.py b/proxsuite_amd/_build.py
--- a/proxsuite_amd/_build.py
+++ b/proxsuite_amd/_build.py
@@ -38,7 +38,7 @@
     return RANDQP_LIB
 
 
-KERNEL_TUS = (1, 2, 3, 4, 5, 6, 7, 8, 9, 12, 13, 14, 15, 16, 17, 18)
+KERNEL_TUS = (1, 2, 3, 4, 5, 6, 7, 8, 9, 12, 13, 14, 15, 16, 17, 18, 19)
 OBJ_DIR = ROOT / "build" / "obj"
 
 
@@ -52,6 +52,7 @@
 
 CODEGEN_FLAGS = ["-mllvm", "-sink-insts-to-avoid-spills", "-mllvm", "-disable-machine-licm"]
 TU_FLAGS = {17: ["-mllvm", "-disable-lsr"],
+            19: ["-mllvm", "-disable-lsr"],
             18: ["-mllvm", "-disable-lsr", "-DPQP_ZG_DEPTH=4"],
             1: ["-mllvm", "-disable-lsr"], 4: ["-mllvm", "-disable-lsr"], 7: ["-mllvm", "-disable-lsr"], 13: ["-mllvm", "-disable-lsr"], 15: ["-mllvm", "-disable-lsr"]}
 
@@ -128,7 +129,7 @@
     odir = OBJ_DIR / tag
     odir.mkdir(parents=True, exist_ok=True)
     common = hip_headers() + [Path(__file__)]
-    only = {"pqp_dwave.hpp": ("kernels_17.o", "kernels_6.o")}
+    only = {"pqp_dwave.hpp": ("kernels_17.o", "kernels_19.o", "kernels_6.o")}
     def deps_of(o):
         return [h for h in common if h.name not in only or o.name in only[h.name]] + [CSRC / HOST_OBJECTS.get(o.name, "pqp_kernels.hip")]
     def compile_object(o):
diff --git a/proxsuite_amd/_native.py b/proxsuite_amd/_native.py
--- a/proxsuite_amd/_native.py
+++ b/proxsuite_amd/_native.py
@@ -45,7 +45,7 @@
                "pqp_batch_update", "pqp_batch_warm_start", "pqp_batch_cleanup", "pqp_batch_reset_qp", "pqp_batch_flush",
                "pqp_batch_solve", "pqp_batch_solve_range", "pqp_batch_solve_subset", "pqp_batch_copy_qp", "pqp_batch_set_stream", "pqp_batch_set_schedule", "pqp_batch_backward", "pqp_batch_backward_range",
                "pqp_batch_get_backward", "pqp_batch_get_results", "pqp_batch_result_device_ptrs", "pqp_batch_pack_results",
-               "pqp_batch_get_scaled", "pqp_batch_get_schur_factor", "pqp_batch_get_primal_factor", "pqp_batch_get_stats", "pqp_batch_get_trace", "pqp_batch_last_solve_ms", "pqp_batch_last_prologue_ms",
+               "pqp_batch_get_scaled", "pqp_batch_get_schur_factor", "pqp_batch_get_primal_factor", "pqp_batch_get_stats", "pqp_batch_get_trace", "pqp_batch_last_solve_ms", "pqp_batch_last_prologue_ms", "pqp_batch_last_tail_ms", "pqp_batch_last_tail_count",
                "pqp_batch_launch_config", "pqp_batch_last_kernel", "pqp_batch_solve_async", "pqp_batch_solve_range_async",
                "pqp_batch_solve_subset_async", "pqp_batch_wait", "pqp_batch_enable_host_results",
                "pqp_batch_host_results", "pqp_batch_host_results_fresh", "pqp_batch_own_stream", "pqp_batch_backward_subset",
@@ -98,6 +98,10 @@
         L.pqp_batch_last_solve_ms.restype = C.c_double
         L.pqp_batch_last_prologue_ms.argtypes = [vp]
         L.pqp_batch_last_prologue_ms.restype = C.c_double
+        L.pqp_batch_last_tail_ms.argtypes = [vp]
+        L.pqp_batch_last_tail_ms.restype = C.c_double
+        L.pqp_batch_last_tail_count.argtypes = [vp]
+        L.pqp_batch_last_tail_count.restype = C.c_int64
         L.pqp_batch_launch_config.argtypes = [vp, C.POINTER(C.c_int), C.POINTER(C.c_int64)]
         L.pqp_batch_last_kernel.argtypes = [vp]
         L.pqp_batch_last_kernel.restype = C.c_char_p
@@ -401,6 +405,14 @@
     def last_prologue_ms(self):
         return self.lib.L.pqp_batch_last_prologue_ms(self._h)
 
+    @property
+    def last_tail_ms(self):
+        return self.lib.L.pqp_batch_last_tail_ms(self._h)
+
+    @property
+    def last_tail_count(self):
+        return int(self.lib.L.pqp_batch_last_tail_count(self._h))
+
     def results(self, idx=-1):
         pre = (self.B,) if idx < 0 else ()
         x = np.zeros(pre + (self.n,))
diff --git a/proxsuite_amd/csrc/pqp_capi.hip b/proxsuite_amd/csrc/pqp_capi.hip
--- a/proxsuite_amd/csrc/pqp_capi.hip
+++ b/proxsuite_amd/csrc/pqp_capi.hip
@@ -413,6 +413,7 @@
   HIP_TRY(hipEventCreate(&h->ev0));
   HIP_TRY(hipEventCreate(&h->ev1));
   HIP_TRY(hipEventCreate(&h->ev_mid));
+  HIP_TRY(hipEventCreate(&h->ev_tail));
   *out = h;
   return PQP_OK;
 }
@@ -440,6 +441,8 @@
     (void)hipEventDestroy(h->ev1);
   if (h->ev_mid)
     (void)hipEventDestroy(h->ev_mid);
+  if (h->ev_tail)
+    (void)hipEventDestroy(h->ev_tail);
   delete h;
 }
 
@@ -900,6 +903,12 @@
   h->last_prologue_ms = 0.f;
   if (h->prologue_timed)
     HIP_TRY(hipEventElapsedTime(&h->last_prologue_ms, h->ev0, h->ev_mid));
+  h->last_tail_ms = 0.f;
+  h->last_tail_count = 0;
+  if (h->tail_timed) {
+    HIP_TRY(hipEventElapsedTime(&h->last_tail_ms, h->ev_tail, h->ev1));
+    h->last_tail_count = *h->tail_resumed;
+  }
   return finish_solve(h);
 }
 
@@ -1447,6 +1456,22 @@
   return h ? double(h->last_prologue_ms) : 0.0;
 }
 
+double
+pqp_batch_last_tail_ms(const pqp_batch* h)
+{
+  if (h && h->solve_in_flight)
+    (void)pqp_batch_wait(const_cast<pqp_batch*>(h));
+  return h ? double(h->last_tail_ms) : 0.0;
+}
+
+int64_t
+pqp_batch_last_tail_count(const pqp_batch* h)
+{
+  if (h && h->solve_in_flight)
+    (void)pqp_batch_wait(const_cast<pqp_batch*>(h));
+  return h ? int64_t(h->last_tail_count) : 0;
+}
+
 int
 pqp_batch_launch_config(const pqp_batch* h, int* threads, int64_t* lds_bytes)
 {
diff --git a/proxsuite_amd/csrc/pqp_dwave.hpp b/proxsuite_amd/csrc/pqp_dwave.hpp
--- a/proxsuite_amd/csrc/pqp_dwave.hpp
+++ b/proxsuite_amd/csrc/pqp_dwave.hpp
@@ -44,6 +44,45 @@
   return d.box == 0 && d.hessian == PQP_HESSIAN_DENSE && d.backend != PQP_BACKEND_PRIMAL_LDLT && d.n <= DW_MAXDIM &&
          d.n_eq <= DW_MAXDIM && d.n_in <= DW_MAXDIM && d.n >= 2;
 }
+
+enum
+{
+  DW_HEAD = 0,
+  DW_TAIL = 1
+};
+
+struct DwCkptHead
+{
+  pqp_info info;
+  State W;
+  double ruiz_c, dual_feasibility_rhs_2;
+  double bcl_eta_ext_init, bcl_eta_ext, bcl_eta_in, eps_in_min;
+  double primal_feasibility_eq_rhs_0, primal_feasibility_in_rhs_0, dual_feasibility_rhs_0, dual_feasibility_rhs_1,
+    dual_feasibility_rhs_3, primal_feasibility_lhs, primal_feasibility_eq_lhs, primal_feasibility_in_lhs, dual_feasibility_lhs,
+    duality_gap, rhs_duality_gap, scaled_eps, primal_feasibility_lhs_new, dual_feasibility_lhs_new, new_bcl_mu_in,
+    new_bcl_mu_eq, new_bcl_mu_in_inv, new_bcl_mu_eq_inv, pend_eps;
+  long long cyc0, wall0;
+  long iter;
+  int n_c, n_slots, r;
+  int flags;
+};
+enum
+{
+  DWF_SCHUR_DIRTY = 1,
+  DWF_SCHUR_INCREMENTAL = 2,
+  DWF_NONFINITE = 4,
+  DWF_DONE = 8
+};
+constexpr int DW_CKPT_HEAD = 128;
+constexpr int DW_CKPT_LANE = 16 + 4 + 1;
+static_assert(sizeof(DwCkptHead) <= DW_CKPT_HEAD * sizeof(double), "checkpoint header");
+
+__host__ __device__ inline size_t
+dwave_ckpt_doubles()
+{
+  return (size_t)DW_CKPT_HEAD + (size_t)DW_CKPT_LANE * 64 + dwave_lds_bytes() / 8;
+}
+static_assert((DW_INTS % 2) == 0, "the LDS block is copied in 8-byte words");
 
 struct DPair
 {
@@ -112,6 +151,7 @@
 #define DW_S(s) _Pragma("unroll") for (int s = 0; s < 2; ++s)
 #define DW_B(b) _Pragma("unroll") for (int b = 0; b < 2; ++b)
 
+template<int ROLE, int HB_, bool DEFER>
 struct DWave
 {
   const Batch& batch;
@@ -350,26 +390,64 @@
         }
       }
     };
-    constexpr int HB = (NCB == 1) ? PQP_DW_HB : 1;
+    constexpr int HB = (NCB == 1) ? HB_ : 1;
     constexpr int GR = (HB >= 2) ? 8 * HB : 16;
-    for (int g = lo_t; g < hi_t; g += GR) {
-      double p[GR];
-#pragma unroll
-      for (int h0 = 0; h0 < GR; h0 += 8 * HB) {
-        DPair v[HB][8][NCB];
-#pragma unroll
-        for (int hb = 0; hb < HB; ++hb)
-          issue(v[hb], g + h0 + 8 * hb);
-        dw_sched_fence();
-#pragma unroll
-        for (int hb = 0; hb < HB; ++hb)
-          consume(v[hb], g + h0 + 8 * hb, p + h0 + 8 * hb);
-      }
-      if (ROWS) {
+    if constexpr (!(DEFER && ROWS)) {
+      for (int g = lo_t; g < hi_t; g += GR) {
+        double p[GR];
+#pragma unroll
+        for (int h0 = 0; h0 < GR; h0 += 8 * HB) {
+          DPair v[HB][8][NCB];
+#pragma unroll
+          for (int hb = 0; hb < HB; ++hb)
+            issue(v[hb], g + h0 + 8 * hb);
+          dw_sched_fence();
+#pragma unroll
+          for (int hb = 0; hb < HB; ++hb)
+            consume(v[hb], g + h0 + 8 * hb, p + h0 + 8 * hb);
+        }
+        if (ROWS) {
+#pragma unroll
+          for (int k = 0; k < GR; k += 16)
+            if (g + k < hi_t)
+              reduce16(p + k, g + k);
+        }
+      }
+    } else {
+      double pp[GR];
+#pragma unroll
+      for (int k = 0; k < GR; ++k)
+        pp[k] = 0.0;
+      for (int g = lo_t; g < hi_t; g += GR) {
+        double p[GR];
+#pragma unroll
+        for (int h0 = 0; h0 < GR; h0 += 8 * HB) {
+          DPair v[HB][8][NCB];
+#pragma unroll
+          for (int hb = 0; hb < HB; ++hb)
+            issue(v[hb], g + h0 + 8 * hb);
+          dw_sched_fence();
+          if (h0 == 0 && g > lo_t) {
+#pragma unroll
+            for (int k = 0; k < GR; k += 16)
+              if (g - GR + k < hi_t)
+                reduce16(pp + k, g - GR + k);
+            dw_sched_fence();
+          }
+#pragma unroll
+          for (int hb = 0; hb < HB; ++hb)
+            consume(v[hb], g + h0 + 8 * hb, p + h0 + 8 * hb);
+        }
+#pragma unroll
+        for (int k = 0; k < GR; ++k)
+          pp[k] = p[k];
+      }
+      {
+        const int gl = lo_t + ((hi_t - lo_t - 1) / GR) * GR;
 #pragma unroll
         for (int k = 0; k < GR; k += 16)
-          if (g + k < hi_t)
-            reduce16(p + k, g + k);
+          if (gl + k < hi_t)
+            reduce16(pp + k, gl + k);
       }
     }
     if (COLS) {
@@ -2048,6 +2126,70 @@
         break;
       }
     }
+  }
+
+  __device__ __forceinline__ int yield_slot(const DwTail& tl)
+  {
+    bool y = false;
+    if (tl.yield_at > 0) {
+      y = info.iter + 1 >= (long)tl.yield_at;
+    } else if (tl.T > 0) {
+      int rem = 0;
+      if (lane == 0)
+        rem = atomicAdd(tl.ctl, 0);
+      y = wave_bcast_i(rem, 0) <= tl.T;
+    }
+    if (!y)
+      return -1;
+    int slot = 0;
+    if (lane == 0)
+      slot = atomicAdd(tl.ctl + 1, 1);
+    slot = wave_bcast_i(slot, 0);
+    return slot < tl.cap ? slot : -1;
+  }
+  template<class F>
+  __device__ __forceinline__ void each_vector(F&& f)
+  {
+    int k = 0;
+    auto one = [&](double(&v)[2]) __attribute__((always_inline)) {
+      f(k, v[0]);
+      f(k + 1, v[1]);
+      k += 2;
+    };
+    one(x), one(dres), one(dF), one(y), one(se), one(z), one(si), one(rup), one(dS[0]), one(dS[1]);
+  }
+  __device__ __forceinline__ gptr ckpt(const DwTail& tl, int slot) const { return (gptr)(tl.rec + (size_t)slot * dwave_ckpt_doubles()); }
+  __device__ __forceinline__ DwCkptHead* ckpt_head(const DwTail& tl, int slot) const
+  {
+    return (DwCkptHead*)(tl.rec + (size_t)slot * dwave_ckpt_doubles());
+  }
+  __device__ __forceinline__ void save_vectors(gptr rec)
+  {
+    gptr v = rec + DW_CKPT_HEAD;
+    each_vector([&](int k, double& val) __attribute__((always_inline)) { v[k * 64 + lane] = val; });
+    PQP_GLOBAL int* fi = (PQP_GLOBAL int*)(v + (DW_CKPT_LANE - 1) * 64 + lane);
+    fi[0] = fl[0];
+    fi[1] = fl[1];
+    __syncthreads();
+    const PQP_LDS long long* lw = (const PQP_LDS long long*)slot_of;
+    PQP_GLOBAL long long* gw = (PQP_GLOBAL long long*)(v + DW_CKPT_LANE * 64);
+    const int nw = (int)(dwave_lds_bytes() / 8);
+    for (int k = lane; k < nw; k += WAVE)
+      gw[k] = lw[k];
+  }
+  __device__ __forceinline__ void restore_vectors(cgptr rec)
+  {
+    cgptr v = rec + DW_CKPT_HEAD;
+    each_vector([&](int k, double& val) __attribute__((always_inline)) { val = v[k * 64 + lane]; });
+    const PQP_GLOBAL int* fi = (const PQP_GLOBAL int*)(v + (DW_CKPT_LANE - 1) * 64 + lane);
+    fl[0] = fi[0];
+    fl[1] = fi[1];
+    PQP_LDS long long* lw = (PQP_LDS long long*)slot_of;
+    const PQP_GLOBAL long long* gw = (const PQP_GLOBAL long long*)(v + DW_CKPT_LANE * 64);
+    const int nw = (int)(dwave_lds_bytes() / 8);
+    for (int k = lane; k < nw; k += WAVE)
+      lw[k] = gw[k];
+    __syncthreads();
   }
 
   __device__ __forceinline__ void unscaled_cols(cgptr M, int R, const double (&c)[2], double (&out)[2])
@@ -2221,194 +2363,307 @@
     duality_gap += zl;
   }
 
-  __device__ __forceinline__ void solve()
-  {
-    State W = *P.state();
-    info.load(*P.info());
-    ruiz_c = W.ruiz_c;
-    dual_feasibility_rhs_2 = W.dual_feasibility_rhs_2;
-#ifdef PQP_STATS
-    {
-      const PQP_GLOBAL long long* gs0 = P.stats();
-      for (int k = lane; k < ST_COUNT + 2; k += WAVE)
-        lds_stat[k] = (k < ST_COUNT) ? gs0[k] : 0;
-      __syncthreads();
-    }
-#endif
-    const long long cyc0 = clock64();
-    const long long wall0 = wall_clock64();
-    DW_S(c)
-    {
-      dx[c] = dres[c] = Hdx[c] = ATdy[c] = CTdz[c] = CTzin[c] = rx[c] = ex[c] = 0.0;
-      dy[c] = se[c] = Adx[c] = 0.0;
-      dz[c] = Cdx[c] = si[c] = rup[c] = 0.0;
-      lv_set(DLV_XP, c, 0.0);
-      lv_set(DLV_YP, c, 0.0);
-      lv_set(DLV_ZP, c, 0.0);
-    }
-    dzero(sd);
-    dzero(rd);
-    dzero(ed);
-    DW_B(b) DW_S(s) dS[b][s] = 1.0;
-    vload(x, P.x(), n);
-    vload(y, P.y(), ne);
-    vload(z, P.z(), ni);
-    {
-      const PQP_GLOBAL int* ga = P.act();
-      DW_S(c)
-      {
-        fl[c] = (idx(c) < ni) ? act_flags(ga[idx(c) < ni ? idx(c) : 0]) : 0;
-        slot_of[idx(c)] = -1;
-        actl[idx(c)] = 0;
-      }
-    }
-    __syncthreads();
-    tic();
-    const int ig = st.initial_guess;
-    const bool wswpr = (ig == PQP_WARM_START_WITH_PREVIOUS_RESULT);
-    const bool dirty = W.dirty != 0;
-    bool do_factor, do_scale_ws, do_aset_from_z, do_eq_guess = false, do_restore = false;
-    if (dirty) {
-      if (ig == PQP_EQUALITY_CONSTRAINED_INITIAL_GUESS || ig == PQP_NO_INITIAL_GUESS) {
-        vzero(x);
-        vzero(y);
-        vzero(z);
-        cold_start(info, st);
-      } else if (wswpr) {
-        cleanup_statistics(info);
-      } else {
-        cold_start(info, st);
-      }
-    }
-    if (ig == PQP_EQUALITY_CONSTRAINED_INITIAL_GUESS) {
-      do_factor = true;
-      do_scale_ws = false;
-      do_aset_from_z = false;
-      do_eq_guess = true;
-    } else if (ig == PQP_NO_INITIAL_GUESS) {
-      do_factor = true;
-      do_scale_ws = false;
-      do_aset_from_z = false;
-    } else if (ig == PQP_COLD_START_WITH_PREVIOUS_RESULT || ig == PQP_WARM_START) {
-      do_factor = true;
-      do_scale_ws = true;
-      do_aset_from_z = true;
-    } else {
-      do_scale_ws = true;
-      if (!dirty && W.refactorize) {
-        do_factor = true;
-        do_aset_from_z = true;
-      } else if (!W.factor_valid) {
-        do_factor = true;
-        do_aset_from_z = true;
-      } else {
-        do_factor = false;
-        do_aset_from_z = false;
-        do_restore = true;
-      }
-    }
-    lv_load(DLV_GS, P.gs(), n);
-    lv_load(DLV_BS, P.bs(), ne);
-    lv_load(DLV_US, P.us(), ni);
-    lv_load(DLV_LS, P.ls(), ni);
-    if (do_scale_ws) {
-      double sx[2], sq[2], sc_[2];
-      vload(sx, P.dlt_x(), n, 1.0);
-      vload(sq, P.dlt_eq(), ne, 1.0);
-      vload(sc_, P.dlt_in(), ni, 1.0);
-      DW_S(k)
-      {
-        x[k] /= sx[k];
-        y[k] = y[k] / sq[k] * ruiz_c;
-        z[k] = z[k] / sc_[k] * ruiz_c;
-      }
-    }
-    vload(dF, P.dF(), n, 1.0);
-    {
-      const bool primal_kept = W.primal_valid != 0 && W.rho_fact == info.rho && !(dirty && !wswpr && W.scaled_valid == 0);
-      W.primal_valid = (do_factor || primal_kept) ? 1 : 0;
-    }
-    if (do_factor) {
-      n_c = 0;
-      n_slots = 0;
-      r = ne;
-      schur_dirty = true;
-    }
-    if (do_restore) {
-      n_c = W.n_c;
-      n_slots = W.n_slots;
-      r = ne + n_slots;
-      {
-        cgptr dSg = P.dS();
-        DW_B(b) DW_S(s)
-        {
-          const int a = didx(b, s);
-          dS[b][s] = (a < r) ? dSg[a] : 1.0;
-        }
-        const PQP_GLOBAL int* ga = P.act();
-        DW_S(c)
-        {
-          const int j = idx(c);
-          if (j < n_slots) {
-            const int i = act_cid(ga[j]);
-            actl[j] = (i >= 0) ? i : 0;
-            if (i >= 0)
-              slot_of[i] = j;
-          }
-        }
-        __syncthreads();
-        DW_S(c) if (idx(c) < ni && slot_of[idx(c)] >= 0) fl[c] |= 8;
-      }
-      build_rowid();
-      schur_dirty = !(W.ls_valid && W.mu_eq_fact == info.mu_eq && W.mu_in_fact == info.mu_in);
-      schur_incremental = W.ls_edited != 0;
-    }
+  __device__ __forceinline__ void solve(const DwTail& tl, int rslot)
+  {
+    State W;
+    long long cyc0, wall0;
     bool pend = false;
     int pend_mode = 0;
     double pend_eps = 1.0;
-    if (do_aset_from_z || do_eq_guess) {
-      if (do_aset_from_z) {
-        DW_S(c) fl[c] = (fl[c] & 11) | ((idx(c) < ni && z[c] != 0) ? 4 : 0);
-      } else {
-        DW_S(c) fl[c] = (fl[c] & 11);
-      }
-      pend = true;
-      pend_mode = do_eq_guess ? 1 : 2;
-    }
-
-    const UD bcl_eta_ext_init = pow(0.1, st.alpha_bcl);
-    UD bcl_eta_ext = bcl_eta_ext_init;
+    UD bcl_eta_ext_init, bcl_eta_ext;
     UD bcl_eta_in = 1;
-    const UD eps_in_min = fmin(st.eps_abs, 1.E-9);
+    UD eps_in_min;
     UD primal_feasibility_eq_rhs_0 = 0, primal_feasibility_in_rhs_0 = 0;
     UD dual_feasibility_rhs_0 = 0, dual_feasibility_rhs_1 = 0, dual_feasibility_rhs_3 = 0;
     UD primal_feasibility_lhs = 0, primal_feasibility_eq_lhs = 0, primal_feasibility_in_lhs = 0;
     UD dual_feasibility_lhs = 0;
     UD duality_gap = 0, rhs_duality_gap = 0;
-    UD scaled_eps = st.eps_abs;
+    UD scaled_eps;
     UD primal_feasibility_lhs_new = 0, dual_feasibility_lhs_new = 0;
     UD new_bcl_mu_in = 0, new_bcl_mu_eq = 0, new_bcl_mu_in_inv = 0, new_bcl_mu_eq_inv = 0;
     bool is_primal_feasible = false, is_dual_feasible = false;
     long iter = 0;
     int stage = 0;
-    bool done = (st.max_iter <= 0);
+    bool done = false;
     bool gpr_fresh = false, gdr_fresh = false;
-    aty_fresh = false;
-    {
-      double mz = 0;
-      DW_S(k)
-      {
-        mz = vmax_abs(mz, x[k]);
-        mz = vmax_abs(mz, y[k]);
-        mz = vmax_abs(mz, z[k]);
-      }
-      iterate_zero = lane_max0(mz) == 0.0;
-    }
     UD pl_cache = 0, dl_cache = 0;
-    toc(ST_CYC_F_PANEL);
+    if constexpr (ROLE == DW_TAIL) {
+      cgptr rec = ckpt(tl, rslot);
+      const DwCkptHead& h = *ckpt_head(tl, rslot);
+      info.load(h.info);
+      W = h.W;
+      ruiz_c = h.ruiz_c;
+      dual_feasibility_rhs_2 = h.dual_feasibility_rhs_2;
+      bcl_eta_ext_init = h.bcl_eta_ext_init;
+      bcl_eta_ext = h.bcl_eta_ext;
+      bcl_eta_in = h.bcl_eta_in;
+      eps_in_min = h.eps_in_min;
+      primal_feasibility_eq_rhs_0 = h.primal_feasibility_eq_rhs_0;
+      primal_feasibility_in_rhs_0 = h.primal_feasibility_in_rhs_0;
+      dual_feasibility_rhs_0 = h.dual_feasibility_rhs_0;
+      dual_feasibility_rhs_1 = h.dual_feasibility_rhs_1;
+      dual_feasibility_rhs_3 = h.dual_feasibility_rhs_3;
+      primal_feasibility_lhs = h.primal_feasibility_lhs;
+      primal_feasibility_eq_lhs = h.primal_feasibility_eq_lhs;
+      primal_feasibility_in_lhs = h.primal_feasibility_in_lhs;
+      dual_feasibility_lhs = h.dual_feasibility_lhs;
+      duality_gap = h.duality_gap;
+      rhs_duality_gap = h.rhs_duality_gap;
+      scaled_eps = h.scaled_eps;
+      primal_feasibility_lhs_new = h.primal_feasibility_lhs_new;
+      dual_feasibility_lhs_new = h.dual_feasibility_lhs_new;
+      new_bcl_mu_in = h.new_bcl_mu_in;
+      new_bcl_mu_eq = h.new_bcl_mu_eq;
+      new_bcl_mu_in_inv = h.new_bcl_mu_in_inv;
+      new_bcl_mu_eq_inv = h.new_bcl_mu_eq_inv;
+      pend_eps = uni((double)h.pend_eps);
+      cyc0 = uni((long)h.cyc0);
+      wall0 = uni((long)h.wall0);
+      iter = uni((long)h.iter);
+      n_c = uni(h.n_c);
+      n_slots = uni(h.n_slots);
+      r = uni(h.r);
+      const int fg = uni(h.flags);
+      schur_dirty = (fg & DWF_SCHUR_DIRTY) != 0;
+      schur_incremental = (fg & DWF_SCHUR_INCREMENTAL) != 0;
+      nonfinite = (fg & DWF_NONFINITE) != 0;
+      done = (fg & DWF_DONE) != 0;
+      pend = true;
+      DW_S(c)
+      {
+        dx[c] = Hdx[c] = ATdy[c] = CTdz[c] = CTzin[c] = rx[c] = ex[c] = 0.0;
+        dy[c] = Adx[c] = dz[c] = Cdx[c] = 0.0;
+      }
+      dzero(sd);
+      dzero(rd);
+      dzero(ed);
+      restore_vectors(rec);
+      tic();
+    } else {
+      W = *P.state();
+      info.load(*P.info());
+      ruiz_c = W.ruiz_c;
+      dual_feasibility_rhs_2 = W.dual_feasibility_rhs_2;
+#ifdef PQP_STATS
+      {
+        const PQP_GLOBAL long long* gs0 = P.stats();
+        for (int k = lane; k < ST_COUNT + 2; k += WAVE)
+          lds_stat[k] = (k < ST_COUNT) ? gs0[k] : 0;
+        __syncthreads();
+      }
+#endif
+      cyc0 = clock64();
+      wall0 = wall_clock64();
+      DW_S(c)
+      {
+        dx[c] = dres[c] = Hdx[c] = ATdy[c] = CTdz[c] = CTzin[c] = rx[c] = ex[c] = 0.0;
+        dy[c] = se[c] = Adx[c] = 0.0;
+        dz[c] = Cdx[c] = si[c] = rup[c] = 0.0;
+        lv_set(DLV_XP, c, 0.0);
+        lv_set(DLV_YP, c, 0.0);
+        lv_set(DLV_ZP, c, 0.0);
+      }
+      dzero(sd);
+      dzero(rd);
+      dzero(ed);
+      DW_B(b) DW_S(s) dS[b][s] = 1.0;
+      vload(x, P.x(), n);
+      vload(y, P.y(), ne);
+      vload(z, P.z(), ni);
+      {
+        const PQP_GLOBAL int* ga = P.act();
+        DW_S(c)
+        {
+          fl[c] = (idx(c) < ni) ? act_flags(ga[idx(c) < ni ? idx(c) : 0]) : 0;
+          slot_of[idx(c)] = -1;
+          actl[idx(c)] = 0;
+        }
+      }
+      __syncthreads();
+      tic();
+      const int ig = st.initial_guess;
+      const bool wswpr = (ig == PQP_WARM_START_WITH_PREVIOUS_RESULT);
+      const bool dirty = W.dirty != 0;
+      bool do_factor, do_scale_ws, do_aset_from_z, do_eq_guess = false, do_restore = false;
+      if (dirty) {
+        if (ig == PQP_EQUALITY_CONSTRAINED_INITIAL_GUESS || ig == PQP_NO_INITIAL_GUESS) {
+          vzero(x);
+          vzero(y);
+          vzero(z);
+          cold_start(info, st);
+        } else if (wswpr) {
+          cleanup_statistics(info);
+        } else {
+          cold_start(info, st);
+        }
+      }
+      if (ig == PQP_EQUALITY_CONSTRAINED_INITIAL_GUESS) {
+        do_factor = true;
+        do_scale_ws = false;
+        do_aset_from_z = false;
+        do_eq_guess = true;
+      } else if (ig == PQP_NO_INITIAL_GUESS) {
+        do_factor = true;
+        do_scale_ws = false;
+        do_aset_from_z = false;
+      } else if (ig == PQP_COLD_START_WITH_PREVIOUS_RESULT || ig == PQP_WARM_START) {
+        do_factor = true;
+        do_scale_ws = true;
+        do_aset_from_z = true;
+      } else {
+        do_scale_ws = true;
+        if (!dirty && W.refactorize) {
+          do_factor = true;
+          do_aset_from_z = true;
+        } else if (!W.factor_valid) {
+          do_factor = true;
+          do_aset_from_z = true;
+        } else {
+          do_factor = false;
+          do_aset_from_z = false;
+          do_restore = true;
+        }
+      }
+      lv_load(DLV_GS, P.gs(), n);
+      lv_load(DLV_BS, P.bs(), ne);
+      lv_load(DLV_US, P.us(), ni);
+      lv_load(DLV_LS, P.ls(), ni);
+      if (do_scale_ws) {
+        double sx[2], sq[2], sc_[2];
+        vload(sx, P.dlt_x(), n, 1.0);
+        vload(sq, P.dlt_eq(), ne, 1.0);
+        vload(sc_, P.dlt_in(), ni, 1.0);
+        DW_S(k)
+        {
+          x[k] /= sx[k];
+          y[k] = y[k] / sq[k] * ruiz_c;
+          z[k] = z[k] / sc_[k] * ruiz_c;
+        }
+      }
+      vload(dF, P.dF(), n, 1.0);
+      {
+        const bool primal_kept = W.primal_valid != 0 && W.rho_fact == info.rho && !(dirty && !wswpr && W.scaled_valid == 0);
+        W.primal_valid = (do_factor || primal_kept) ? 1 : 0;
+      }
+      if (do_factor) {
+        n_c = 0;
+        n_slots = 0;
+        r = ne;
+        schur_dirty = true;
+      }
+      if (do_restore) {
+        n_c = W.n_c;
+        n_slots = W.n_slots;
+        r = ne + n_slots;
+        {
+          cgptr dSg = P.dS();
+          DW_B(b) DW_S(s)
+          {
+            const int a = didx(b, s);
+            dS[b][s] = (a < r) ? dSg[a] : 1.0;
+          }
+          const PQP_GLOBAL int* ga = P.act();
+          DW_S(c)
+          {
+            const int j = idx(c);
+            if (j < n_slots) {
+              const int i = act_cid(ga[j]);
+              actl[j] = (i >= 0) ? i : 0;
+              if (i >= 0)
+                slot_of[i] = j;
+            }
+          }
+          __syncthreads();
+          DW_S(c) if (idx(c) < ni && slot_of[idx(c)] >= 0) fl[c] |= 8;
+        }
+        build_rowid();
+        schur_dirty = !(W.ls_valid && W.mu_eq_fact == info.mu_eq && W.mu_in_fact == info.mu_in);
+        schur_incremental = W.ls_edited != 0;
+      }
+      if (do_aset_from_z || do_eq_guess) {
+        if (do_aset_from_z) {
+          DW_S(c) fl[c] = (fl[c] & 11) | ((idx(c) < ni && z[c] != 0) ? 4 : 0);
+        } else {
+          DW_S(c) fl[c] = (fl[c] & 11);
+        }
+        pend = true;
+        pend_mode = do_eq_guess ? 1 : 2;
+      }
+
+      bcl_eta_ext_init = pow(0.1, st.alpha_bcl);
+      bcl_eta_ext = bcl_eta_ext_init;
+      eps_in_min = fmin(st.eps_abs, 1.E-9);
+      scaled_eps = st.eps_abs;
+      done = (st.max_iter <= 0);
+      aty_fresh = false;
+      {
+        double mz = 0;
+        DW_S(k)
+        {
+          mz = vmax_abs(mz, x[k]);
+          mz = vmax_abs(mz, y[k]);
+          mz = vmax_abs(mz, z[k]);
+        }
+        iterate_zero = lane_max0(mz) == 0.0;
+      }
+      toc(ST_CYC_F_PANEL);
+    }
     for (;;) {
       if (pend) {
-        newton_semi_smooth(pend_eps, pend_mode);
+        int yslot = -1;
+        if constexpr (ROLE == DW_HEAD) {
+          if (pend_mode == 0)
+            yslot = yield_slot(tl);
+        }
+        if (yslot < 0)
+          newton_semi_smooth(pend_eps, pend_mode);
+        if constexpr (ROLE == DW_HEAD) {
+          if (PQP_UNLIKELY(yslot >= 0)) {
+            gptr rec = ckpt(tl, yslot);
+            save_vectors(rec);
+            if (lane == 0) {
+              DwCkptHead& h = *ckpt_head(tl, yslot);
+              info.store(h.info);
+              h.W = W;
+              h.ruiz_c = ruiz_c;
+              h.dual_feasibility_rhs_2 = dual_feasibility_rhs_2;
+              h.bcl_eta_ext_init = bcl_eta_ext_init;
+              h.bcl_eta_ext = bcl_eta_ext;
+              h.bcl_eta_in = bcl_eta_in;
+              h.eps_in_min = eps_in_min;
+              h.primal_feasibility_eq_rhs_0 = primal_feasibility_eq_rhs_0;
+              h.primal_feasibility_in_rhs_0 = primal_feasibility_in_rhs_0;
+              h.dual_feasibility_rhs_0 = dual_feasibility_rhs_0;
+              h.dual_feasibility_rhs_1 = dual_feasibility_rhs_1;
+              h.dual_feasibility_rhs_3 = dual_feasibility_rhs_3;
+              h.primal_feasibility_lhs = primal_feasibility_lhs;
+              h.primal_feasibility_eq_lhs = primal_feasibility_eq_lhs;
+              h.primal_feasibility_in_lhs = primal_feasibility_in_lhs;
+              h.dual_feasibility_lhs = dual_feasibility_lhs;
+              h.duality_gap = duality_gap;
+              h.rhs_duality_gap = rhs_duality_gap;
+              h.scaled_eps = scaled_eps;
+              h.primal_feasibility_lhs_new = primal_feasibility_lhs_new;
+              h.dual_feasibility_lhs_new = dual_feasibility_lhs_new;
+              h.new_bcl_mu_in = new_bcl_mu_in;
+              h.new_bcl_mu_eq = new_bcl_mu_eq;
+              h.new_bcl_mu_in_inv = new_bcl_mu_in_inv;
+              h.new_bcl_mu_eq_inv = new_bcl_mu_eq_inv;
+              h.pend_eps = pend_eps;
+              h.cyc0 = cyc0;
+              h.wall0 = wall0;
+              h.iter = iter;
+              h.n_c = n_c;
+              h.n_slots = n_slots;
+              h.r = r;
+              h.flags = (schur_dirty ? DWF_SCHUR_DIRTY : 0) | (schur_incremental ? DWF_SCHUR_INCREMENTAL : 0) |
+                        (nonfinite ? DWF_NONFINITE : 0) | (done ? DWF_DONE : 0);
+              tl.list[yslot] = (int)q;
+              atomicAdd(tl.ctl, -1);
+            }
+            return;
+          }
+        }
         pend = false;
         tic();
         if (pend_mode != 0) {
@@ -2627,6 +2882,10 @@
         done = true;
     }
 
+    if constexpr (ROLE == DW_HEAD) {
+      if (lane == 0)
+        atomicAdd(tl.ctl, -1);
+    }
     tic();
     {
       double sx[2], sq[2], sc_[2];
@@ -2724,13 +2983,21 @@
 #undef DW_S
 #undef DW_B
 
+template<int HB_ = PQP_DW_HB, bool DEFER = false>
 __device__ __forceinline__ void
-dwave_solve_body(const Batch& batch, long q, lptr lds)
+dwave_solve_body(const Batch& batch, long q, lptr lds, const DwTail& tl)
 {
-  DWave S(batch, q, lds);
-  S.solve();
+  DWave<DW_HEAD, HB_, DEFER> S(batch, q, lds);
+  S.solve(tl, 0);
 }
-
+template<int HB_, bool DEFER>
+__device__ __forceinline__ void
+dwave_resume_body(const Batch& batch, int slot, lptr lds, const DwTail& tl)
+{
+  DWave<DW_TAIL, HB_, DEFER> S(batch, (long)tl.list[slot], lds);
+  S.solve(tl, slot);
 }
 
+}
+
 #endif
diff --git a/proxsuite_amd/csrc/pqp_host.hpp b/proxsuite_amd/csrc/pqp_host.hpp
--- a/proxsuite_amd/csrc/pqp_host.hpp
+++ b/proxsuite_amd/csrc/pqp_host.hpp
@@ -51,6 +51,13 @@
   hipEvent_t ev_mid = nullptr;
   bool prologue_timed = false;
   float last_prologue_ms = 0.f;
+  pqp::DwTail tail{};
+  long tail_alloc = 0;
+  int *tail_resumed = nullptr, *tail_resumed_dev = nullptr;
+  hipEvent_t ev_tail = nullptr;
+  bool tail_timed = false;
+  float last_tail_ms = 0.f;
+  int last_tail_count = 0;
   float last_ms = 0.f;
   bool solve_in_flight = false;
   long flight_first = 0, flight_count = 0;
@@ -128,6 +135,7 @@
   int threads;
   size_t lds;
   bool prologue;
+  bool tail = false;
 };
 
 int pqp_launch_setup(pqp_batch* h);
diff --git a/proxsuite_amd/csrc/pqp_kernels.hip b/proxsuite_amd/csrc/pqp_kernels.hip
--- a/proxsuite_amd/csrc/pqp_kernels.hip
+++ b/proxsuite_amd/csrc/pqp_kernels.hip
@@ -12,7 +12,7 @@
 #if (PQP_TU == 1 || PQP_TU == 4 || PQP_TU == 8 || PQP_TU == 9) && !defined(PQP_ZG_DEPTH)
 #define PQP_ZG_DEPTH 4
 #endif
-#if PQP_TU == 16 || PQP_TU == 17
+#if PQP_TU == 16 || PQP_TU == 17 || PQP_TU == 19
 #define PQP_OPAQUE_SCALAR(v)
 #define PQP_OPAQUE_VECTOR(v)
 #endif
@@ -84,7 +84,7 @@
 using pqp_enqueue = int(pqp_batch* h, const LaunchPlan& p, const int* order, bool prepare);
 pqp_enqueue pqp_enqueue_256_4_1, pqp_enqueue_256_3_1, pqp_enqueue_256_2_1, pqp_enqueue_256_1_1, pqp_enqueue_256_3_0,
   pqp_enqueue_256_1_0, pqp_enqueue_256_2_2, pqp_enqueue_diag_wave, pqp_enqueue_dense_wave, pqp_enqueue_prologue,
-  pqp_enqueue_512_2, pqp_enqueue_512_4, pqp_enqueue_1024, pqp_enqueue_hbm;
+  pqp_enqueue_dense_tail, pqp_enqueue_512_2, pqp_enqueue_512_4, pqp_enqueue_1024, pqp_enqueue_hbm;
 #define PQP_SOLVE_ENTRY(name, NT, WPS, SPEC)                                                        \
   int name(pqp_batch* h, const LaunchPlan& p, const int* order, bool prepare) { return enqueue_solve<NT, WPS, SPEC>(h, p, order, prepare); }
 #define PQP_SOLVE_ENTRY_1_0(name, NT, WPS, K_SPEC_1)  \
@@ -154,9 +154,13 @@
 #if PQP_TU_HAS(18)
 template<int NT>
 __global__ __launch_bounds__(NT, 4) void
-pqp_prologue_kernel(pqp::Batch batch, long first, const int* __restrict__ order)
-{
-  HIP_DYNAMIC_SHARED(double, smem)
+pqp_prologue_kernel(pqp::Batch batch, long first, const int* __restrict__ order, pqp::DwTail tl)
+{
+  HIP_DYNAMIC_SHARED(double, smem)
+  if (blockIdx.x == 0 && threadIdx.x == 0 && tl.ctl) {
+    tl.ctl[0] = tl.count;
+    tl.ctl[1] = 0;
+  }
   const long slot = order ? (long)order[blockIdx.x] : (long)blockIdx.x;
   pqp::Solver<NT, 1> S(batch, first + slot, (pqp::lptr)smem);
   S.prologue();
@@ -166,27 +170,62 @@
 pqp_enqueue_prologue(pqp_batch* h, const LaunchPlan&, const int* order, bool prepare)
 {
   static const std::string label = kernel_label<256>("pqp_prologue_kernel");
-  return enqueue(&pqp_prologue_kernel<256>, label, h, 256, h->lds_solve, order, prepare);
+  return enqueue(&pqp_prologue_kernel<256>, label, h, 256, h->lds_solve, order, prepare, h->tail);
 }
 #endif
 #if PQP_TU_HAS(17)
 #ifndef PQP_WPS_DENSE_WAVE
 #define PQP_WPS_DENSE_WAVE 2
 #endif
+#ifndef PQP_DW_DEFER
+#define PQP_DW_DEFER 0
+#endif
 template<int WPS>
 __global__ __launch_bounds__(64, WPS) void
-pqp_dwave_kernel(pqp::Batch batch, long first, const int* __restrict__ order)
+pqp_dwave_kernel(pqp::Batch batch, long first, const int* __restrict__ order, pqp::DwTail tl)
 {
   HIP_DYNAMIC_SHARED(double, smem)
   const long slot = order ? (long)order[blockIdx.x] : (long)blockIdx.x;
-  pqp::dwave_solve_body(batch, first + slot, (pqp::lptr)smem);
+  pqp::dwave_solve_body<PQP_DW_HB, PQP_DW_DEFER != 0>(batch, first + slot, (pqp::lptr)smem, tl);
 }
 
 int
 pqp_enqueue_dense_wave(pqp_batch* h, const LaunchPlan& p, const int* order, bool prepare)
 {
   static const std::string label = kernel_label<PQP_WPS_DENSE_WAVE>("pqp_dwave_kernel");
-  return enqueue(&pqp_dwave_kernel<PQP_WPS_DENSE_WAVE>, label, h, 64, p.lds, order, prepare);
+  return enqueue(&pqp_dwave_kernel<PQP_WPS_DENSE_WAVE>, label, h, 64, p.lds, order, prepare, h->tail);
+}
+#endif
+#if PQP_TU_HAS(19)
+#ifndef PQP_DW_TAIL_HB
+#define PQP_DW_TAIL_HB 2
+#endif
+#ifndef PQP_DW_TAIL_DEFER
+#define PQP_DW_TAIL_DEFER 0
+#endif
+template<int HB, int DEFER>
+__global__ __launch_bounds__(64, 1) void
+dwave_tail_kernel(pqp::Batch batch, pqp::DwTail tl, int* __restrict__ resumed)
+{
+  HIP_DYNAMIC_SHARED(double, smem)
+  int nh = tl.ctl[1];
+  nh = nh < tl.cap ? nh : tl.cap;
+  if (blockIdx.x == 0 && threadIdx.x == 0)
+    *resumed = nh;
+  if ((int)blockIdx.x >= nh)
+    return;
+  pqp::dwave_resume_body<HB, DEFER != 0>(batch, (int)blockIdx.x, (pqp::lptr)smem, tl);
+}
+
+int
+pqp_enqueue_dense_tail(pqp_batch* h, const LaunchPlan& p, const int*, bool prepare)
+{
+  if (prepare)
+    return PQP_OK;
+  hipLaunchKernelGGL((dwave_tail_kernel<PQP_DW_TAIL_HB, PQP_DW_TAIL_DEFER>), dim3((unsigned)h->tail.cap), dim3(64), p.lds, h->stream,
+                     h->dev, h->tail, h->tail_resumed_dev);
+  HIP_TRY(hipGetLastError());
+  return PQP_OK;
 }
 #endif
 #if PQP_TU_HAS(3)
@@ -398,6 +437,29 @@
   if (count < round)
     return 5 * count >= 3 * round;
   return rem == 0 || 5 * rem >= 2 * round;
+}
+
+#ifndef PQP_DWAVE_TAIL_T_CU
+#define PQP_DWAVE_TAIL_T_CU 2
+#endif
+static long
+tail_T(const pqp_batch* h, long count)
+{
+  const char* e = std::getenv("PQP_DWAVE_TAIL");
+  if (e && e[0] == '0')
+    return 0;
+  if (const char* t = std::getenv("PQP_DWAVE_TAIL_T"))
+    return std::min(std::max(0L, std::atol(t)), count);
+  return count > 4L * h->n_cu ? std::min(4L, (long)PQP_DWAVE_TAIL_T_CU) * h->n_cu : 0;
+}
+static long
+tail_yield_at()
+{
+  const char* e = std::getenv("PQP_DWAVE_TAIL");
+  if (e && e[0] == '0')
+    return 0;
+  const char* k = std::getenv("PQP_DWAVE_YIELD_AT");
+  return k ? std::max(0L, std::atol(k)) : 0;
 }
 
 LaunchPlan
@@ -423,7 +485,7 @@
         return workgroup(count <= n_cu ? PQP_K_256_1_0 : PQP_K_256_3_0);
       }
       if (dense_wave(h, count))
-        return LaunchPlan{ PQP_K_DWAVE, 64, pqp::dwave_lds_bytes(), true };
+        return LaunchPlan{ PQP_K_DWAVE, 64, pqp::dwave_lds_bytes(), true, tail_T(h, count) > 0 || tail_yield_at() > 0 };
       if (count > 3 * n_cu && 4 * h->lds_solve <= 160 * 1024)
         return workgroup(PQP_K_256_4_1);
       if (count <= n_cu)
@@ -445,6 +507,43 @@
   pqp_enqueue_hbm, pqp_enqueue_hbm
 };
 
+static int
+prepare_tail(pqp_batch* h, const LaunchPlan& p)
+{
+  pqp::DwTail& t = h->tail;
+  const long T = p.tail ? tail_T(h, h->range_count) : 0, yield_at = p.tail ? tail_yield_at() : 0;
+  const long cap = !p.tail ? 0 : std::max(std::max(4L * h->n_cu, T), yield_at > 0 ? h->range_count : 0L);
+  if (!t.ctl) {
+    void* q = nullptr;
+    HIP_TRY(hipMalloc(&q, 2 * sizeof(int)));
+    HIP_TRY(hipMemset(q, 0, 2 * sizeof(int)));
+    h->allocs.push_back(q);
+    t.ctl = (int*)q;
+    HIP_TRY(hipHostMalloc(&q, sizeof(int), hipHostMallocMapped));
+    h->host_allocs.push_back(q);
+    h->tail_resumed = (int*)q;
+    *h->tail_resumed = 0;
+    void* dq = nullptr;
+    HIP_TRY(hipHostGetDevicePointer(&dq, q, 0));
+    h->tail_resumed_dev = (int*)dq;
+  }
+  if (cap > h->tail_alloc) {
+    void* q = nullptr;
+    HIP_TRY(hipMalloc(&q, size_t(cap) * sizeof(int)));
+    h->allocs.push_back(q);
+    t.list = (int*)q;
+    HIP_TRY(hipMalloc(&q, size_t(cap) * pqp::dwave_ckpt_doubles() * sizeof(double)));
+    h->allocs.push_back(q);
+    t.rec = (double*)q;
+    h->tail_alloc = cap;
+  }
+  t.cap = (int)cap;
+  t.T = (int)T;
+  t.yield_at = (int)yield_at;
+  t.count = (int)h->range_count;
+  return PQP_OK;
+}
+
 int
 pqp_launch_solve(pqp_batch* h)
 {
@@ -454,6 +553,10 @@
   const bool whole = h->range_first == 0 && h->range_count == h->dev.B;
   const int* order = h->subset_order ? h->subset_order : ((h->lpt && h->order_valid && whole) ? h->d_order : nullptr);
   h->prologue_timed = false;
+  h->tail_timed = false;
+  if (p.kernel == PQP_K_DWAVE)
+    if (int rc = prepare_tail(h, p))
+      return rc;
   if (p.prologue)
     if (int rc = pqp_enqueue_prologue(h, p, order, true))
       return rc;
@@ -468,6 +571,12 @@
   }
   if (int rc = ENTRY_OF[p.kernel](h, p, order, false))
     return rc;
+  if (p.tail) {
+    HIP_TRY(hipEventRecord(h->ev_tail, h->stream));
+    if (int rc = pqp_enqueue_dense_tail(h, p, order, false))
+      return rc;
+    h->tail_timed = true;
+  }
   HIP_TRY(hipEventRecord(h->ev1, h->stream));
   return PQP_OK;
 }
diff --git a/proxsuite_amd/csrc/pqp_solver.hpp b/proxsuite_amd/csrc/pqp_solver.hpp
--- a/proxsuite_amd/csrc/pqp_solver.hpp
+++ b/proxsuite_amd/csrc/pqp_solver.hpp
@@ -189,6 +189,17 @@
   const int* trace_slot;
   int trace_cap;
   int primal_reuse;
+};
+
+struct DwTail
+{
+  int* ctl;
+  int* list;
+  double* rec;
+  int cap;
+  int T;
+  int yield_at;
+  int count;
 };
 
 struct BackwardArgs
```

Result: slower. 295,200 QPs/s (-9.3%).
